# cliarie/radix-join

Hardware: AMD Instinct MI355X
Metric: probe_tuples_per_sec (higher is better)
Workload: dtype int32

## Files before the change

include/rj.h:

```cpp
#ifndef RJ_H_
#define RJ_H_

#include <stddef.h>
#include <stdint.h>

#ifdef __cplusplus
extern "C" {
#endif

#define RJ_PAGE_SIZE 8192u

typedef enum rj_dtype {
    RJ_INT32   = 0,
    RJ_INT64   = 1,
    RJ_FP64    = 2,
    RJ_VARCHAR = 3
} rj_dtype;

typedef enum rj_status {
    RJ_OK            = 0,
    RJ_ERR_ARG       = 1,
    RJ_ERR_DEVICE    = 2,
    RJ_ERR_NOMEM     = 3,
    RJ_ERR_DATA      = 4,
// ... 18 lines not shown
    RJ_AGG_SUM        = 3,
    RJ_AGG_MIN        = 4,
    RJ_AGG_MAX        = 5
} rj_agg_func;
#define RJ_AGG_OUT(func, col) (((uint64_t)(func) << 56) | (uint64_t)(col))
#define RJ_AGG_FUNC(x) ((uint32_t)((uint64_t)(x) >> 56))
#define RJ_AGG_COL(x) ((uint64_t)(x) & 0x00ffffffffffffffull)

typedef struct rj_node {
    int32_t         kind;
    int32_t         build_left;
    uint64_t        base_table_id;
    uint64_t        left, right;
    uint64_t        left_attr, right_attr;
    uint64_t        n_out;
    const uint64_t* out_idx;
    const int32_t*  out_type;
} rj_node;

typedef struct rj_column {
    int32_t            type;
    uint64_t           n_pages;
    const void* const* pages;
} rj_column;

typedef struct rj_input {
    uint64_t         num_rows;
    uint64_t         n_cols;
    const rj_column* cols;
} rj_input;

typedef struct rj_plan {
    uint64_t        n_nodes;
    const rj_node*  nodes;
    uint64_t        n_inputs;
    const rj_input* inputs;
    uint64_t        root;
} rj_plan;

typedef struct rj_context rj_context;

#define RJ_COMM_ID_BYTES 128
typedef struct rj_comm_id { char bytes[RJ_COMM_ID_BYTES]; } rj_comm_id;
int rj_comm_id_create(rj_comm_id* out);

enum { RJ_EXCHANGE_AUTO = 0, RJ_EXCHANGE_P2P = 1, RJ_EXCHANGE_RCCL = 2 };

typedef struct rj_config {
    int32_t  device;
    int32_t  profile;
    void*    stream;
    int32_t  radix_bits;
    int32_t  n_devices;
    const int32_t* devices;
    int32_t  world_size;
    int32_t  rank_base;
    const rj_comm_id* comm_id;
    int32_t  exchange;
    int32_t  flags;
} rj_config;

enum { RJ_CTX_PREWARM = 1 };

int         rj_context_create(rj_context** out, const rj_config* cfg );
void        rj_context_destroy(rj_context* ctx);
const char* rj_last_error(const rj_context* ctx);
int         rj_abi_version(void);
uint32_t    rj_context_n_devices(const rj_context* ctx);
rj_context* rj_context_device(rj_context* ctx, uint32_t i);

typedef struct rj_table rj_table;

int  rj_table_upload(rj_context* ctx, const rj_input* host, rj_table** out);

int  rj_table_adopt_device(rj_context* ctx, uint64_t num_rows, uint64_t n_cols,
                           const int32_t* col_type, const void* const* dev_pages,
                           const uint64_t* n_pages, rj_table** out);
void rj_table_release(rj_context* ctx, rj_table* t);

typedef enum rj_filter_opcode {
    RJ_F_EQ = 0, RJ_F_NEQ = 1, RJ_F_LT = 2, RJ_F_GT = 3, RJ_F_LEQ = 4, RJ_F_GEQ = 5,
    RJ_F_IS_NULL = 6, RJ_F_IS_NOT_NULL = 7,
    RJ_F_HOST_BITMAP = 8,
    RJ_F_AND = 9, RJ_F_OR = 10, RJ_F_NOT = 11,
    RJ_F_LIKE = 12, RJ_F_NOT_LIKE = 13
} rj_filter_opcode;

typedef struct rj_filter_op {
    int32_t        op;
    int32_t        column;
    int64_t        ivalue;
    const uint8_t* bytes;
} rj_filter_op;

int rj_table_from_csv(rj_context* ctx, const char* text, uint64_t n_bytes, uint64_t n_cols,
                      const int32_t* col_type, const rj_filter_op* filter, uint64_t n_filter_ops,
                      rj_table** out);
int rj_debug_parse_fp64(const char* field, uint64_t n, uint64_t* bits);
uint64_t rj_table_num_rows(const rj_table* t);
uint64_t rj_table_col_pages(const rj_table* t, uint64_t col);
int      rj_table_copy_pages(rj_context* ctx, const rj_table* t, uint64_t col, void* const* dst, uint64_t n_dst);

typedef struct rj_result rj_result;

enum { RJ_EXEC_KEEP_ON_DEVICE = 1 };

int rj_execute(rj_context* ctx, const rj_plan* plan, rj_result** out);
int rj_execute_resident(rj_context* ctx, const rj_plan* plan, rj_table* const* tables,
                        uint64_t n_tables, int32_t flags, rj_result** out);

uint64_t rj_result_num_rows(const rj_result* r);
uint64_t rj_result_num_cols(const rj_result* r);
int32_t  rj_result_col_type(const rj_result* r, uint64_t col);
uint64_t rj_result_col_pages(const rj_result* r, uint64_t col);
int      rj_result_copy_pages(rj_result* r, uint64_t col, void* const* dst, uint64_t n_dst);
const void* rj_result_device_pages(const rj_result* r, uint64_t col);
void     rj_result_free(rj_result* r);

int rj_execute_sharded(rj_context* ctx, const rj_plan* plan, rj_table* const* tables,
                       uint64_t n_inputs, int32_t flags, rj_result** out );
int rj_plan_shardable(const rj_plan* plan, char* why, size_t why_cap);

int rj_exchange_plan(uint32_t world, uint32_t subs, uint32_t rank, const uint64_t* counts,
                     uint64_t* send_off, uint64_t* send_cnt, uint64_t* recv_off, uint64_t* recv_cnt,
                     uint32_t* seg_begin, uint32_t* seg_end, uint32_t* part_off, uint64_t* n_recv);

typedef struct rj_tuples {
    uint64_t n;
    void*    key;
    void*    carry;
    uint32_t hashed;
    uint32_t reserved;
} rj_tuples;

int  rj_shard_partition(rj_context* ctx, const rj_table* t, uint64_t key_col,
                        uint64_t carry_col, uint32_t n_ranks, rj_tuples* out,
                        uint64_t* counts );

int  rj_join_tuples(rj_context* ctx, const rj_tuples* build, const rj_tuples* probe,
                    uint32_t skip_rank_bits, int32_t flags, rj_result** out);

typedef struct rj_kernel_stat {
    char     name[48];
    uint64_t launches;
    double   total_ms;
} rj_kernel_stat;

int  rj_profile_read(rj_context* ctx, rj_kernel_stat* out, uint64_t cap, uint64_t* n);
void rj_profile_reset(rj_context* ctx);

int  rj_debug_launch_log(rj_context* ctx, int on);
int  rj_debug_launch_read(rj_context* ctx, char* buf, uint64_t cap, uint64_t* need);
int  rj_debug_pool(rj_context* ctx, uint64_t out[4]);

typedef struct rj_device_info {
    char     name[128];
    char     arch[64];
    int32_t  compute_units;
    int32_t  wavefront;
    uint64_t hbm_bytes;
    uint64_t lds_per_cu;
    int32_t  device_count;
    int32_t  reserved;
} rj_device_info;
int rj_device_query(rj_context* ctx, rj_device_info* out);

#ifdef __cplusplus
}
#endif
#endif
```

radix-join_amd/csrc/rj_api.hip:

```cpp
#include <chrono>
#include <cstdlib>
#include <mutex>

#include "rj_internal.hpp"
#include "rj_xplan.hpp"

using namespace rj;

static std::mutex  g_err_mu;
static std::string g_create_error;

template <class F>
static int guarded(rj_context* ctx, F&& f) {
    try {
        f();
        return RJ_OK;
    } catch (const rj::Error& e) {
        if (ctx) ctx->last_error = e.what();
        return e.code;
    } catch (const std::bad_alloc&) {
        if (ctx) ctx->last_error = "host allocation failed";
        return RJ_ERR_NOMEM;
    } catch (const std::exception& e) {
        if (ctx) ctx->last_error = e.what();
// ... 35 lines not shown
            c->device = dev;
            if (first && cfg && cfg->stream) {
                c->stream = static_cast<hipStream_t>(cfg->stream);
            } else {
                RJ_HIP(hipStreamCreateWithFlags(&c->stream, hipStreamNonBlocking));
                c->own_stream = true;
            }
            c->prof.on = cfg && cfg->profile;
            c->prof.level = cfg && cfg->profile >= 2 ? 2 : 1;
            c->prof.stream = c->stream;
            c->radix_bits_override = cfg ? cfg->radix_bits : 0;
            c->tune.from_env();
            c->pool.set_poison(c.get(), c->tune.debug_poison);
            if (!c->radix_bits_override && c->tune.radix_bits > 0) c->radix_bits_override = c->tune.radix_bits;
            return c;
        };
        std::unique_ptr<rj_context> c = make_lane(devs[0], true);
        for (size_t i = 1; i < devs.size(); ++i) {
            rj_context* p = make_lane(devs[i], false).release();
            p->group = c.get();
            c->peers.push_back(p);
        }
        const int world = cfg && cfg->world_size > 0 ? cfg->world_size : (int)devs.size();
        if (world > 1 || (cfg && cfg->exchange != RJ_EXCHANGE_AUTO)) {
            std::vector<Context*> lanes;
            for (int i = 0; i < c->n_lanes(); ++i) lanes.push_back(c->lane(i));
            c->comm.reset(new Comm(lanes, world, cfg ? cfg->rank_base : 0, cfg ? cfg->exchange : 0,
                                   cfg ? cfg->comm_id : nullptr, c->tune.exchange_timeout_ms,
                                   c->tune.bringup_timeout_ms));
        }
        if (cfg && (cfg->flags & RJ_CTX_PREWARM))
            for (int i = 0; i < c->n_lanes(); ++i) c->lane(i)->prewarm();
        RJ_HIP(hipSetDevice(devs[0]));
        *out = c.release();
    } catch (const rj::Error& e) {
        code = e.code;
        msg = e.what();
    } catch (const std::exception& e) {
        code = RJ_ERR_DEVICE;
        msg = e.what();
    }
    if (code != RJ_OK) {
        std::lock_guard<std::mutex> g(g_err_mu);
        g_create_error = msg;
    }
    return code;
}

void rj_context_destroy(rj_context* ctx) {
    if (!ctx) return;
    if (ctx->group) {
        ctx->last_error = "rj_context_destroy: this is a per-device handle owned by its group context (ignored)";
        return;
    }
    delete ctx;
}

uint32_t rj_context_n_devices(const rj_context* ctx) { return ctx ? (uint32_t)ctx->n_lanes() : 0; }

rj_context* rj_context_device(rj_context* ctx, uint32_t i) {
    if (!ctx || i >= (uint32_t)ctx->n_lanes()) return nullptr;
    return static_cast<rj_context*>(ctx->lane((int)i));
}

int rj_comm_id_create(rj_comm_id* out) {
    if (!out) return RJ_ERR_ARG;
    try {
        Comm::make_id(out);
        return RJ_OK;
    } catch (const std::exception& e) {
        std::lock_guard<std::mutex> g(g_err_mu);
        g_create_error = e.what();
        return RJ_ERR_DEVICE;
    }
}

const char* rj_last_error(const rj_context* ctx) {
    if (ctx) return ctx->last_error.c_str();
    std::lock_guard<std::mutex> g(g_err_mu);
    return g_create_error.c_str();
}

int rj_table_upload(rj_context* ctx, const rj_input* host, rj_table** out) {
    if (!ctx || !out) return RJ_ERR_ARG;
    *out = nullptr;
    return guarded(ctx, [&] {
        RJ_HIP(hipSetDevice(ctx->device));
        *out = static_cast<rj_table*>(table_upload(ctx, host));
    });
}

int rj_table_adopt_device(rj_context* ctx, uint64_t num_rows, uint64_t n_cols,
                          const int32_t* col_type, const void* const* dev_pages,
                          const uint64_t* n_pages, rj_table** out) {
    if (!ctx || !out || (n_cols && (!col_type || !dev_pages || !n_pages))) return RJ_ERR_ARG;
    *out = nullptr;
    return guarded(ctx, [&] {
        RJ_HIP(hipSetDevice(ctx->device));
        *out = static_cast<rj_table*>(
            table_adopt(ctx, num_rows, n_cols, col_type, dev_pages, n_pages));
    });
}

int rj_table_from_csv(rj_context* ctx, const char* text, uint64_t n_bytes, uint64_t n_cols, const int32_t* col_type,
                      const rj_filter_op* filter, uint64_t n_filter_ops, rj_table** out) {
    if (!ctx || !out || (n_filter_ops && !filter)) return RJ_ERR_ARG;
    *out = nullptr;
    return guarded(ctx, [&] {
        RJ_HIP(hipSetDevice(ctx->device));
        *out = static_cast<rj_table*>(table_from_csv(ctx, text, n_bytes, n_cols, col_type, filter, n_filter_ops));
    });
}

int rj_debug_parse_fp64(const char* field, uint64_t n, uint64_t* bits) {
    if (!bits || (n && !field)) return RJ_ERR_ARG;
    return rj::parse_fp64_host(field, n, bits);
}

int rj_debug_launch_log(rj_context* ctx, int on) {
    if (!ctx) return RJ_ERR_ARG;
    for (int l = 0; l < ctx->n_lanes(); ++l) {
        ctx->lane(l)->klog.clear();
        ctx->lane(l)->klog.on = on != 0;
    }
    return RJ_OK;
}

int rj_debug_launch_read(rj_context* ctx, char* buf, uint64_t cap, uint64_t* need) {
    if (!ctx || !need || (cap && !buf)) return RJ_ERR_ARG;
    return guarded(ctx, [&] {
        std::map<std::string, uint64_t> all;
        for (int l = 0; l < ctx->n_lanes(); ++l) ctx->lane(l)->klog.merge_into(all);
        std::string text;
        for (const auto& kv : all) text += kv.first + " " + std::to_string(kv.second) + "\n";
        *need = text.size() + 1;
        if (cap) {
            const size_t n = std::min<size_t>(text.size(), cap - 1);
            memcpy(buf, text.data(), n);
            buf[n] = 0;
        }
    });
}

int rj_debug_pool(rj_context* ctx, uint64_t out[4]) {
    if (!ctx || !out) return RJ_ERR_ARG;
    out[0] = out[1] = out[2] = out[3] = 0;
    for (int l = 0; l < ctx->n_lanes(); ++l) {
        const DevPool& p = ctx->lane(l)->pool;
        out[0] += p.bytes_in_use();
        out[1] += p.bytes_cached();
        out[2] += p.n_fills();
        out[3] += p.bytes_filled();
    }
    return RJ_OK;
}

uint64_t rj_table_num_rows(const rj_table* t) { return t ? t->num_rows : 0; }
uint64_t rj_table_col_pages(const rj_table* t, uint64_t col) { return table_col_pages(t, col); }

int rj_table_copy_pages(rj_context* ctx, const rj_table* t, uint64_t col, void* const* dst, uint64_t n_dst) {
    if (!ctx || !t || (n_dst && !dst)) return RJ_ERR_ARG;
    return guarded(ctx, [&] {
        RJ_HIP(hipSetDevice(ctx->device));
        table_copy_pages(ctx, t, col, dst, n_dst);
    });
}

void rj_table_release(rj_context* ctx, rj_table* t) {
    (void)ctx;
    delete t;
}

int rj_execute_resident(rj_context* ctx, const rj_plan* plan, rj_table* const* tables,
                        uint64_t n_tables, int32_t flags, rj_result** out) {
    if (!ctx || !plan || !out) return RJ_ERR_ARG;
    *out = nullptr;
    return guarded(ctx, [&] {
        RJ_HIP(hipSetDevice(ctx->device));
        std::vector<Table*> ts(n_tables);
        for (uint64_t i = 0; i < n_tables; ++i) {
            if (!tables[i]) throw rj::Error(RJ_ERR_ARG, "null table");
            ts[i] = tables[i];
        }
        *out = static_cast<rj_result*>(execute_plan(ctx, plan, ts.data(), n_tables, flags));
    });
}

int rj_execute(rj_context* ctx, const rj_plan* plan, rj_result** out) {
    if (!ctx || !plan || !out) return RJ_ERR_ARG;
    *out = nullptr;
    return guarded(ctx, [&] {
        RJ_HIP(hipSetDevice(ctx->device));
        if (plan->n_inputs && !plan->inputs) throw rj::Error(RJ_ERR_ARG, "plan has no inputs");
        std::vector<bool> used(plan->n_inputs, false);
        for (uint64_t i = 0; i < plan->n_nodes; ++i)
            if (plan->nodes[i].kind == RJ_NODE_SCAN) {
                if (plan->nodes[i].base_table_id >= plan->n_inputs)
                    throw rj::Error(RJ_ERR_ARG, "scan: bad base_table_id");
                used[plan->nodes[i].base_table_id] = true;
            }
        std::vector<std::vector<bool>> col_used(plan->n_inputs);
        for (uint64_t i = 0; i < plan->n_inputs; ++i)
            col_used[i].assign(plan->inputs[i].n_cols, false);
        for (uint64_t i = 0; i < plan->n_nodes; ++i) {
            const rj_node& nd = plan->nodes[i];
            if (nd.kind != RJ_NODE_SCAN) continue;
            for (uint64_t k = 0; k < nd.n_out; ++k) {
                if (nd.out_idx[k] >= col_used[nd.base_table_id].size())
                    throw rj::Error(RJ_ERR_ARG, "scan: output attr out of range");
                col_used[nd.base_table_id][nd.out_idx[k]] = true;
            }
        }
        if (ctx->n_lanes() > 1 && !ctx->group) {
            if (Result* r = execute_host_sharded(ctx, plan, used, col_used)) {
                *out = static_cast<rj_result*>(r);
                return;
            }
        }
        const bool  diag = ctx->tune.diag >= 2;
        auto        t0 = std::chrono::steady_clock::now();
        const uint64_t m0 = ctx->pool.n_malloc, tr0 = ctx->pool.n_trim;
        const double   mm0 = ctx->pool.malloc_ms;
        auto        ms_since = [](std::chrono::steady_clock::time_point t) {
            return std::chrono::duration<double, std::milli>(std::chrono::steady_clock::now() - t).count();
        };
        if (ctx->tune.sync_upload > 0) {
            std::vector<std::unique_ptr<Table>> owned(plan->n_inputs);
            std::vector<Table*>                 ts(plan->n_inputs, nullptr);
            rj_input                            none{};
            for (uint64_t i = 0; i < plan->n_inputs; ++i) {
                owned[i].reset(table_upload(ctx, used[i] ? &plan->inputs[i] : &none,
                                            used[i] ? &col_used[i] : nullptr, true));
                ts[i] = owned[i].get();
            }
            double up = ms_since(t0);
            *out = static_cast<rj_result*>(execute_plan(ctx, plan, ts.data(), plan->n_inputs, 0));
            if (diag)
                fprintf(stderr, "[rj host] upload %.2f ms, then plan (device + host VARCHAR) %.2f ms\n", up,
                        ms_since(t0) - up);
            return;
        }
        AsyncUpload  upl(ctx, plan, used, col_used);
        try {
            *out = static_cast<rj_result*>(execute_plan(ctx, plan, nullptr, plan->n_inputs, 0, &upl));
        } catch (...) {
            (void)hipStreamSynchronize(ctx->stream);
            throw;
        }
        if (diag)
            fprintf(stderr,
                    "[rj host] execute %.2f ms (plan walk blocked on uploads for %.2f ms); HBM cache: %llu "
                    "hipMalloc %.2f ms, %llu trims, %.1f GB in use, %.1f GB cached\n",
                    ms_since(t0), upl.wait_ms(), (unsigned long long)(ctx->pool.n_malloc - m0),
                    ctx->pool.malloc_ms - mm0, (unsigned long long)(ctx->pool.n_trim - tr0),
                    ctx->pool.bytes_in_use() / 1e9, ctx->pool.bytes_cached() / 1e9);
    });
}

uint64_t rj_result_num_rows(const rj_result* r) { return r ? r->num_rows : 0; }
uint64_t rj_result_num_cols(const rj_result* r) { return r ? r->cols.size() : 0; }
int32_t  rj_result_col_type(const rj_result* r, uint64_t c) {
    return (r && c < r->cols.size()) ? r->cols[c].type : -1;
}
uint64_t rj_result_col_pages(const rj_result* r, uint64_t c) {
    return (r && c < r->cols.size()) ? r->cols[c].n_pages : 0;
}

int rj_result_copy_pages(rj_result* r, uint64_t col, void* const* dst, uint64_t n_dst) {
    if (!r) return RJ_ERR_ARG;
    return guarded(static_cast<rj_context*>(r->ctx), [&] {
        RJ_HIP(hipSetDevice(r->ctx->device));
        result_copy_pages(r, col, dst, n_dst);
    });
}

const void* rj_result_device_pages(const rj_result* r, uint64_t c) {
    if (!r || c >= r->cols.size() || !r->cols[c].dev_pages) return nullptr;
    if (!r->cols[c].more.empty()) return nullptr;
    return r->cols[c].dev_pages->p;
}

void rj_result_free(rj_result* r) { delete r; }

int rj_execute_sharded(rj_context* ctx, const rj_plan* plan, rj_table* const* tables,
                       uint64_t n_inputs, int32_t flags, rj_result** out) {
    if (!ctx || !plan || !out || (n_inputs && !tables)) return RJ_ERR_ARG;
    const int nl = ctx->n_lanes();
    for (int l = 0; l < nl; ++l) out[l] = nullptr;
    return guarded(ctx, [&] {
        if (ctx->group) throw rj::Error(RJ_ERR_ARG, "rj_execute_sharded wants the group context, not one of its devices");
        std::vector<Table*>  ts((size_t)nl * n_inputs);
        for (size_t i = 0; i < ts.size(); ++i) ts[i] = tables[i];
        std::vector<Result*> rs((size_t)nl, nullptr);
        execute_sharded(ctx, plan, ts.data(), n_inputs, flags, rs.data());
        for (int l = 0; l < nl; ++l) out[l] = static_cast<rj_result*>(rs[l]);
    });
}

int rj_plan_shardable(const rj_plan* plan, char* why, size_t why_cap) {
    std::string w;
    bool        ok = false;
    try {
        ok = plan_shardable(plan, &w);
    } catch (const std::exception& e) {
        w = e.what();
    }
// ... 99 lines not shown
```

radix-join_amd/csrc/rj_context.hip:

```cpp
#include <dlfcn.h>

#include <chrono>
#include <cstdlib>

#include "rj_internal.hpp"

namespace rj {

[[noreturn]] void launch_failed(const char* kernel, const char* what, bool unsupported) {
    throw_fmt(unsupported ? RJ_ERR_UNSUPPORTED : RJ_ERR_DEVICE, "launch %s: %s", kernel, what);
}

static int env_int(const char* name, int def) {
    const char* v = getenv(name);
    return v && *v ? atoi(v) : def;
}

void Tuning::from_env() {
    blocked_mid = env_int("RJ_TUNE_BLOCKED_MID", blocked_mid);
    mall_chunk = env_int("RJ_TUNE_MALL_CHUNK", mall_chunk);
    radix_bits = env_int("RJ_TUNE_RADIX_BITS", radix_bits);
    p1_bits = env_int("RJ_TUNE_P1_BITS", p1_bits);
    fine = env_int("RJ_TUNE_FINE", fine);
    pack = env_int("RJ_TUNE_PACK", pack);
    aos3 = env_int("RJ_TUNE_AOS3", aos3);
    aos_mid = env_int("RJ_TUNE_AOS_MID", aos_mid);
    tpg1 = env_int("RJ_TUNE_TPG1", tpg1);
    xcd_split = env_int("RJ_TUNE_XCD_SPLIT", xcd_split);
    tpg2 = env_int("RJ_TUNE_TPG2", tpg2);
    packed_side = env_int("RJ_TUNE_PACKED_SIDE", packed_side);
    xcd_min_rows = env_int("RJ_TUNE_XCD_MIN_ROWS", xcd_min_rows);
    bcast = env_int("RJ_TUNE_BCAST", bcast);
    diag = env_int("RJ_DIAG", diag);
    varchar_dev_rows = env_int("RJ_TUNE_VARCHAR_DEV", varchar_dev_rows);
    vkey_hash_bits = env_int("RJ_DEBUG_VKEY_HASH_BITS", vkey_hash_bits);
    sync_upload = env_int("RJ_SYNC_UPLOAD", sync_upload);
    wide_carry = env_int("RJ_TUNE_WIDE_CARRY", wide_carry);
    fold_owner = env_int("RJ_TUNE_FOLD_OWNER", fold_owner);
    exchange_timeout_ms = env_int("RJ_EXCHANGE_TIMEOUT_MS", exchange_timeout_ms);
    bringup_timeout_ms = env_int("RJ_BRINGUP_TIMEOUT_MS", bringup_timeout_ms);
    debug_shard_fail = env_int("RJ_DEBUG_SHARD_FAIL", debug_shard_fail);
    debug_shard_fail_rank = env_int("RJ_DEBUG_SHARD_FAIL_RANK", debug_shard_fail_rank);
    if (const char* v = getenv("RJ_DEBUG_POISON"))
        debug_poison = (int)strtol(v, nullptr, 0) & 0x1ff;
}

static size_t round_size(size_t n) {
    const size_t small = 256, big = size_t(2) << 20;
    if (n < (size_t(1) << 20)) return (n + small - 1) / small * small;
    return (n + big - 1) / big * big;
}

void* DevPool::alloc(size_t bytes) {
    size_t need = round_size(bytes ? bytes : 1);
    int    best = -1;
    for (size_t i = 0; i < blocks_.size(); ++i) {
        Block& b = blocks_[i];
        if (!b.free || b.size < need) continue;
        if (b.size > need + need / 2 + (size_t(4) << 20)) continue;
        if (best < 0 || b.size < blocks_[best].size) best = (int)i;
    }
    if (best >= 0) {
        if (poison_) {
            hipError_t e = fill(blocks_[best].p, blocks_[best].size);
            if (e != hipSuccess) throw_fmt(RJ_ERR_DEVICE, "RJ_DEBUG_POISON: fill on alloc failed: %s", hipGetErrorString(e));
        }
        blocks_[best].free = false;
        in_use_ += blocks_[best].size;
        cached_ -= blocks_[best].size;
        return blocks_[best].p;
    }
    void*      p = nullptr;
    auto       t0 = std::chrono::steady_clock::now();
    hipError_t e = hipMalloc(&p, need);
    if (e != hipSuccess) {
        (void)hipGetLastError();
        trim();
        ++n_trim;
        e = hipMalloc(&p, need);
        if (e != hipSuccess) {
            (void)hipGetLastError();
            throw_fmt(RJ_ERR_NOMEM, "hipMalloc(%zu bytes) failed: %s", need, hipGetErrorString(e));
        }
    }
    ++n_malloc;
    malloc_ms += std::chrono::duration<double, std::milli>(std::chrono::steady_clock::now() - t0).count();
    if (poison_) {
        hipError_t f = fill(p, need);
        if (f != hipSuccess) {
            (void)hipFree(p);
            throw_fmt(RJ_ERR_DEVICE, "RJ_DEBUG_POISON: fill on alloc failed: %s", hipGetErrorString(f));
        }
    }
    blocks_.push_back({p, need, false});
    in_use_ += need;
    return p;
}

hipError_t DevPool::fill(void* p, size_t bytes) {
    Context* c = owner_;
    int      prev = -1;
    if (hipGetDevice(&prev) != hipSuccess) prev = -1;
    hipError_t e = prev == c->device ? hipSuccess : hipSetDevice(c->device);
    for (hipStream_t s : {c->stream, c->aux, c->copy_stream})
        if (e == hipSuccess && s) e = hipStreamSynchronize(s);
    if (e == hipSuccess) e = hipMemsetAsync(p, poison_ & 0xff, bytes, c->stream);
    if (e == hipSuccess) e = hipStreamSynchronize(c->stream);
    if (e == hipSuccess) {
        n_fill_.fetch_add(1, std::memory_order_relaxed);
        fill_bytes_.fetch_add(bytes, std::memory_order_relaxed);
    } else {
        (void)hipGetLastError();
    }
    if (prev >= 0 && prev != c->device) (void)hipSetDevice(prev);
    return e;
}

void DevPool::release(void* p) {
    if (!p) return;
    for (Block& b : blocks_)
        if (b.p == p && !b.free) {
            if (poison_ & 0x100) (void)fill(b.p, b.size);
            b.free = true;
            in_use_ -= b.size;
            cached_ += b.size;
            return;
        }
}

void DevPool::trim() {
    std::vector<Block> keep;
    for (Block& b : blocks_) {
        if (b.free) {
            (void)hipFree(b.p);
            cached_ -= b.size;
        } else {
            keep.push_back(b);
        }
    }
    blocks_.swap(keep);
}

DevPool::~DevPool() {
    for (Block& b : blocks_) (void)hipFree(b.p);
}

Buf::Buf(Context* c, size_t n) : ctx(c), bytes(n) { p = c->pool.alloc(n); }
Buf::~Buf() {
    if (ctx && p) ctx->pool.release(p);
}

hipEvent_t Profiler::get_event() {
    if (!spare_.empty()) {
        hipEvent_t e = spare_.back();
        spare_.pop_back();
        return e;
    }
    hipEvent_t e;
    RJ_HIP(hipEventCreate(&e));
    return e;
}

static bool hot_kernel(const char* n) {
    return !strncmp(n, "pass", 4) || !strncmp(n, "join_build", 10) || !strncmp(n, "exchange", 8);
}

bool Profiler::timed(const char* name, hipEvent_t* start, hipEvent_t* stop) {
    if (!on || (level < 2 && !hot_kernel(name))) return false;
    Rec r{name, get_event(), get_event()};
    open_.push_back(r);
    *start = r.a;
    *stop = r.b;
    return true;
}

void Profiler::drain() {
    if (open_.empty()) return;
    RJ_HIP(hipStreamSynchronize(stream));
    for (Rec& r : open_) {
        float ms = 0;
        if (hipEventElapsedTime(&ms, r.a, r.b) == hipSuccess) {
            auto it = totals.find(r.name);
            if (it == totals.end()) {
                order.push_back(r.name);
// ... 154 lines not shown
```

radix-join_amd/csrc/rj_device.hpp:

```cpp
#pragma once
#include <stdint.h>

namespace rj {

constexpr uint32_t PAGE_BYTES = 8192;
constexpr uint32_t ROWS32 = 1984;
constexpr uint32_t ROWS64 = 1007;
constexpr uint32_t HDR32 = 4;
constexpr uint32_t HDR64 = 8;

enum ColKind : int32_t {
    COL_NONE  = 0,
    COL_PAGED = 1,
    COL_DENSE = 2,
    COL_IOTA  = 3
};

struct ColRef {
    const uint8_t* ptr;
    const uint8_t* valid;
    int32_t        kind;
    int32_t        width;
};

enum CarryMode : int32_t {
    CARRY_NONE   = 0,
    CARRY_ROWIDX = 1,
    CARRY_COLUMN = 2,
    CARRY_WIDE   = 3
};

enum WideLayout : int32_t {
    WIDE_NONE = 0,
    WIDE_32S  = 1,
    WIDE_64_32 = 2
};

struct TupleSrc {
    ColRef   key;
    ColRef   carry;
    uint32_t n_rows;
    int32_t  carry_mode;
    int32_t  key_f64;
    int32_t  prehashed;
    int32_t  wide;
    int32_t  pad;
    ColRef   carry2, carry3;
};

constexpr int MAX_WORDS = 4;
struct Words {
    uint32_t* w[MAX_WORDS];
};

#ifndef RJ_PT_THREADS
#define RJ_PT_THREADS 1024
#endif
#ifndef RJ_PT_ITEMS
#define RJ_PT_ITEMS 16
#endif
constexpr int PT_THREADS = RJ_PT_THREADS;
constexpr int PT_ITEMS   = RJ_PT_ITEMS;
constexpr int PT_TILE    = PT_THREADS * PT_ITEMS;
constexpr uint32_t PT_ALL_ITEMS = PT_ITEMS >= 32 ? 0xffffffffu : ((1u << (PT_ITEMS & 31)) - 1u);
#ifndef RJ_PT_CAPBITS
#define RJ_PT_CAPBITS 9
#endif
constexpr int PT_CAPBITS = RJ_PT_CAPBITS;
constexpr int PT_MAXF    = 1 << PT_CAPBITS;
constexpr int PT_MAXBITS = 9;
static_assert(PT_CAPBITS >= PT_MAXBITS && PT_CAPBITS <= 10, "fan-out capacity");
constexpr int PT_FINEBITS = 15;
constexpr int LDS_BYTES  = 160 * 1024;
static_assert(PT_THREADS >= PT_MAXF, "thread d scans digit d");
static_assert(PT_TILE * 8 + 3 * PT_MAXF * 4 + (PT_THREADS / 64) * 4 <= LDS_BYTES,
              "scatter tile does not fit the 160 KiB of LDS");
static_assert((4 << PT_FINEBITS) <= LDS_BYTES, "fine histogram does not fit the LDS");
static_assert(PT_TILE <= 65536, "ranks are packed into 16 bits");
static_assert(PT_ITEMS % 4 == 0 && PT_ITEMS <= 32, "full tiles are loaded as 16-byte vectors; one mask bit per item");

struct PassParams {
    const uint32_t* seg_off;
    const uint32_t* grp_start;
    uint32_t        nseg;
    uint32_t        n;
    uint32_t        shift;
    uint32_t        fanout_log2;
    uint32_t        tiles_per_group;
    uint32_t*       hist;
    uint32_t*       cursor;
    uint32_t        xcd_log2;
    uint32_t        xcd_remap;
    uint16_t*       side_out;
    uint32_t        next_shift, next_mask;
    const uint32_t* seg_end;
    uint32_t        oseg_shift;
    uint32_t        grp_base;
    uint32_t        hi_shift, lo_bits;
};

__host__ __device__ inline uint32_t pass_digit(const PassParams& pp, uint32_t w, uint32_t mask) {
    if (pp.hi_shift) return (((w >> pp.shift) & ((1u << pp.lo_bits) - 1u)) | ((w >> pp.hi_shift) << pp.lo_bits)) & mask;
    return (w >> pp.shift) & mask;
}

#ifndef RJ_JN_THREADS
#define RJ_JN_THREADS 512
#endif
#ifndef RJ_JN_SPT
#define RJ_JN_SPT 8
#endif
#ifndef RJ_JN_CAP
#define RJ_JN_CAP 8192
#endif
constexpr int      JN_THREADS = RJ_JN_THREADS;
constexpr int      JN_SPT     = RJ_JN_SPT;
constexpr int      JN_SUB     = JN_THREADS * JN_SPT;
constexpr int      JN_CAP     = RJ_JN_CAP;
constexpr int      JN_RMAX    = JN_CAP / 2;
constexpr int      JN_RPT     = (JN_RMAX + JN_THREADS - 1) / JN_THREADS;
constexpr int jn_threads(int table_words) { return table_words >= 3 ? 2 * JN_THREADS : JN_THREADS; }
constexpr int jn_min_waves(int table_words) {
    int blocks = (160 * 1024) / (JN_CAP * 4 * table_words + JN_CAP + 1024);
    int w = blocks * jn_threads(table_words) / 256;
    return w > 8 ? 8 : (w < 1 ? 1 : w);
}
static_assert(JN_RPT % 4 == 0 && JN_SPT % 4 == 0, "tuples are loaded as 16-byte vectors");
static_assert(JN_CAP * 4 * 4 + JN_CAP + 1024 <= 160 * 1024, "a four-array join table does not fit the LDS");
#ifndef RJ_JN_PPW
#define RJ_JN_PPW 1
#endif
#ifndef RJ_JN_PPW3
#define RJ_JN_PPW3 4
#endif
constexpr int jn_ppw(int table_words) { return table_words >= 3 ? RJ_JN_PPW3 : RJ_JN_PPW; }
#ifndef RJ_JN_HEAVY
#define RJ_JN_HEAVY 65536
#endif
constexpr uint32_t JN_HEAVY   = RJ_JN_HEAVY;
constexpr uint32_t JN_TARGET_BUILD = JN_RMAX * 3 / 4;

enum StreamMode : int32_t {
    ST_NONE    = 0,
    ST_DENSE32 = 1,
    ST_DENSE64 = 2,
    ST_PAGED32 = 3,
    ST_PAGED64 = 4,
    ST_DENSE96 = 5
};

struct OutStream {
    uint8_t* base;
    int32_t  mode;
    int32_t  pad;
};

struct JoinParams {
    Words           R, S;
    const uint32_t* offR;
    const uint32_t* offS;
    uint32_t        NP;
    uint32_t        radix_bits;
    uint32_t        n_pass;
    uint32_t        pass_bits[4];
    OutStream       key, bc, pc;
    unsigned long long* out_cursor;
    uint64_t        out_cap;
    const uint32_t* heavy_tasks;
    const uint32_t* n_heavy;
    uint32_t        heavy_grid;
    int32_t         packR, packS;
    int32_t         aosR, aosS;
    int32_t         pad;
    unsigned long long* diag;
};

struct SplitParams {
    const uint32_t* rec;
    uint32_t        cw;
    int32_t         n_cols;
    int32_t         valid_word;
    int32_t         pad;
    struct Col {
        uint8_t* out;
        uint8_t* valid;
        int32_t  word;
        int32_t  width;
        int32_t  valid_bit;
        int32_t  paged;
    } col[3];
};

struct VcRow {
    uint32_t page;
    uint32_t beg;
    uint32_t len;
};
struct VcPage {
    uint32_t first;
    uint32_t nr;
    uint32_t kind;
};
constexpr uint32_t VC_CHUNK = 512;

struct BcastParams {
    TupleSrc        R, S;
    OutStream       key, bc, pc;
    unsigned long long* out_cursor;
    uint64_t        out_cap;
};

struct FilterParams {
    TupleSrc        F, P;
    Words           Fw, Pw;
    const uint32_t* offF;
    const uint32_t* offP;
    uint32_t        NP;
    uint32_t        radix_bits;
    int32_t         packP, aosP;
    const uint32_t* heavy_tasks;
    const uint32_t* n_heavy;
    uint32_t        heavy_grid;
    int32_t         anti;
    int32_t         keyless;
    int32_t         pad;
    OutStream       key, pc;
    unsigned long long* out_cursor;
    uint64_t        out_cap;
};

constexpr uint32_t OUTER_NO_ROW = 0xffffffffu;
struct OuterParams {
    TupleSrc        B, P;
    Words           Bw, Pw;
    const uint32_t* offB;
    const uint32_t* offP;
    uint32_t        NP;
    uint32_t        radix_bits;
    int32_t         packB, aosB;
    int32_t         packP, aosP;
    const uint32_t* heavy_tasks;
    const uint32_t* n_heavy;
    uint32_t        heavy_grid;
    int32_t         keyless;
    uint32_t        pad_bc;
    int32_t         pad;
    OutStream       key, bc, pc;
    unsigned long long* out_cursor;
    uint64_t        out_cap;
};

struct FullParams {
    OuterParams     o;
    uint32_t*       flags;
    uint32_t        pad_pc;
    int32_t         use_flags;
};

constexpr int AGG_THREADS = 512;
constexpr int AGG_SPT     = 2;
constexpr int AGG_STEP    = AGG_THREADS * AGG_SPT;
constexpr int AGG_CAP     = 1024;
constexpr int AGG_FREEZE  = AGG_CAP * 5 / 8;
constexpr int AGG_WALK    = 32;
constexpr uint32_t AGG_TARGET = AGG_CAP * 3 / 8;
constexpr int AGG_MAX_COLS = 3;
static_assert((AGG_CAP & (AGG_CAP - 1)) == 0 && AGG_CAP % AGG_THREADS == 0, "table entries: a power of two, whole rows of threads");
static_assert(AGG_CAP * (12 + 28 * AGG_MAX_COLS) + 1024 <= LDS_BYTES, "the widest aggregation table does not fit the LDS");

enum AggNeed : uint32_t { AGG_NEED_COUNT = 1, AGG_NEED_SUM = 2, AGG_NEED_MIN = 4, AGG_NEED_MAX = 8 };
struct AggCol {
    int32_t  word;
    int32_t  width;
    int32_t  valid_bit;
    uint32_t need;
};
struct AggArrays {
    uint8_t*            key;
    unsigned long long* rows;
    unsigned long long* nn[AGG_MAX_COLS];
    unsigned long long* sum[AGG_MAX_COLS];
    long long*          mn[AGG_MAX_COLS];
    long long*          mx[AGG_MAX_COLS];
};
constexpr unsigned long long AGG_NO_KEY = ~0ull;
struct AggParams {
    TupleSrc        src;
    Words           W;
    const uint32_t* off;
    uint32_t        NP;
    int32_t         pack, aos;
    const uint32_t* heavy_tasks;
    const uint32_t* n_heavy;
    uint32_t        heavy_grid;
    int32_t         n_cols;
    int32_t         valid_word;
    AggCol          col[AGG_MAX_COLS];
    AggArrays       out;
    uint8_t*        out_keyvalid;
    unsigned long long* out_cursor;
    uint64_t        out_cap;
    AggArrays       m;
    uint32_t        m_slots;
    uint32_t*       m_overflow;
};

}
// ... 1 lines not shown
```

radix-join_amd/csrc/rj_exec.hip:

```cpp
#include <algorithm>
#include <chrono>
#include <cstdlib>
#include <functional>
#include <set>

#include "rj_internal.hpp"
#include "rj_xplan.hpp"

namespace rj {

namespace {

struct DCol {
    int32_t        type = RJ_INT32;
    int32_t        kind = COL_NONE;
    int32_t        width = 4;
    const uint8_t* ptr = nullptr;
    const uint8_t* valid = nullptr;
    BufP           hold, hold_valid;
    int            vc_table = -1, vc_col = -1;
    const TableColumn* tcol = nullptr;
    ColRef ref() const { return ColRef{ptr, valid, kind, width}; }
};

// ... 132 lines not shown

    void run_shard(const Table* t, uint64_t key_col, uint64_t carry_col, uint32_t n_ranks,
                   rj_tuples* out, uint64_t* counts) {
        if (n_ranks == 0 || (n_ranks & (n_ranks - 1)) || n_ranks > (1u << PT_MAXBITS))
            throw_fmt(RJ_ERR_UNSUPPORTED, "n_ranks must be a power of two <= %d", 1 << PT_MAXBITS);
        if (key_col >= t->cols.size() || carry_col >= t->cols.size())
            throw_fmt(RJ_ERR_ARG, "column out of range");
        DCol k = table_col(t, (int)key_col), c = table_col(t, (int)carry_col);
        if (k.type != RJ_INT32 || c.type != RJ_INT32)
            throw_fmt(RJ_ERR_UNSUPPORTED, "sharded path carries INT32 key + INT32 payload");
        if (c.valid) throw_fmt(RJ_ERR_UNSUPPORTED, "sharded path: payload column has NULLs");
        TupleSrc src{};
        src.key = k.ref();
        src.carry = c.ref();
        src.n_rows = (uint32_t)t->num_rows;
        src.carry_mode = CARRY_COLUMN;
        if (!out->key || !out->carry) throw_fmt(RJ_ERR_ARG, "rj_shard_partition: null output buffers");
        uint32_t rb = ceil_log2(n_ranks);
        Words    ext{};
        ext.w[0] = static_cast<uint32_t*>(out->key);
        ext.w[1] = static_cast<uint32_t*>(out->carry);
        Parted P = partition(&src, nullptr, 1, 1, rb, rb ? 32 - rb : 31,  true, &ext);
        std::vector<uint32_t> off(n_ranks + 1);
        RJ_HIP(hipMemcpyAsync(off.data(), P.off->p, (n_ranks + 1) * 4, hipMemcpyDeviceToHost,
                              ctx->stream));
        ctx->sync();
        for (uint32_t r = 0; r < n_ranks; ++r) counts[r] = off[r + 1] - off[r];
        out->n = off[n_ranks];
        out->hashed = 1;
        out->reserved = 0;
    }

    Context*       ctx;
    const rj_plan* plan;
    Table* const*  tables;
    uint64_t       n_tables;
    int            flags;
    TableFetch*    fetch = nullptr;
    Launch         L;
    std::map<std::pair<const Table*, int>, DCol> decoded_;
    std::map<std::pair<int, int>, std::vector<uint64_t>> vc_dir_;

    DCol table_col(const Table* t, int c) {
        const TableColumn& tc = t->cols[c];
        if (tc.skipped) throw_fmt(RJ_ERR_ARG, "column was not uploaded (not referenced by a scan)");
        DCol               d;
        d.type = tc.type;
        d.tcol = &tc;
        if (tc.type == RJ_VARCHAR) {
            d.kind = COL_IOTA;
            d.width = 4;
            return d;
        }
        d.width = tc.type == RJ_INT32 ? 4 : 8;
        if (t->num_rows == 0) {
            d.kind = COL_DENSE;
            return d;
        }
        if (tc.regular) {
            d.kind = COL_PAGED;
            d.ptr = tc.dev_pages;
            return d;
        }
        auto key = std::make_pair(t, c);
        auto it = decoded_.find(key);
        if (it != decoded_.end()) return it->second;
        uint64_t n = t->num_rows;
        d.kind = COL_DENSE;
        d.hold = ctx->buf(n * d.width);
        d.hold_valid = ctx->buf(n);
        RJ_HIP(hipMemsetAsync(d.hold->p, 0, n * d.width, ctx->stream));
        RJ_HIP(hipMemsetAsync(d.hold_valid->p, 0, n, ctx->stream));
        if (tc.n_pages) {
            BufP row_base = ctx->buf((tc.n_pages + 1) * 4);
            launch_scan_bins(L, tc.page_rows->as<uint32_t>(), (uint32_t)tc.n_pages,
                             row_base->as<uint32_t>(), nullptr);
            launch_decode_pages(L, tc.dev_pages, (uint32_t)tc.n_pages, d.width,
                                row_base->as<uint32_t>(), n, d.hold->as<uint8_t>(),
                                d.hold_valid->as<uint8_t>());
        }
        d.ptr = d.hold->as<uint8_t>();
        d.valid = d.hold_valid->as<uint8_t>();
        decoded_[key] = d;
        return d;
    }

    const Table* table_of(const rj_node& n) {
        return table_by_id(n.base_table_id);
    }
    const Table* table_by_id(uint64_t id) {
        if (id >= n_tables) throw_fmt(RJ_ERR_ARG, "scan: bad base_table_id");
        return fetch ? fetch->get(id) : tables[id];
    }

    Rel scan(const rj_node& n) {
        const Table* t = table_of(n);
        Rel          r;
        r.n = t->num_rows;
        for (uint64_t k = 0; k < n.n_out; ++k) {
            uint64_t c = n.out_idx[k];
            if (c >= t->cols.size()) throw_fmt(RJ_ERR_ARG, "scan: output attr out of range");
            if (t->cols[c].type != n.out_type[k])
                throw_fmt(RJ_ERR_ARG, "scan: declared type differs from the column's type");
            DCol d = table_col(t, (int)c);
            if (d.type == RJ_VARCHAR) {
                d.vc_table = (int)n.base_table_id;
                d.vc_col = (int)c;
            }
            r.cols.push_back(d);
        }
        return r;
    }

    void root_scan(const rj_node& n, Result& res) {
        const Table* t = table_of(n);
        res.num_rows = t->num_rows;
        for (uint64_t k = 0; k < n.n_out; ++k) {
            uint64_t c = n.out_idx[k];
            if (c >= t->cols.size()) throw_fmt(RJ_ERR_ARG, "scan: output attr out of range");
            const TableColumn& tc = t->cols[c];
            if (tc.type != n.out_type[k])
                throw_fmt(RJ_ERR_ARG, "scan: declared type differs from the column's type");
            ResultColumn rc;
            rc.type = tc.type;
            rc.n_pages = tc.n_pages;
            if (tc.skipped) throw_fmt(RJ_ERR_ARG, "column was not uploaded");
            if (tc.type == RJ_VARCHAR) {
                rc.n_pages = tc.vc_pages.size();
                rc.host_pages.resize(rc.n_pages * PAGE_BYTES);
                for (uint64_t pg = 0; pg < rc.n_pages; ++pg)
                    memcpy(rc.host_pages.data() + pg * PAGE_BYTES, tc.vc_pages[pg], PAGE_BYTES);
            } else if (tc.n_pages) {
                rc.dev_pages = ctx->buf(tc.n_pages * PAGE_BYTES);
                RJ_HIP(hipMemcpyAsync(rc.dev_pages->p, tc.dev_pages, tc.n_pages * PAGE_BYTES,
                                      hipMemcpyDeviceToDevice, ctx->stream));
            }
            res.cols.push_back(std::move(rc));
        }
    }

    Rel node(uint64_t idx, Result* root_res, int depth) {
        if (idx >= plan->n_nodes) throw_fmt(RJ_ERR_ARG, "bad node index");
        if (depth > 4096) throw_fmt(RJ_ERR_ARG, "plan too deep (cycle?)");
        const rj_node& n = plan->nodes[idx];
        if (n.kind == RJ_NODE_SCAN) return scan(n);
        if (n.kind == RJ_NODE_AGG) {
            Rel child = node(n.left, nullptr, depth + 1);
            return agg(child, n, root_res);
        }
        const JoinKind& K = join_kind(n.kind);
        Rel             l = node(n.left, nullptr, depth + 1);
        Rel             r = node(n.right, nullptr, depth + 1);
        const JoinSpec  js = join_spec(n, ctx->radix_bits_override);
        if (n.kind == RJ_NODE_OUTER) return outer_join(l, r, js, K, root_res);
        if (n.kind == RJ_NODE_FULL) return full_join(l, r, js, K, root_res);
        if (n.kind != RJ_NODE_JOIN) return filter_join(l, r, js, K, root_res);
        return join_core(l, r, js, root_res);
    }

    static uint32_t tiles_per_group(uint64_t tuples_per_segment, uint64_t target_groups) {
        uint64_t k = (tuples_per_segment + (uint64_t)PT_TILE * target_groups - 1) /
                     ((uint64_t)PT_TILE * target_groups);
        return (uint32_t)std::min<uint64_t>(std::max<uint64_t>(k, 1), 8);
    }

    Parted partition(const TupleSrc* srcp, const WordSrc* ws, int KW, int CW, uint32_t bits,
                     uint32_t shift0 = 0, bool single_pass = false, const Words* external = nullptr,
                     const std::function<void(const uint32_t*)>* after_offsets = nullptr,
                     const PassShape* shape = nullptr) {
        Parted P;
        const bool preseg = shape && shape->nseg > 0;
        P.NW = KW + CW;
        const TupleSrc none{};
        const TupleSrc& src = srcp ? *srcp : none;
        const uint64_t  n = ws ? ws->n : src.n_rows;
        uint32_t       passes = single_pass ? 1 : (bits + PT_MAXBITS - 1) / PT_MAXBITS;
        if (passes == 0) passes = 1;
        std::vector<uint32_t> pbits(passes, bits / passes);
        for (uint32_t i = 0; i < bits % passes; ++i) pbits[i]++;
        if (passes == 2 && ctx->tune.p1_bits > 0) {
            uint32_t b1 = (uint32_t)ctx->tune.p1_bits;
            if (b1 < bits && b1 <= PT_CAPBITS && bits - b1 <= PT_CAPBITS) {
                pbits[0] = b1;
                pbits[1] = bits - b1;
            }
        }

        const bool fine = passes == 2 && bits <= (uint32_t)PT_FINEBITS && !external && !shape &&
                          ctx->tune.fine != 0;
        const int pack_mode = ctx->tune.pack;
        P.packed = ws ? ws->packed
                      : (!external && KW == 1 && CW == 1 && (pack_mode == 1 || (pack_mode == 2 && fine)));
        P.aos3 = KW == 1 && CW == 2 && !external && !single_pass && ctx->tune.aos3 != 0;
        const bool aos_mid = P.aos3 && passes >= 2 &&
                             (ctx->tune.aos_mid == 1 || ctx->tune.aos_mid == 3 || (ctx->tune.aos_mid == 2 && fine));
        const bool mid_side = aos_mid && !fine && ctx->tune.aos_mid != 3;
        BufP  A[MAX_WORDS], B[MAX_WORDS], AOS, MID[2], SIDE[2];
        Words wa{}, wb{}, waos{};
        if (P.aos3) {
            AOS = ctx->buf(std::max<uint64_t>(n, 1) * 12);
            waos.w[0] = AOS->as<uint32_t>();
        }
        if (aos_mid) {
            for (uint32_t k = 0; k < std::min<uint32_t>(passes - 1, 2); ++k) {
                MID[k] = ctx->buf(std::max<uint64_t>(n, 1) * 12);
                if (mid_side) SIDE[k] = ctx->buf(std::max<uint64_t>(n, 1) * 2 + 16);
            }
        }
        const bool packed_side = P.packed && !fine && passes >= 2 && ctx->tune.packed_side != 0 &&
                                 n >= (uint64_t)ctx->tune.xcd_min_rows;
        if (packed_side)
            for (uint32_t k = 0; k < std::min<uint32_t>(passes - 1, 2); ++k)
                SIDE[k] = ctx->buf(std::max<uint64_t>(n, 1) * 2 + 16);
        const int pair_word = CW >= 2 ? KW + CW - 2 : -1;
        for (int a = 0; a < (P.packed ? 1 : P.NW); ++a) {
            if (pair_word >= 0 && a == pair_word + 1) continue;
            const uint64_t wbytes = (P.packed || a == pair_word) ? 8 : 4;
            if (external) {
                wa.w[a] = external->w[a];
                continue;
            }
            if ((P.aos3 && passes == 1) || aos_mid) continue;
            A[a] = ctx->buf(n * wbytes + 2048);
            wa.w[a] = A[a]->as<uint32_t>();
            if (passes > (P.aos3 ? 2u : 1u)) {
                B[a] = ctx->buf(n * wbytes + 2048);
                wb.w[a] = B[a]->as<uint32_t>();
            }
        }
        BufP     seg_off;
        uint32_t nseg = 1, shift = shift0;
        Words    cur = ws ? ws->w : Words{}, nxt = (P.aos3 && passes == 1) ? waos : wa;
        bool     cur_is_a = false;
        BufP       fine_off, fine_cursor, coarse_off, coarse_cursor;
        uint32_t tpg_first = tiles_per_group(n, 4096);
        if (ctx->tune.tpg1 > 0) tpg_first = (uint32_t)ctx->tune.tpg1;
        bool fine_xcd = false;
        if (fine) {
            const uint32_t NB = 1u << bits, F1 = 1u << pbits[0], F2 = 1u << pbits[1];
            BufP           fh = ctx->buf((uint64_t)NB * 4);
            const uint64_t tiles = (n + PT_TILE - 1) / PT_TILE;
            uint32_t       fgrid = (uint32_t)std::min<uint64_t>(tiles, (uint64_t)ctx->compute_units());
            fine_xcd = ctx->tune.xcd_split && n >= (uint64_t)ctx->tune.xcd_min_rows && fgrid >= 8;
            if (fine_xcd) fgrid &= ~7u;
            fine_off = ctx->buf(((uint64_t)NB + 1) * 4);
            fine_cursor = ctx->buf((uint64_t)NB * 4);
            coarse_off = ctx->buf(((uint64_t)F1 + 1) * 4);
            coarse_cursor = ctx->buf((uint64_t)F1 * 4 * (fine_xcd ? 8 : 1));
            BufP coarse_x;
            RJ_HIP(hipMemsetAsync(fh->p, 0, (uint64_t)NB * 4, ctx->stream));
            if (fine_xcd) {
                coarse_x = ctx->buf((uint64_t)F1 * 8 * 4);
                RJ_HIP(hipMemsetAsync(coarse_x->p, 0, (uint64_t)F1 * 8 * 4, ctx->stream));
            }
            uint32_t* cx = fine_xcd ? coarse_x->as<uint32_t>() : nullptr;
            if (ws)
                launch_fine_hist_words(L, ws->w, ws->packed, (uint32_t)n, shift0, pbits[0], pbits[1], fgrid,
                                       fh->as<uint32_t>(), fine_xcd ? tpg_first : 0u, cx);
            else
                launch_fine_hist_src(L, src, KW, shift0, pbits[0], pbits[1], fgrid, fh->as<uint32_t>(),
                                     fine_xcd ? tpg_first : 0u, cx);
            launch_scan_fine(L, fh->as<uint32_t>(), F1, F2, fine_off->as<uint32_t>(),
                             fine_cursor->as<uint32_t>(), coarse_off->as<uint32_t>(),
                             coarse_cursor->as<uint32_t>(), cx);
        }
        struct Ev2 {
            hipEvent_t e = nullptr;
            void       make() { RJ_HIP(hipEventCreateWithFlags(&e, hipEventDisableTiming)); }
            ~Ev2() {
                if (e) (void)hipEventDestroy(e);
            }
        } chunk_ev;
        const bool chunk_second = ctx->tune.mall_chunk > 0 && passes == 2 && !fine && !shape && !ws && !external && P.packed &&
                                  !packed_side && ctx->tune.xcd_split && n >= (uint64_t)ctx->tune.xcd_min_rows;
        const bool blocked_mid = ctx->tune.blocked_mid != 0 && P.packed && passes >= 2 && !fine && !shape && !ws && !external &&
                                 !packed_side && !chunk_second;
        for (uint32_t p = 0; p < passes; ++p) {
            const uint32_t F = 1u << pbits[p];
            PassParams     pp{};
            pp.nseg = nseg;
            pp.n = (uint32_t)n;
            pp.shift = shift;
            pp.fanout_log2 = pbits[p];
            uint32_t n_groups;
            BufP     grp_start;
            const bool      first_preseg = p == 0 && preseg;
            const uint32_t  nseg_in = first_preseg ? shape->nseg : nseg;
            const uint32_t  n_oseg = first_preseg ? shape->n_oseg : nseg;
            const uint64_t  bins = (uint64_t)n_oseg * F;
            if (p == 0 && shape && shape->hi_shift) {
                pp.hi_shift = shape->hi_shift;
                pp.lo_bits = shape->lo_bits;
            }
            if (p == 0 && !preseg) {
                pp.tiles_per_group = tpg_first;
                uint64_t gt = (uint64_t)pp.tiles_per_group * PT_TILE;
                n_groups = (uint32_t)((n + gt - 1) / gt);
            } else {
                pp.tiles_per_group = tiles_per_group(n / nseg_in + 1, 16);
                if (P.aos3 && p + 1 == passes) pp.tiles_per_group = std::min<uint32_t>(pp.tiles_per_group, 2u);
                uint64_t gt = (uint64_t)pp.tiles_per_group * PT_TILE;
                if (ctx->tune.tpg2 > 0) {
                    pp.tiles_per_group = (uint32_t)ctx->tune.tpg2;
                    gt = (uint64_t)pp.tiles_per_group * PT_TILE;
                }
                n_groups = (uint32_t)(n / gt + nseg_in);
                if (ctx->tune.xcd_split && n >= (uint64_t)ctx->tune.xcd_min_rows) {
                    pp.xcd_remap = 1;
                    n_groups += 8;
                }
                const uint32_t* in_off = first_preseg ? shape->seg_begin : seg_off->as<uint32_t>();
                grp_start = ctx->buf(((uint64_t)nseg_in + 1) * 4);
                launch_group_table(L, in_off, nseg_in, (uint32_t)gt, grp_start->as<uint32_t>(),
                                   first_preseg ? shape->seg_end : nullptr);
                pp.nseg = nseg_in;
                pp.seg_off = in_off;
                pp.seg_end = first_preseg ? shape->seg_end : nullptr;
                pp.oseg_shift = first_preseg ? shape->oseg_shift : 0u;
                pp.grp_start = grp_start->as<uint32_t>();
            }
            BufP off, hist, cursor;
            if (fine) {
                off = p == 0 ? coarse_off : fine_off;
                cursor = p == 0 ? coarse_cursor : fine_cursor;
                pp.cursor = cursor->as<uint32_t>();
                pp.xcd_log2 = (p == 0 && fine_xcd) ? 3u : 0u;
            } else {
                pp.xcd_log2 = (ctx->tune.xcd_split && p == 0 && !preseg && n >= (uint64_t)ctx->tune.xcd_min_rows) ? 3u : 0u;
                hist = ctx->buf((bins << pp.xcd_log2) * 4);
                off = ctx->buf((bins + 1) * 4);
                cursor = ctx->buf((bins << pp.xcd_log2) * 4);
                RJ_HIP(hipMemsetAsync(hist->p, 0, (bins << pp.xcd_log2) * 4, ctx->stream));
                pp.hist = hist->as<uint32_t>();
                pp.cursor = cursor->as<uint32_t>();
                if (p == 1 && chunk_second) {
                    RJ_HIP(hipEventSynchronize(chunk_ev.e));
                    const uint32_t* hoff = static_cast<const uint32_t*>(ctx->small_pinned());
                    const uint64_t  gt = (uint64_t)pp.tiles_per_group * PT_TILE;
                    std::vector<uint32_t> gstart(nseg_in + 1, 0);
                    for (uint32_t sgi = 0; sgi < nseg_in; ++sgi)
                        gstart[sgi + 1] = gstart[sgi] + (uint32_t)(((uint64_t)(hoff[sgi + 1] - hoff[sgi]) + gt - 1) / gt);
                    Ev2 e_in, e_aux;
                    e_in.make();
                    e_aux.make();
                    hipStream_t aux = ctx->aux_stream();
                    RJ_HIP(hipEventRecord(e_in.e, ctx->stream));
                    RJ_HIP(hipStreamWaitEvent(aux, e_in.e, 0));
                    Launch L2 = L;
                    L2.stream = aux;
                    const uint32_t CH = (uint32_t)ctx->tune.mall_chunk;
                    uint32_t       c = 0;
                    for (uint32_t s0 = 0; s0 < nseg_in; s0 += CH, ++c) {
                        const uint32_t s1 = std::min(nseg_in, s0 + CH), G = gstart[s1] - gstart[s0];
                        const Launch& Lc = (c & 1u) ? L2 : L;
                        PassParams    pc = pp;
                        pc.nseg = s1 - s0;
                        pc.seg_off = pp.seg_off + s0;
                        pc.grp_start = pp.grp_start + s0;
                        pc.grp_base = gstart[s0];
                        pc.hist = pp.hist + (size_t)s0 * F;
                        pc.cursor = pp.cursor + (size_t)s0 * F;
                        const uint32_t grid = pp.xcd_remap ? ((G + 7u) & ~7u) : G;
                        if (G) launch_pass_hist_packed(Lc, cur.w[0], pc, grid);
                        launch_scan_segments(Lc, pc.hist, pc.seg_off, pc.nseg, F, 0, off->as<uint32_t>() + (size_t)s0 * F, pc.cursor);
                        if (G) launch_pass_scatter_packed(Lc, cur.w[0], pc, grid, nxt.w[0]);
                    }
                    RJ_HIP(hipEventRecord(e_aux.e, aux));
                    RJ_HIP(hipStreamWaitEvent(ctx->stream, e_aux.e, 0));
                    seg_off = off;
                    nseg = (uint32_t)bins;
                    shift += pbits[p];
                    cur = nxt;
                    cur_is_a = (p % 2 == 0);
                    nxt = cur_is_a ? wb : wa;
                    continue;
                }
                if (p == 0 && !ws)
                    launch_pass_hist_src(L, src, KW, pp, n_groups);
                else if ((mid_side || packed_side) && p > 0)
                    launch_pass_hist_digits(L, SIDE[(p - 1) % 2]->as<uint16_t>(), pp, n_groups);
                else if (aos_mid && p > 0)
                    launch_pass_hist_aos3(L, MID[(p - 1) % 2]->as<uint32_t>(), pp, n_groups);
                else if (P.packed && blocked_mid && p > 0)
                    launch_pass_hist_blocked(L, cur.w[0], pp, n_groups);
                else if (P.packed)
                    launch_pass_hist_packed(L, cur.w[0], pp, n_groups);
                else
                    launch_pass_hist_dense(L, cur, pp, n_groups);
                launch_scan_segments(L, pp.hist, first_preseg ? shape->oseg_off : (p == 0 ? nullptr : pp.seg_off),
                                     n_oseg, F, pp.xcd_log2, off->as<uint32_t>(), pp.cursor);
            }
            if (p == 0 && after_offsets) (*after_offsets)(off->as<uint32_t>());
            if (p == 0 && chunk_second) {
                if ((bins + 1) * 4 > Context::SMALL_PINNED / 4) throw_fmt(RJ_ERR_DEVICE, "chunked pass: too many segments");
                RJ_HIP(hipMemcpyAsync(ctx->small_pinned(), off->p, (bins + 1) * 4, hipMemcpyDeviceToHost, ctx->stream));
                chunk_ev.make();
                RJ_HIP(hipEventRecord(chunk_ev.e, ctx->stream));
            }
            if (aos_mid) {
                const bool last = p + 1 == passes;
                Words      o{};
                o.w[0] = last ? waos.w[0] : MID[p % 2]->as<uint32_t>();
                if (!last && mid_side) {
                    pp.side_out = SIDE[p % 2]->as<uint16_t>();
                    pp.next_shift = shift + pbits[p];
                    pp.next_mask = (1u << pbits[p + 1]) - 1u;
                }
                if (p == 0 && !ws)
                    launch_pass_scatter_src(L, src, KW, CW, pp, n_groups, o, true);
                else if (p == 0)
                    launch_pass_scatter_dense(L, cur, P.NW, KW, pp, n_groups, o, true);
                else
                    launch_pass_scatter_aos3(L, MID[(p - 1) % 2]->as<uint32_t>(), pp, n_groups, o.w[0]);
                nxt = o;
            } else if (P.packed) {
                if (packed_side && p + 1 < passes) {
                    pp.side_out = SIDE[p % 2]->as<uint16_t>();
                    pp.next_shift = shift + pbits[p];
                    pp.next_mask = (1u << pbits[p + 1]) - 1u;
                }
                const bool blk_out = blocked_mid && p + 1 < passes;
                if (p == 0 && !ws)
                    launch_pass_scatter_src_packed(L, src, pp, n_groups, nxt.w[0], blk_out);
                else if (blocked_mid)
                    launch_pass_scatter_blocked(L, cur.w[0], pp, n_groups, nxt.w[0], blk_out);
                else
                    launch_pass_scatter_packed(L, cur.w[0], pp, n_groups, nxt.w[0]);
            } else if (p == 0 && !ws) {
                launch_pass_scatter_src(L, src, KW, CW, pp, n_groups, nxt, P.aos3 && p + 1 == passes);
            } else {
                launch_pass_scatter_dense(L, cur, P.NW, pair_word, pp, n_groups, nxt,
                                          P.aos3 && p + 1 == passes);
            }
            seg_off = off;
            nseg = (uint32_t)bins;
            shift += pbits[p];
            cur = nxt;
            cur_is_a = (p % 2 == 0);
            nxt = cur_is_a ? wb : wa;
            if (P.aos3 && p + 2 == passes) nxt = waos;
            if (aos_mid) {
            }
        }
        P.w = cur;
        for (int a = 0; a < P.NW; ++a) P.wbuf[a] = cur_is_a ? A[a] : B[a];
        if (P.aos3) P.wbuf[0] = AOS;
        P.off = seg_off;
        P.NP = nseg;
        P.pbits = pbits;
        if (shape && !shape->prior_bits.empty()) P.pbits.insert(P.pbits.begin(), shape->prior_bits.begin(), shape->prior_bits.end());
        P.n_tuples = n;
        return P;
    }

    struct Side {
        Rel*          rel = nullptr;
        uint64_t      key_col = 0;
        std::set<int> need;
        int           carry_mode = CARRY_NONE;
        int           carry_col = -1;
        int           CW = 0;
        BufP          stream;
        int           stream_mode = ST_NONE;
        std::vector<int> wide_cols;
        int              wide = WIDE_NONE;
        int              valid_word = -1;
        BufP             vword;
        struct WideOut {
            BufP values, valid;
            int  mode = ST_NONE;
        };
        std::map<int, WideOut> wide_out;
        uint64_t null_mask = 0;
        bool     shared = false;
        bool     optional = false;
        bool     nullable(int c) const {
            if (optional || rel->cols[c].valid != nullptr) return true;
            return shared && (c >= 64 || ((null_mask >> c) & 1u));
        }
    };
    static uint64_t null_columns(const Rel& r) {
        uint64_t m = 0;
        for (size_t c = 0; c < r.cols.size() && c < 64; ++c)
            if (r.cols[c].valid != nullptr) m |= 1ull << c;
        return m;
    }

    static uint64_t pages_for(uint64_t rows, int width) {
        uint64_t rf = width == 4 ? ROWS32 : ROWS64;
        return (rows + rf - 1) / rf;
    }

    Rel empty_rel(const JoinSpec& js, Result* root_res) {
        Rel r;
        r.n = 0;
        for (size_t k = 0; k < js.out_type.size(); ++k) {
            DCol d;
            d.type = js.out_type[k];
            d.kind = COL_DENSE;
            d.width = d.type == RJ_INT32 || d.type == RJ_VARCHAR ? 4 : 8;
            r.cols.push_back(d);
        }
        if (root_res) {
            root_res->num_rows = 0;
            for (size_t k = 0; k < js.out_type.size(); ++k) {
                ResultColumn rc;
                rc.type = js.out_type[k];
                root_res->cols.push_back(std::move(rc));
            }
        }
        return r;
    }

    struct JoinState {
        Side     ls, rs;
        bool     build_left = true, is_root = false, f64 = false, need_key_stream = false;
        bool     type_mismatch = false;
        size_t   lw = 0, rw = 0;
        int      KW = 1;
        uint64_t cap_hint = 0;
        const JoinKind* kind = nullptr;
        bool vkey = false;
        struct VKey {
            Rel            rel;
            BufP           rows, hash, valid;
            const uint8_t* pages = nullptr;
            uint32_t       n_pages = 0;
        } vk[2];
        Side&    bs() { return build_left ? ls : rs; }
        Side&    ps() { return build_left ? rs : ls; }
    };

    void join_prepare(Rel& left, Rel& right, const JoinSpec& js, bool is_root, JoinState& st, const JoinKind& K,
                      const uint64_t* shared_nulls = nullptr) {
        st.kind = &K;
        const size_t lw = left.cols.size(), rw = right.cols.size();
        st.lw = lw;
        st.rw = rw;
        st.is_root = is_root;
        st.build_left = js.build_left;
        if (js.left_attr >= lw || js.right_attr >= rw)
            throw_fmt(RJ_ERR_ARG, "join: key attr out of range");
        for (size_t k = 0; k < js.out_idx.size(); ++k) {
            if (js.out_idx[k] >= lw + rw) throw_fmt(RJ_ERR_ARG, "join: output attr out of range");
            const DCol& c = js.out_idx[k] < lw ? left.cols[js.out_idx[k]]
                                               : right.cols[js.out_idx[k] - lw];
            if (c.type != js.out_type[k])
                throw_fmt(RJ_ERR_ARG, "join: declared type differs from the child column's type");
        }
        Side &ls = st.ls, &rs = st.rs;
        ls.rel = &left;
        ls.key_col = js.left_attr;
        rs.rel = &right;
        rs.key_col = js.right_attr;
        if (shared_nulls) {
            ls.shared = rs.shared = true;
            ls.null_mask = shared_nulls[0];
            rs.null_mask = shared_nulls[1];
        }
        const DCol& bk = st.bs().rel->cols[st.bs().key_col];
        const DCol& pk = st.ps().rel->cols[st.ps().key_col];
        if (bk.type < RJ_INT32 || bk.type > RJ_VARCHAR) throw_fmt(RJ_ERR_ARG, "Unsupported join type");
        st.type_mismatch = pk.type != bk.type;
        st.vkey = bk.type == RJ_VARCHAR && !st.type_mismatch;
        st.KW = bk.type == RJ_INT32 ? 1 : 2;
        st.f64 = bk.type == RJ_FP64;
        const bool key_stream_ok =
            K.node == RJ_NODE_JOIN ||
            (!st.type_mismatch && !(K.emits_unmatched && st.ps().rel->cols[st.ps().key_col].valid));
        st.bs().optional = K.build_optional;
        st.ps().optional = K.probe_optional;
        for (size_t k = 0; k < js.out_idx.size(); ++k) {
            bool  is_left = js.out_idx[k] < lw;
            Side& s = is_left ? ls : rs;
            int   c = (int)(is_left ? js.out_idx[k] : js.out_idx[k] - lw);
            if ((uint64_t)c == s.key_col && !st.vkey && key_stream_ok && !s.optional)
                st.need_key_stream = true;
            else
                s.need.insert(c);
        }
        for (Side* s : {&ls, &rs}) {
            if (st.vkey) {
                s->carry_mode = CARRY_ROWIDX;
                s->CW = 1;
            } else if (s->need.empty()) {
                s->carry_mode = CARRY_NONE;
                s->CW = 0;
            } else if (s->need.size() == 1 && !s->nullable(*s->need.begin())) {
                s->carry_mode = CARRY_COLUMN;
                s->carry_col = *s->need.begin();
                s->CW = s->rel->cols[s->carry_col].width / 4;
            } else if (plan_wide_carry(*s, st.KW)) {
                s->carry_mode = CARRY_WIDE;
            } else {
                s->carry_mode = CARRY_ROWIDX;
                s->CW = 1;
            }
        }
        st.cap_hint = std::max(left.n, right.n);
    }

    bool plan_wide_carry(Side& s, int KW, bool honour_switch = true) {
        if ((honour_switch && !ctx->tune.wide_carry) || s.need.empty()) return false;
        int  words = 0, n64 = 0;
        bool any_null = false;
        for (int c : s.need) {
            const DCol& col = s.rel->cols[c];
            if (col.width != 4 && col.width != 8) return false;
            words += col.width / 4;
            n64 += col.width == 8;
            any_null = any_null || s.nullable(c);
        }
        if (any_null) ++words;
        if (words < 2 || words > MAX_WORDS - KW || n64 > 1 || (n64 == 1 && words != 3)) return false;
        s.wide_cols.clear();
        for (int c : s.need)
            if (s.rel->cols[c].width == 8) s.wide_cols.push_back(c);
        for (int c : s.need)
            if (s.rel->cols[c].width == 4) s.wide_cols.push_back(c);
        s.wide = n64 ? WIDE_64_32 : WIDE_32S;
        s.valid_word = any_null ? words - 1 : -1;
        s.CW = words;
        return true;
    }

    void prepare_wide(Side& s) {
        if (s.carry_mode != CARRY_WIDE || s.valid_word < 0 || s.rel->n == 0) return;
        const uint8_t* v[3] = {nullptr, nullptr, nullptr};
        for (size_t i = 0; i < s.wide_cols.size() && i < 3; ++i) v[i] = s.rel->cols[s.wide_cols[i]].valid;
        s.vword = ctx->buf(s.rel->n * 4);
        launch_pack_validity(L, v[0], v[1], v[2], (uint32_t)s.rel->n, s.vword->as<uint32_t>());
    }

    uint32_t join_bits(const JoinSpec& js, uint64_t build_n, uint32_t top_bits_taken = 0) {
        uint32_t bits = js.forced_bits > 0 ? (uint32_t)js.forced_bits
                                           : ceil_log2((build_n + JN_TARGET_BUILD - 1) / JN_TARGET_BUILD);
        if (js.forced_bits <= 0 && bits > 2 * PT_MAXBITS &&
            (build_n >> (2 * PT_MAXBITS)) <= (uint64_t)(JN_RMAX * 0.95))
            bits = 2 * PT_MAXBITS;
        bits = std::min<uint32_t>(std::max<uint32_t>(bits, 1), 21);
        if (top_bits_taken && bits > 32 - top_bits_taken) bits = 32 - top_bits_taken;
        return bits;
    }

    TupleSrc make_src(const JoinState& st, const Side& s, const JoinSpec& js) {
        TupleSrc src{};
        src.key = s.rel->cols[s.key_col].ref();
        src.n_rows = (uint32_t)s.rel->n;
        src.carry_mode = s.carry_mode;
        if (s.carry_mode == CARRY_COLUMN) {
            src.carry = s.rel->cols[s.carry_col].ref();
            if (src.carry.kind == COL_IOTA) src.carry_mode = CARRY_ROWIDX;
        }
        if (s.carry_mode == CARRY_WIDE) {
            ColRef refs[3] = {};
            size_t k = 0;
            for (int c : s.wide_cols) refs[k++] = s.rel->cols[c].ref();
            if (s.valid_word >= 0)
                refs[k++] = ColRef{s.vword ? s.vword->as<uint8_t>() : nullptr, nullptr, COL_DENSE, 4};
            src.wide = s.wide;
            src.carry = refs[0];
            src.carry2 = refs[1];
            src.carry3 = refs[2];
        }
        src.key_f64 = st.f64 ? 1 : 0;
        src.prehashed = js.prehashed ? 1 : 0;
        return src;
    }


    bool broadcast_form(JoinState& st, const JoinSpec& js) const {
        const uint64_t nb = st.bs().rel->n;
        return (nb <= (uint64_t)JN_RMAX && js.forced_bits <= 0 && !js.prehashed && ctx->tune.bcast != 0) || nb == 0 ||
               st.type_mismatch;
    }
    uint32_t stride_grid(uint64_t rows) const {
        return (uint32_t)std::min<uint64_t>((rows + JN_SUB - 1) / JN_SUB, (uint64_t)ctx->compute_units() * 8);
    }

    struct CoParts {
        Parted   B, P;
        BufP     tasks;
        uint32_t max_tasks = 0;
    };
    CoParts partition_sides(JoinState& st, const JoinSpec& js, uint32_t bits) {
        CoParts        cp;
        const TupleSrc sb = make_src(st, st.bs(), js), sp = make_src(st, st.ps(), js);
        cp.B = partition(&sb, nullptr, st.KW, st.bs().CW, bits);
        cp.P = partition(&sp, nullptr, st.KW, st.ps().CW, bits);
        return cp;
    }
    void heavy_tasks(CoParts& cp, const BufP& counters) {
        cp.max_tasks = (uint32_t)(2 * (cp.P.n_tuples / JN_HEAVY) + 2);
        cp.tasks = ctx->buf((uint64_t)cp.max_tasks * 12);
        launch_heavy_tasks_zeroed(cp.B, cp.P, cp.tasks, counters, cp.max_tasks);
    }
    CoParts co_partition(JoinState& st, const JoinSpec& js, uint32_t bits, const BufP& counters) {
        CoParts cp = partition_sides(st, js, bits);
        heavy_tasks(cp, counters);
        return cp;
    }
    BufP zeroed_counters() {
        BufP counters = ctx->buf(16);
        RJ_HIP(hipMemsetAsync(counters->p, 0, 16, ctx->stream));
        return counters;
    }
    template <class Params>
    static void set_heavy(Params& p, const CoParts& cp, const BufP& counters, uint32_t bits) {
        p.NP = cp.B.NP;
        p.radix_bits = bits;
        p.heavy_tasks = cp.tasks->as<uint32_t>();
        p.n_heavy = counters->as<uint32_t>() + 2;
        p.heavy_grid = cp.max_tasks;
    }
    static void set_parts(OuterParams& op, const CoParts& cp, const BufP& counters, uint32_t bits) {
        set_heavy(op, cp, counters, bits);
        op.Bw = cp.B.w;
        op.Pw = cp.P.w;
        op.offB = cp.B.off->as<uint32_t>();
        op.offP = cp.P.off->as<uint32_t>();
        op.packB = cp.B.packed ? 1 : 0;
        op.aosB = cp.B.aos3 ? 1 : 0;
        op.packP = cp.P.packed ? 1 : 0;
        op.aosP = cp.P.aos3 ? 1 : 0;
    }

    static OutStream out_stream(const BufP& b, int mode) { return OutStream{b ? b->as<uint8_t>() : nullptr, mode, 0}; }
    static OutStream out_stream(const Side& s) { return out_stream(s.stream, s.stream_mode); }
    static uint64_t first_cap(uint64_t rows) { return std::min<uint64_t>(rows + 1024, 0xfffffff0ull); }

    struct Emitted {
        uint64_t        nrows = 0;
        BufP            key_stream;
        int             key_mode = ST_NONE;
        std::set<void*> finished;
    };
    template <class LaunchFn>
    Emitted emit_with_retry(JoinState& st, const BufP& counters, uint64_t cap, LaunchFn&& launch) {
        const JoinKind& K = *st.kind;
        Emitted         e;
        e.key_mode = st.need_key_stream ? stream_mode_of(st.is_root, st.KW * 4, true) : ST_NONE;
        for (int attempt = 1;; ++attempt) {
            e.key_stream = e.key_mode != ST_NONE ? ctx->buf(stream_bytes(e.key_mode, cap)) : BufP();
            for (Side* s : {&st.ls, &st.rs})
                s->stream = s->stream_mode != ST_NONE ? ctx->buf(stream_bytes(s->stream_mode, cap)) : BufP();
            if (K.attempts > 1) RJ_HIP(hipMemsetAsync(counters->p, 0, 8, ctx->stream));
            launch(out_stream(e.key_stream, e.key_mode), cap);
            e.finished.clear();
            finish_paged_streams(st, e, counters, cap);
            unsigned long long h = 0;
            RJ_HIP(hipMemcpyAsync(&h, counters->p, 8, hipMemcpyDeviceToHost, ctx->stream));
            ctx->sync();
            e.nrows = h;
            if (e.nrows <= cap) return e;
            if (K.attempts == 1)
                throw_fmt(RJ_ERR_DEVICE, "%s emitted %llu rows out of %llu", K.name, h, (unsigned long long)cap);
            if (e.nrows > 0xfffffff0ull) throw_fmt(RJ_ERR_UNSUPPORTED, "%s result exceeds 2^32 rows (%llu)", K.name, h);
            if (attempt == K.attempts) throw_fmt(RJ_ERR_DEVICE, "%s output overflowed twice", K.name);
            cap = e.nrows;
        }
    }

    Rel join_core(Rel& left, Rel& right, const JoinSpec& js, Result* root_res) {
        if (left.n == 0 || right.n == 0) return empty_rel(js, root_res);
        JoinState st;
        join_prepare(left, right, js, root_res != nullptr, st, join_kind(RJ_NODE_JOIN));
        if (st.type_mismatch) return empty_rel(js, root_res);
        if (st.vkey) hash_varchar_keys(st);
        prepare_wide(st.ls);
        prepare_wide(st.rs);
        Side&          bs = st.bs();
        Side&          ps = st.ps();
        const uint32_t bits = join_bits(js, bs.rel->n, js.top_bits_taken);
        if (ctx->tune.diag >= 2)
            fprintf(stderr, "[rj diag] join build=%llu probe=%llu bits=%u cw=%d/%d\n",
                    (unsigned long long)bs.rel->n, (unsigned long long)ps.rel->n, bits, bs.CW, ps.CW);
        if (broadcast_form(st, js)) return join_finish(st, js, nullptr, bits, root_res);
        CoParts cp = partition_sides(st, js, bits);
        return join_finish(st, js, &cp, bits, root_res);
    }

    Rel join_finish(JoinState& st, const JoinSpec& js, CoParts* cp, uint32_t bits, Result* root_res) {
        Side &    bs = st.bs(), &ps = st.ps();
        const int KW = st.KW;
        BufP counters = ctx->buf(16);
        if (cp) heavy_tasks(*cp, counters);
        plan_carry_streams(st);
        Emitted e = emit_with_retry(st, counters, first_cap(st.cap_hint), [&](const OutStream& key, uint64_t cap) {
            if (!cp) {
                BcastParams bp{};
                bp.R = make_src(st, bs, js);
                bp.S = make_src(st, ps, js);
                bp.key = key;
                bp.bc = out_stream(bs);
                bp.pc = out_stream(ps);
                bp.out_cursor = counters->as<unsigned long long>();
                bp.out_cap = cap;
                launch_join_bcast(L, KW, bs.CW, ps.CW, bp, stride_grid(ps.rel->n));
                return;
            }
            const Parted &PB = cp->B, &PP = cp->P;
            JoinParams    jp{};
            set_heavy(jp, *cp, counters, bits);
            jp.R = PB.w;
            jp.S = PP.w;
            jp.packR = PB.packed ? 1 : 0;
            jp.packS = PP.packed ? 1 : 0;
            jp.aosR = PB.aos3 ? 1 : 0;
            jp.aosS = PP.aos3 ? 1 : 0;
            jp.offR = PB.off->as<uint32_t>();
            jp.offS = PP.off->as<uint32_t>();
            jp.n_pass = (uint32_t)PB.pbits.size();
            for (size_t i = 0; i < PB.pbits.size() && i < 4; ++i) jp.pass_bits[i] = PB.pbits[i];
            jp.key = key;
            jp.bc = out_stream(bs);
            jp.pc = out_stream(ps);
            jp.out_cursor = counters->as<unsigned long long>();
            jp.out_cap = cap;
            BufP diag;
            if (ctx->tune.diag) {
                diag = ctx->buf(16 * 8);
                RJ_HIP(hipMemsetAsync(diag->p, 0, 16 * 8, ctx->stream));
                jp.diag = diag->as<unsigned long long>();
            }
            const uint32_t ppw = join_partitions_per_workgroup(KW, bs.CW, jp);
            launch_join(L, KW, bs.CW, ps.CW, jp, cp->max_tasks + (PB.NP + ppw - 1) / ppw);
            if (diag) {
                unsigned long long hd[16];
                RJ_HIP(hipMemcpyAsync(hd, diag->p, sizeof hd, hipMemcpyDeviceToHost, ctx->stream));
                ctx->sync();
                static const char* names[] = {"loads issued", "table clear", "build", "count/probe",
                                              "prefix+barrier", "reserve", "emit"};
                double tot = 0;
                for (int i = 0; i < 7; ++i) tot += (double)hd[i];
                fprintf(stderr, "[rj diag] join phases (cycles of thread 0, summed over %u workgroups):\n", PB.NP);
                for (int i = 0; i < 7; ++i)
                    fprintf(stderr, "[rj diag]   %-16s %6.1f %%  %8.0f cyc/wg\n", names[i],
                            100.0 * hd[i] / tot, (double)hd[i] / PB.NP);
            }
        });
        if (st.vkey && e.nrows) e.nrows = verify_varchar_pairs(st, e.nrows);
        return join_assemble(st, js, e, root_res);
    }

    Rel filter_join(Rel& left, Rel& right, const JoinSpec& js, const JoinKind& K, Result* root_res) {
        const bool   anti = K.node == RJ_NODE_ANTI;
        Rel&         fil = js.build_left ? left : right;
        Rel&         pre = js.build_left ? right : left;
        const size_t lw = left.cols.size();
        for (uint64_t o : js.out_idx)
            if (o < lw + right.cols.size() && (o < lw) == js.build_left)
                throw_fmt(RJ_ERR_ARG, "%s: output attr %llu names a column of the filter side", K.name,
                          (unsigned long long)o);
        const uint64_t fattr = js.build_left ? js.left_attr : js.right_attr;
        if (fattr < fil.cols.size() && fil.cols[fattr].type == RJ_VARCHAR)
            throw_fmt(RJ_ERR_UNSUPPORTED, "%s on a VARCHAR key", K.name);
        if (pre.n == 0 || (!anti && fil.n == 0)) return empty_rel(js, root_res);
        JoinState st;
        join_prepare(left, right, js, root_res != nullptr, st, K);
        if (st.type_mismatch && !anti) return empty_rel(js, root_res);
        Side&     fs = st.bs();
        Side&     ps = st.ps();
        const int KW = st.KW;
        prepare_wide(ps);
        plan_carry_streams(st);
        const bool     bcast = broadcast_form(st, js);
        const uint32_t bits = join_bits(js, fs.rel->n);
        if (ctx->tune.diag >= 2)
            fprintf(stderr, "[rj diag] %s filter=%llu preserved=%llu %s bits=%u cw=%d\n", K.name,
                    (unsigned long long)fs.rel->n, (unsigned long long)ps.rel->n, bcast ? "broadcast" : "partitioned",
                    bits, ps.CW);

        FilterParams fp{};
        fp.anti = anti ? 1 : 0;
        fp.keyless = st.type_mismatch ? 1 : 0;
        fp.P = make_src(st, ps, js);
        if (bcast && !fp.keyless) fp.F = make_src(st, fs, js);
        BufP counters = zeroed_counters();
        fp.out_cursor = counters->as<unsigned long long>();
        CoParts cp;
        if (!bcast) {
            cp = co_partition(st, js, bits, counters);
            set_heavy(fp, cp, counters, bits);
            fp.Fw = cp.B.w;
            fp.Pw = cp.P.w;
            fp.offF = cp.B.off->as<uint32_t>();
            fp.offP = cp.P.off->as<uint32_t>();
            fp.packP = cp.P.packed ? 1 : 0;
            fp.aosP = cp.P.aos3 ? 1 : 0;
        }
        Emitted e = emit_with_retry(st, counters, ps.rel->n, [&](const OutStream& key, uint64_t cap) {
            fp.key = key;
            fp.pc = out_stream(ps);
            fp.out_cap = cap;
            if (bcast) {
                launch_filter_bcast(L, KW, ps.CW, fp, stride_grid(ps.rel->n));
            } else {
                launch_filter_join(L, KW, ps.CW, fp, cp.max_tasks + cp.B.NP);
                if (anti && (fp.P.key.valid || fp.P.key_f64))
                    launch_filter_nullkeys(L, KW, ps.CW, fp, stride_grid(ps.rel->n));
            }
        });
        return join_assemble(st, js, e, root_res);
    }

    Rel outer_join(Rel& left, Rel& right, const JoinSpec& js, const JoinKind& K, Result* root_res) {
        Rel&           opt = js.build_left ? left : right;
        Rel&           pre = js.build_left ? right : left;
        const uint64_t oattr = js.build_left ? js.left_attr : js.right_attr;
        if (oattr < opt.cols.size() && opt.cols[oattr].type == RJ_VARCHAR)
            throw_fmt(RJ_ERR_UNSUPPORTED, "%s on a VARCHAR key", K.name);
        if (pre.n == 0) return empty_rel(js, root_res);
        JoinState st;
        join_prepare(left, right, js, root_res != nullptr, st, K);
        return outer_probe(st, js, root_res);
    }

    Rel full_join(Rel& left, Rel& right, const JoinSpec& js_in, const JoinKind& K, Result* root_res) {
        for (int side = 0; side < 2; ++side) {
            const Rel&     r = side == 0 ? left : right;
            const uint64_t a = side == 0 ? js_in.left_attr : js_in.right_attr;
            if (a < r.cols.size() && r.cols[a].type == RJ_VARCHAR)
                throw_fmt(RJ_ERR_UNSUPPORTED, "%s on a VARCHAR key", K.name);
        }
        if (left.n == 0 && right.n == 0) {
            JoinState chk;
            join_prepare(left, right, js_in, root_res != nullptr, chk, K);
            refuse_varchar_outputs(chk);
            return empty_rel(js_in, root_res);
        }
        JoinSpec js = js_in;
        if ((js.build_left ? right : left).n == 0) js.build_left = !js.build_left;
        JoinState st;
        join_prepare(left, right, js, root_res != nullptr, st, K);
        return outer_probe(st, js, root_res);
    }

    static void refuse_varchar_outputs(JoinState& st) {
        for (Side* s : {&st.ls, &st.rs})
            for (int c : s->need) {
                if (!s->optional || s->rel->cols[c].type != RJ_VARCHAR) continue;
                if (st.kind->probe_optional)
                    throw_fmt(RJ_ERR_UNSUPPORTED,
                              "full outer join: a VARCHAR column in the output is not supported (%s child column %d)",
                              s == &st.ls ? "left" : "right", c);
                throw_fmt(RJ_ERR_UNSUPPORTED,
                          "outer join: a VARCHAR column of the optional side in the output is not supported "
                          "(child column %d)", c);
            }
    }

    Rel outer_probe(JoinState& st, const JoinSpec& js, Result* root_res) {
        const bool full = st.kind->probe_optional;
        Side&      bs = st.bs();
        Side&      ps = st.ps();
        const int  KW = st.KW;
        refuse_varchar_outputs(st);
        prepare_wide(bs);
        prepare_wide(ps);
        plan_carry_streams(st);
        const bool     bcast = broadcast_form(st, js);
        const uint32_t bits = join_bits(js, bs.rel->n);
        if (ctx->tune.diag >= 2)
            fprintf(stderr, "[rj diag] %s %s=%llu %s=%llu %s bits=%u cw=%d/%d\n", st.kind->name, full ? "built" : "optional",
                    (unsigned long long)bs.rel->n, full ? "probed" : "preserved", (unsigned long long)ps.rel->n,
                    bcast ? "broadcast" : "partitioned", bits, bs.CW, ps.CW);

        FullParams   fp{};
        OuterParams& op = fp.o;
        op.keyless = st.type_mismatch ? 1 : 0;
        op.pad_bc = bs.carry_mode == CARRY_ROWIDX ? OUTER_NO_ROW : 0u;
        op.P = make_src(st, ps, js);
        if (full || !op.keyless) op.B = make_src(st, bs, js);
        BufP counters = zeroed_counters();
        op.out_cursor = counters->as<unsigned long long>();
        CoParts cp;
        if (!bcast) {
            cp = co_partition(st, js, bits, counters);
            set_parts(op, cp, counters, bits);
        }
        BufP flags;
        if (full) {
            fp.pad_pc = ps.carry_mode == CARRY_ROWIDX ? OUTER_NO_ROW : 0u;
            const uint64_t flag_bytes = ((bcast ? (uint64_t)JN_RMAX : cp.B.n_tuples) / 32 + 2) * 4;
            flags = ctx->buf(flag_bytes);
            RJ_HIP(hipMemsetAsync(flags->p, 0, flag_bytes, ctx->stream));
            fp.flags = flags->as<uint32_t>();
            fp.use_flags = bcast ? 1 : 0;
        }
        const uint32_t probe_grid = stride_grid(ps.rel->n), build_grid = stride_grid(bs.rel->n);
        const uint64_t rows0 = std::max(st.cap_hint, full ? bs.rel->n + ps.rel->n : ps.rel->n);
        Emitted e = emit_with_retry(st, counters, first_cap(rows0), [&](const OutStream& key, uint64_t cap) {
            op.key = key;
// ... 1170 lines not shown
```

radix-join_amd/csrc/rj_internal.hpp:

```cpp
#pragma once
#include <hip/hip_runtime.h>

#include <atomic>
#include <cstdarg>
#include <cstdio>
#include <cstring>
#include <functional>
#include <map>
#include <memory>
#include <mutex>
#include <stdexcept>
#include <string>
#include <vector>

#include "../../include/rj.h"
#include "rj_comm.hpp"
#include "rj_device.hpp"
#include "rj_kernels.hpp"

namespace rj {

struct Context;

struct Error : std::runtime_error {
// ... 7 lines not shown
    va_start(ap, fmt);
    vsnprintf(buf, sizeof buf, fmt, ap);
    va_end(ap);
    throw Error(code, buf);
}

#define RJ_HIP(expr)                                                                          \
    do {                                                                                      \
        hipError_t _e = (expr);                                                               \
        if (_e != hipSuccess)                                                                 \
            ::rj::throw_fmt(_e == hipErrorOutOfMemory ? RJ_ERR_NOMEM : RJ_ERR_DEVICE,         \
                            "%s failed: %s (%s:%d)", #expr, hipGetErrorString(_e), __FILE__, \
                            __LINE__);                                                        \
    } while (0)

class DevPool {
   public:
    void* alloc(size_t bytes);
    void  release(void* p);
    void     set_poison(Context* owner, int mode) { owner_ = owner, poison_ = mode; }
    int      poison() const { return poison_; }
    uint64_t n_fills() const { return n_fill_.load(std::memory_order_relaxed); }
    uint64_t bytes_filled() const { return fill_bytes_.load(std::memory_order_relaxed); }
    void  trim();
    ~DevPool();
    size_t bytes_in_use() const { return in_use_; }
    size_t bytes_cached() const { return cached_; }
    uint64_t n_malloc = 0, n_trim = 0;
    double   malloc_ms = 0;

   private:
    struct Block {
        void*  p;
        size_t size;
        bool   free;
    };
    std::vector<Block> blocks_;
    size_t             in_use_ = 0, cached_ = 0;
    Context*           owner_ = nullptr;
    int                poison_ = 0;
    std::atomic<uint64_t> n_fill_{0}, fill_bytes_{0};
    hipError_t         fill(void* p, size_t bytes);
};

struct Buf {
    Context* ctx = nullptr;
    void*    p = nullptr;
    size_t   bytes = 0;
    Buf(Context* c, size_t n);
    ~Buf();
    Buf(const Buf&) = delete;
    Buf& operator=(const Buf&) = delete;
    template <class T>
    T* as() const {
        return reinterpret_cast<T*>(p);
    }
};
using BufP = std::shared_ptr<Buf>;

class Profiler {
   public:
    bool        on = false;
    int         level = 1;
    hipStream_t stream = nullptr;
    bool        timed(const char* name, hipEvent_t* start, hipEvent_t* stop);
    void        drain();
    void        reset();
    struct Tot {
        uint64_t launches = 0;
        double   ms = 0;
    };
    std::map<std::string, Tot> totals;
    std::vector<std::string>   order;
    ~Profiler();

   private:
    struct Rec {
        const char* name;
        hipEvent_t  a, b;
    };
    std::vector<Rec>        open_;
    std::vector<hipEvent_t> spare_;
    hipEvent_t              get_event();
};

class LaunchLog {
   public:
    bool on = false;
    void add(const void* kernel);
    void clear();
    void merge_into(std::map<std::string, uint64_t>& out);

   private:
    std::mutex                         mu_;
    std::map<const void*, uint64_t>    counts_;
    std::map<const void*, std::string> names_;
};

struct TableColumn {
    int32_t  type = 0;
    uint64_t n_pages = 0;
    const uint8_t* dev_pages = nullptr;
    BufP           owned;
    bool           regular = false;
    uint64_t       page_rows_total = 0;
    BufP           page_rows;
    std::vector<uint32_t> page_rows_host;
    std::vector<uint8_t>        host_pages;
    std::vector<const uint8_t*> vc_pages;
    mutable BufP vc_dev, vc_dev_dir;
    bool                        skipped = false;
};

struct Table {
    Context*                 ctx = nullptr;
    uint64_t                 num_rows = 0;
    std::vector<TableColumn> cols;
};

struct ResultColumn {
    int32_t              type = 0;
    uint64_t             n_pages = 0;
    BufP                 dev_pages;
    std::vector<uint8_t> host_pages;
    struct Part {
        Context* ctx;
        BufP     pages;
        uint64_t n_pages;
    };
    std::vector<Part> more;
    uint64_t          n_first = 0;
};

struct Result {
    Context*                  ctx = nullptr;
    uint64_t                  num_rows = 0;
    std::vector<ResultColumn> cols;
};

struct Tuning {
    int blocked_mid = 1;
    int mall_chunk = 0;
    int radix_bits = 0;
    int p1_bits = 0;
    int fine = 1;
    int pack = 1;
    int aos3 = 1;
    int aos_mid = 2;
    int tpg1 = 0;
    int packed_side = 0;
    int tpg2 = 0;
    int xcd_min_rows = 40 << 20;
    int xcd_split = 1;
    int bcast = 1;
    int diag = 0;
    int varchar_dev_rows = 200000;
    int vkey_hash_bits = 0;
    int sync_upload = 0;
    int wide_carry = 1;
    int fold_owner = 1;
    int exchange_timeout_ms = 120000;
    int bringup_timeout_ms = 0;
    int debug_shard_fail = 0, debug_shard_fail_rank = 0;
    int debug_poison = 0;
    void from_env();
};

struct Context {
    Tuning      tune;
    int         device = 0;
    hipStream_t stream = nullptr;
    bool        own_stream = false;
    int         radix_bits_override = 0;
    DevPool     pool;
    Profiler    prof;
    LaunchLog   klog;
    std::string last_error;
    void*  pinned = nullptr;
    size_t pinned_bytes = 0;
    static constexpr size_t SMALL_PINNED = 32768;
    void*  pinned_small = nullptr;
    void*  small_pinned();
    hipStream_t copy_stream = nullptr;
    void*       pinned_up = nullptr;
    size_t      pinned_up_bytes = 0;
    hipStream_t upload_stream();
    hipStream_t aux = nullptr;
    hipStream_t aux_stream();
    void*       upload_staging(size_t bytes);
    Launch launch() {
        Launch L;
        L.stream = stream;
        L.self = this;
        L.timed = prof.on ? [](void* s, const char* n, hipEvent_t* a, hipEvent_t* b) {
            return static_cast<Context*>(s)->prof.timed(n, a, b);
        } : (bool (*)(void*, const char*, hipEvent_t*, hipEvent_t*)) nullptr;
        L.logged = klog.on ? [](void* s, const void* k) { static_cast<Context*>(s)->klog.add(k); }
                           : (void (*)(void*, const void*)) nullptr;
        return L;
    }
    std::vector<Context*>  peers;
    std::unique_ptr<Comm>  comm;
    Context*               group = nullptr;
    int                    n_lanes() const { return 1 + (int)peers.size(); }
    Context*               lane(int i) { return i == 0 ? this : peers[(size_t)i - 1]; }
    int   n_cu = 0;
    int   compute_units();
    void  prewarm();
    BufP  buf(size_t bytes) { return std::make_shared<Buf>(this, bytes ? bytes : 16); }
    void* staging(size_t bytes);
    void  sync() { RJ_HIP(hipStreamSynchronize(stream)); }
    ~Context();
};

struct TableFetch {
    virtual Table* get(uint64_t id) = 0;
    virtual ~TableFetch() = default;
};

Result* execute_plan(Context* ctx, const rj_plan* plan, Table* const* tables, uint64_t n_tables,
                     int flags, TableFetch* fetch = nullptr);
Result* join_tuples(Context* ctx, const rj_tuples* build, const rj_tuples* probe,
                    uint32_t skip_rank_bits, int flags);
void    execute_sharded(Context* group, const rj_plan* plan, Table* const* tables, uint64_t n_inputs,
                        int flags, Result** out);
bool    plan_shardable(const rj_plan* plan, std::string* why);
void    shard_partition(Context* ctx, const Table* t, uint64_t key_col, uint64_t carry_col,
                        uint32_t n_ranks, rj_tuples* out, uint64_t* counts);

Table* table_upload(Context* ctx, const rj_input* host, const std::vector<bool>* col_used = nullptr,
                    bool borrow_varchar = false);
class AsyncUpload : public TableFetch {
   public:
    AsyncUpload(Context* ctx, const rj_plan* plan, const std::vector<bool>& used,
                const std::vector<std::vector<bool>>& col_used);
    ~AsyncUpload() override;
    Table* get(uint64_t id) override;
    double busy_ms() const { return busy_ms_; }
    double wait_ms() const { return wait_ms_; }

   private:
    struct Impl;
    std::unique_ptr<Impl> im_;
    double                busy_ms_ = 0, wait_ms_ = 0;
};
Table* table_adopt(Context* ctx, uint64_t num_rows, uint64_t n_cols, const int32_t* types,
                   const void* const* dev_pages, const uint64_t* n_pages);
void   result_copy_pages(Result* r, uint64_t col, void* const* dst, uint64_t n_dst);
void   upload_host_pages(Context* ctx, const uint8_t* const* pages, uint64_t n_pages, uint8_t* dev);
Result* execute_host_sharded(Context* group, const rj_plan* plan, const std::vector<bool>& used,
                             const std::vector<std::vector<bool>>& col_used);

Table*   table_from_csv(Context* ctx, const char* text, uint64_t n_bytes, uint64_t n_cols, const int32_t* col_type,
                        const rj_filter_op* filter, uint64_t n_filter_ops);
int parse_fp64_host(const char* s, uint64_t n, uint64_t* bits);
uint64_t table_col_pages(const Table* t, uint64_t col);
void     table_copy_pages(Context* ctx, const Table* t, uint64_t col, void* const* dst, uint64_t n_dst);

void parallel_for(size_t n, size_t grain, const std::function<void(size_t, size_t)>& fn);

void copy_page(void* dst, const void* src);
void copy_pages_fence();

void varchar_dir_build(const uint8_t* const* pages, uint64_t n_pages, uint64_t num_rows,
                       std::vector<uint64_t>& row_base);
void varchar_gather_encode(const uint8_t* const* pages, uint64_t n_pages,
                           const std::vector<uint64_t>& row_base, const uint32_t* idx, uint64_t n,
                           std::vector<uint8_t>& out_pages, uint64_t& n_out_pages);

}

struct rj_context : rj::Context {};
struct rj_table : rj::Table {};
struct rj_result : rj::Result {};
```

radix-join_amd/csrc/rj_kernels.hip:

```cpp
#include <hip/hip_ext.h>

#include "rj_kernels.hpp"

#include <algorithm>
#include <type_traits>

namespace rj {

__device__ __forceinline__ uint32_t fmix32(uint32_t h) {
    h ^= h >> 16;
    h *= 0x85ebca6bu;
    h ^= h >> 13;
    h *= 0xc2b2ae35u;
    h ^= h >> 16;
    return h;
}
__device__ __forceinline__ uint32_t unfmix32(uint32_t h) {
    h ^= h >> 16;
    h *= 0x7ed1b41du;
    h ^= (h >> 13) ^ (h >> 26);
    h *= 0xa5cb9243u;
    h ^= h >> 16;
    return h;
}
// ... 703 lines not shown
        ok = drop_invalid(base + PT_TILE <= end, base, end, ok);
        return hash_keys(ok, lo, hi);
    }
    template <int NW>
    __device__ __forceinline__ uint32_t issue_tile(uint32_t base, uint32_t end,
                                                   uint32_t (&w)[PT_ITEMS][NW]) const {
        static_assert(NW == KW + CW, "word count");
        const bool vec = base + PT_TILE <= end;
        uint32_t   lo[PT_ITEMS], hi[PT_ITEMS];
        uint32_t   ok = raw_keys(vec, base, end, lo, hi);
        if constexpr (WIDE == WIDE_32S) {
            uint32_t c0[PT_ITEMS];
            load_col32_any(s.carry, vec, base, end, c0);
#pragma unroll
            for (int j = 0; j < PT_ITEMS; ++j) w[j][KW] = c0[j];
            load_col32_any(s.carry2, vec, base, end, c0);
#pragma unroll
            for (int j = 0; j < PT_ITEMS; ++j) w[j][KW + 1] = c0[j];
            if constexpr (CW == 3) {
                load_col32_any(s.carry3, vec, base, end, c0);
#pragma unroll
                for (int j = 0; j < PT_ITEMS; ++j) w[j][KW + 2] = c0[j];
            }
        } else if constexpr (WIDE == WIDE_64_32) {
            uint32_t c0[PT_ITEMS], c1[PT_ITEMS];
            load_col64(s.carry, vec, base, end, c0, c1);
#pragma unroll
            for (int j = 0; j < PT_ITEMS; ++j) {
                w[j][KW] = c0[j];
                w[j][KW + 1] = c1[j];
            }
            load_col32_any(s.carry2, vec, base, end, c0);
#pragma unroll
            for (int j = 0; j < PT_ITEMS; ++j) w[j][KW + 2] = c0[j];
        } else if constexpr (CW >= 1) {
            if (s.carry_mode == CARRY_ROWIDX) {
#pragma unroll
                for (int j = 0; j < PT_ITEMS; ++j) w[j][KW] = item_row(vec, base, j);
            } else if constexpr (CW == 1) {
                uint32_t c0[PT_ITEMS];
                load_col32(s.carry, vec, base, end, c0);
#pragma unroll
                for (int j = 0; j < PT_ITEMS; ++j) w[j][KW] = c0[j];
            } else {
                uint32_t c0[PT_ITEMS], c1[PT_ITEMS];
                load_col64(s.carry, vec, base, end, c0, c1);
#pragma unroll
                for (int j = 0; j < PT_ITEMS; ++j) {
                    w[j][KW] = c0[j];
                    w[j][KW + 1] = c1[j];
                }
            }
        }
#pragma unroll
        for (int j = 0; j < PT_ITEMS; ++j) {
            w[j][0] = lo[j];
            if constexpr (KW == 2) w[j][1] = hi[j];
        }
        return ok;
    }
    template <int NW>
    __device__ __forceinline__ uint32_t finish_tile(uint32_t base, uint32_t end, uint32_t ok,
                                                    uint32_t (&w)[PT_ITEMS][NW]) const {
        const bool vec = base + PT_TILE <= end;
        uint32_t   lo[PT_ITEMS], hi[PT_ITEMS];
#pragma unroll
        for (int j = 0; j < PT_ITEMS; ++j) {
            lo[j] = w[j][0];
            hi[j] = KW == 2 ? w[j][KW - 1] : 0u;
        }
        ok = drop_invalid(vec, base, end, ok);
        ok = hash_keys(ok, lo, hi);
#pragma unroll
        for (int j = 0; j < PT_ITEMS; ++j) {
            w[j][0] = lo[j];
            if constexpr (KW == 2) w[j][1] = hi[j];
        }
        return ok;
    }
    template <int NW>
    __device__ __forceinline__ uint32_t load_tile(uint32_t base, uint32_t end,
                                                  uint32_t (&w)[PT_ITEMS][NW]) const {
        return finish_tile<NW>(base, end, issue_tile<NW>(base, end, w), w);
    }
};

__device__ __forceinline__ bool group_range(const PassParams& pp, uint32_t g, uint32_t& seg,
                                            uint32_t& begin, uint32_t& end) {
    const uint32_t gt = pp.tiles_per_group * (uint32_t)PT_TILE;
    if (pp.seg_off == nullptr) {
        seg = 0;
        uint64_t b = (uint64_t)g * gt;
        if (b >= pp.n) return false;
        begin = (uint32_t)b;
        end = (uint32_t)min((uint64_t)pp.n, b + gt);
        return true;
    }
    const uint32_t G = pp.grp_start[pp.nseg] - pp.grp_base;
    if (pp.xcd_remap) {
        const uint32_t per = (G + 7u) >> 3;
        if ((g >> 3) >= per) return false;
        g = (g & 7u) * per + (g >> 3);
    }
    if (g >= G) return false;
    uint32_t lo = 0, hi = pp.nseg;
    while (hi - lo > 1) {
        uint32_t mid = (lo + hi) >> 1;
        if (pp.grp_start[mid] - pp.grp_base <= g)
            lo = mid;
        else
            hi = mid;
    }
    seg = lo >> pp.oseg_shift;
    uint32_t gi = g - (pp.grp_start[lo] - pp.grp_base);
    uint64_t b = (uint64_t)pp.seg_off[lo] + (uint64_t)gi * gt;
    begin = (uint32_t)b;
    end = (uint32_t)min((uint64_t)(pp.seg_end ? pp.seg_end[lo] : pp.seg_off[lo + 1]), b + gt);
    return begin < end;
}

template <class L, class = void>
struct loader_needs_begin : std::false_type {};
template <class L>
struct loader_needs_begin<L, std::enable_if_t<L::kNeedsBegin>> : std::true_type {};

template <class Loader>
__global__ __launch_bounds__(PT_THREADS) void k_pass_hist(Loader ld, PassParams pp) {
    __shared__ uint32_t s_h[PT_MAXF];
    uint32_t            seg, begin, end;
    if (!group_range(pp, blockIdx.x, seg, begin, end)) return;
    const uint32_t F = 1u << pp.fanout_log2, mask = F - 1u;
    for (uint32_t d = threadIdx.x; d < F; d += PT_THREADS) s_h[d] = 0;
    lds_barrier();
    for (uint32_t base = begin; base < end; base += PT_TILE) {
        uint32_t hk[PT_ITEMS];
        uint32_t ok;
        if constexpr (loader_needs_begin<Loader>::value)
            ok = ld.key_tile(base, begin, end, hk);
        else
            ok = ld.key_tile(base, end, hk);
#pragma unroll
        for (int j = 0; j < PT_ITEMS; ++j) {
            if ((ok >> j) & 1u) atomicAdd(&s_h[pass_digit(pp, hk[j], mask)], 1u);
        }
    }
    if constexpr (loader_needs_begin<Loader>::value) {
        uint32_t hx;
        if (ld.extra(begin, end, hx)) atomicAdd(&s_h[pass_digit(pp, hx, mask)], 1u);
    }
    lds_barrier();
    for (uint32_t d = threadIdx.x; d < F; d += PT_THREADS) {
        uint32_t c = s_h[d];
        if (c) atomicAdd(&pp.hist[(((size_t)seg * F + d) << pp.xcd_log2) | (blockIdx.x & ((1u << pp.xcd_log2) - 1u))], c);
    }
}

template <class Loader>
__global__ __launch_bounds__(PT_THREADS) void k_fine_hist(Loader ld, uint32_t n, uint32_t shift,
                                                          uint32_t b1, uint32_t b2,
                                                          uint32_t* fine, uint32_t xcd_tpg,
                                                          uint32_t* coarse_x) {
    __shared__ uint32_t s_f[1u << PT_FINEBITS];
    const uint32_t      NB = 1u << (b1 + b2), m1 = (1u << b1) - 1u, m2 = (1u << b2) - 1u;
    for (uint32_t d = threadIdx.x; d < NB; d += PT_THREADS) s_f[d] = 0;
    lds_barrier();
    const uint32_t tiles = (uint32_t)(((uint64_t)n + PT_TILE - 1) / PT_TILE);
    const uint32_t x = blockIdx.x & 7u, gstride = gridDim.x >> 3;
    uint32_t       gk = blockIdx.x >> 3, gj = 0;
    auto           tile_of = [&](uint32_t k, uint32_t j) { return (x + 8u * k) * xcd_tpg + j; };
    auto           advance = [&](uint32_t t) -> uint32_t {
        if (!xcd_tpg) return t + gridDim.x;
        if (++gj < xcd_tpg && tile_of(gk, gj) < tiles) return tile_of(gk, gj);
        gk += gstride;
        gj = 0;
        const uint64_t nt = (uint64_t)(x + 8ull * gk) * xcd_tpg;
        return nt < tiles ? (uint32_t)nt : 0xffffffffu;
    };
    uint32_t t = xcd_tpg ? tile_of(gk, 0) : blockIdx.x;
    uint32_t lo[PT_ITEMS], hi[PT_ITEMS], raw = 0;
    if (t < tiles) raw = ld.issue_keys(t * (uint32_t)PT_TILE, n, lo, hi);
    while (t < tiles) {
        const uint32_t ok = ld.finish_keys(t * (uint32_t)PT_TILE, n, raw, lo, hi);
        uint32_t       q[PT_ITEMS];
#pragma unroll
        for (int j = 0; j < PT_ITEMS; ++j) {
            const uint32_t h = lo[j] >> shift;
            q[j] = ((h & m1) << b2) | ((h >> b1) & m2);
        }
        const uint32_t t2 = advance(t);
        if (t2 < tiles) raw = ld.issue_keys(t2 * (uint32_t)PT_TILE, n, lo, hi);
#pragma unroll
        for (int j = 0; j < PT_ITEMS; ++j)
            if ((ok >> j) & 1u) atomicAdd(&s_f[q[j]], 1u);
        t = t2;
    }
    lds_barrier();
    for (uint32_t d = threadIdx.x; d < NB; d += PT_THREADS) {
        uint32_t c = s_f[d];
        if (c) atomicAdd(&fine[d], c);
    }
    if (xcd_tpg) {
        const uint32_t F2 = 1u << b2;
        for (uint32_t d1 = threadIdx.x; d1 <= m1; d1 += PT_THREADS) {
            uint32_t sum = 0;
            for (uint32_t i = 0; i < F2; ++i) sum += s_f[d1 * F2 + ((i + d1) & m2)];
            if (sum) atomicAdd(&coarse_x[(d1 << 3) | x], sum);
        }
    }
}

__global__ __launch_bounds__(PT_MAXF) void k_scan_fine(const uint32_t* fine, uint32_t F1,
                                                       uint32_t F2, uint32_t* off2,
                                                       uint32_t* cursor2, uint32_t* off1,
                                                       uint32_t* cursor1, const uint32_t* coarse_x) {
    __shared__ uint32_t s_wsum[PT_MAXF / 64];
    const uint32_t      d1 = blockIdx.x, below = d1 * F2;
    uint32_t            sum = 0;
    if ((F2 & 3u) == 0) {
        const uint4* f4 = reinterpret_cast<const uint4*>(fine);
        for (uint32_t i = threadIdx.x; i < below / 4; i += PT_MAXF) {
            const uint4 v = f4[i];
            sum += v.x + v.y + v.z + v.w;
        }
    } else {
        for (uint32_t i = threadIdx.x; i < below; i += PT_MAXF) sum += fine[i];
    }
    uint32_t base, tot;
    (void)block_excl_scan(sum, s_wsum, base);
    lds_barrier();
    const uint32_t v = threadIdx.x < F2 ? fine[below + threadIdx.x] : 0u;
    const uint32_t ex = block_excl_scan(v, s_wsum, tot);
    if (threadIdx.x < F2) {
        off2[below + threadIdx.x] = base + ex;
        cursor2[below + threadIdx.x] = base + ex;
    }
    if (threadIdx.x == 0) {
        off1[d1] = base;
        if (coarse_x) {
            uint32_t at = base;
            for (uint32_t x = 0; x < 8; ++x) {
                cursor1[(d1 << 3) | x] = at;
                at += coarse_x[(d1 << 3) | x];
            }
        } else {
            cursor1[d1] = base;
        }
        if (d1 + 1 == F1) {
            off1[F1] = base + tot;
            off2[(size_t)F1 * F2] = base + tot;
        }
    }
}

template <int NW, class Loader, int PAIR, bool AOS>
__global__ __launch_bounds__(PT_THREADS) void k_pass_scatter(Loader ld, PassParams pp, Words out) {
    static_assert(PAIR < 0 || (PAIR >= 1 && PAIR + 1 < NW), "pair = two carry words behind the key");
    static_assert(!AOS || (NW == 3 && PAIR == 1), "12-byte tuples: one key word + a two-word carry");
    __shared__ uint2    s_stage2[PT_TILE];
    uint32_t* const     s_stage = reinterpret_cast<uint32_t*>(s_stage2);
    __shared__ uint32_t s_cnt[PT_MAXF];
    __shared__ uint32_t s_base[PT_MAXF];
    __shared__ uint32_t s_delta[PT_MAXF];
    __shared__ uint32_t s_wsum[PT_THREADS / 64];
    uint32_t            seg, begin, end;
    if (!group_range(pp, blockIdx.x, seg, begin, end)) return;
    const uint32_t F = 1u << pp.fanout_log2, mask = F - 1u;

    uint32_t run = 0;
    uint32_t w[PT_ITEMS][NW];

    for (uint32_t base = begin; base < end; base += PT_TILE) {
        for (uint32_t d = threadIdx.x; d < F; d += PT_THREADS) s_cnt[d] = 0;
        lds_barrier();

        uint32_t dr[PT_ITEMS];
        const uint32_t ok = ld.template load_tile<NW>(base, end, w);
#pragma unroll
        for (int j = 0; j < PT_ITEMS; ++j) {
            dr[j] = 0xffffffffu;
            if ((ok >> j) & 1u) {
                uint32_t d = pass_digit(pp, w[j][0], mask);
                uint32_t r = atomicAdd(&s_cnt[d], 1u);
                dr[j] = (d << 16) | r;
            }
        }
        lds_barrier();

        uint32_t c = threadIdx.x < F ? s_cnt[threadIdx.x] : 0u;
        if (c) {
            run = atomicAdd(&pp.cursor[(((size_t)seg * F + threadIdx.x) << pp.xcd_log2) |
                                       (blockIdx.x & ((1u << pp.xcd_log2) - 1u))], c);
        }
        uint32_t total;
        uint32_t ex = block_excl_scan(c, s_wsum, total);
        if (threadIdx.x < F) s_base[threadIdx.x] = ex;
        lds_barrier();

#pragma unroll
        for (int j = 0; j < PT_ITEMS; ++j)
            if (dr[j] != 0xffffffffu) dr[j] = s_base[dr[j] >> 16] + (dr[j] & 0xffffu);

        if constexpr (NW == 3 && PAIR == 1) {
            constexpr uint32_t HALF = PT_TILE / 2;
            uint2* const       s_p = s_stage2;
            uint32_t* const    s_k = reinterpret_cast<uint32_t*>(s_stage2 + HALF);
            if (threadIdx.x < F) s_delta[threadIdx.x] = run - ex;
#pragma unroll
            for (int h = 0; h < 2; ++h) {
#pragma unroll
                for (int j = 0; j < PT_ITEMS; ++j) {
                    const uint32_t lp = dr[j] - h * HALF;
                    if (lp < HALF) {
                        s_k[lp] = w[j][0];
                        s_p[lp] = make_uint2(w[j][1], w[j][2]);
                    }
                }
                lds_barrier();
#pragma unroll
                for (int k = 0; k < PT_ITEMS / 2; ++k) {
                    const uint32_t i = k * PT_THREADS + threadIdx.x, gi = h * HALF + i;
                    if (gi < total) {
                        const uint32_t v = s_k[i];
                        const uint2    c = s_p[i];
                        const uint32_t g = s_delta[pass_digit(pp, v, mask)] + gi;
                        if constexpr (AOS) {
                            uint32_t* o = out.w[0] + (size_t)g * 3u;
                            o[0] = v;
                            o[1] = c.x;
                            o[2] = c.y;
                            if (pp.side_out) pp.side_out[g] = (uint16_t)((v >> pp.next_shift) & pp.next_mask);
                        } else {
                            out.w[0][g] = v;
                            reinterpret_cast<uint2*>(out.w[1])[g] = c;
                        }
                    }
                }
                lds_barrier();
            }
            continue;
        }
#pragma unroll
        for (int j = 0; j < PT_ITEMS; ++j)
            if (dr[j] != 0xffffffffu) s_stage[dr[j]] = w[j][0];
        if (threadIdx.x < F) s_delta[threadIdx.x] = run - ex;
        lds_barrier();
        uint32_t dest[PT_ITEMS];
#pragma unroll
        for (int k = 0; k < PT_ITEMS; ++k) {
            const uint32_t i = k * PT_THREADS + threadIdx.x;
            dest[k] = 0;
            if (i < total) {
                const uint32_t v = s_stage[i];
                dest[k] = s_delta[pass_digit(pp, v, mask)] + i;
                out.w[0][dest[k]] = v;
            }
        }
        lds_barrier();
#pragma unroll
        for (int a = 1; a < NW; ++a) {
            if constexpr (PAIR >= 0) {
                if (a == PAIR + 1) continue;
                if (a == PAIR) {
#pragma unroll
                    for (int j = 0; j < PT_ITEMS; ++j)
                        if (dr[j] != 0xffffffffu)
                            s_stage2[dr[j]] = make_uint2(w[j][a], w[j][a + 1 < NW ? a + 1 : a]);
                    lds_barrier();
                    uint2* dst2 = reinterpret_cast<uint2*>(out.w[a]);
#pragma unroll
                    for (int k = 0; k < PT_ITEMS; ++k) {
                        const uint32_t i = k * PT_THREADS + threadIdx.x;
                        if (i < total) dst2[dest[k]] = s_stage2[i];
                    }
                    lds_barrier();
                    continue;
                }
            }
#pragma unroll
            for (int j = 0; j < PT_ITEMS; ++j)
                if (dr[j] != 0xffffffffu) s_stage[dr[j]] = w[j][a];
            lds_barrier();
            uint32_t* dst = out.w[a];
#pragma unroll
            for (int k = 0; k < PT_ITEMS; ++k) {
                const uint32_t i = k * PT_THREADS + threadIdx.x;
                if (i < total) dst[dest[k]] = s_stage[i];
            }
            lds_barrier();
        }
    }
}

template <class Loader, bool BLK_OUT = false>
__global__ __launch_bounds__(PT_THREADS) void k_pass_scatter_packed(Loader ld, PassParams pp, uint2* out) {
    __shared__ uint2    s_stage[PT_TILE];
    __shared__ uint32_t s_cnt[PT_MAXF];
    __shared__ uint32_t s_base[PT_MAXF];
    __shared__ uint32_t s_delta[PT_MAXF];
    __shared__ uint32_t s_wsum[PT_THREADS / 64];
    uint32_t            seg, begin, end;
    if (!group_range(pp, blockIdx.x, seg, begin, end)) return;
    const uint32_t F = 1u << pp.fanout_log2, mask = F - 1u;

    uint32_t run = 0;
    uint32_t w[PT_ITEMS][2];
    uint32_t ok_raw = ld.template issue_tile<2>(begin, end, w);
    for (uint32_t base = begin; base < end; base += PT_TILE) {
        for (uint32_t d = threadIdx.x; d < F; d += PT_THREADS) s_cnt[d] = 0;
        lds_barrier();

        uint32_t       dr[PT_ITEMS];
        const uint32_t ok = ld.template finish_tile<2>(base, end, ok_raw, w);
#pragma unroll
        for (int j = 0; j < PT_ITEMS; ++j) {
            dr[j] = 0xffffffffu;
            if ((ok >> j) & 1u) {
                uint32_t d = pass_digit(pp, w[j][0], mask);
                uint32_t r = atomicAdd(&s_cnt[d], 1u);
                dr[j] = (d << 16) | r;
            }
        }
        lds_barrier();

        uint32_t c = threadIdx.x < F ? s_cnt[threadIdx.x] : 0u;
        if (c)
            run = atomicAdd(&pp.cursor[(((size_t)seg * F + threadIdx.x) << pp.xcd_log2) |
                                       (blockIdx.x & ((1u << pp.xcd_log2) - 1u))], c);
        uint32_t total;
        uint32_t ex = block_excl_scan(c, s_wsum, total);
        if (threadIdx.x < F) s_base[threadIdx.x] = ex;
        lds_barrier();

#pragma unroll
        for (int j = 0; j < PT_ITEMS; ++j)
            if (dr[j] != 0xffffffffu)
                s_stage[s_base[dr[j] >> 16] + (dr[j] & 0xffffu)] = make_uint2(w[j][0], w[j][1]);
        if (base + PT_TILE < end) ok_raw = ld.template issue_tile<2>(base + PT_TILE, end, w);
        if (threadIdx.x < F) s_delta[threadIdx.x] = run - ex;
        lds_barrier();

#pragma unroll
        for (int k = 0; k < PT_ITEMS; ++k) {
            const uint32_t i = k * PT_THREADS + threadIdx.x;
            if (i < total) {
                const uint2    v = s_stage[i];
                const uint32_t g = s_delta[pass_digit(pp, v.x, mask)] + i;
                if constexpr (BLK_OUT) {
                    uint32_t* o = reinterpret_cast<uint32_t*>(out) + BlockedLoader::key_at(g);
                    o[0] = v.x;
                    o[BlockedLoader::BLK] = v.y;
                } else {
                    out[g] = v;
                }
                if (pp.side_out) pp.side_out[g] = (uint16_t)((v.x >> pp.next_shift) & pp.next_mask);
            }
        }
    }
}

__global__ void k_heavy_tasks(const uint32_t* offR, const uint32_t* offS, uint32_t NP,
                              uint32_t* tasks, uint32_t* n_heavy, uint32_t max_tasks) {
    uint32_t q = blockIdx.x * blockDim.x + threadIdx.x;
    if (q >= NP) return;
    uint32_t sb = offS[q], se = offS[q + 1];
    uint32_t len = se - sb;
    if (len <= JN_HEAVY || offR[q + 1] == offR[q]) return;
    uint32_t nt = (len + JN_HEAVY - 1) / JN_HEAVY;
    uint32_t b = atomicAdd(n_heavy, nt);
    for (uint32_t t = 0; t < nt; ++t) {
        uint32_t k = b + t;
        if (k >= max_tasks) break;
        tasks[3 * k + 0] = q;
        tasks[3 * k + 1] = (uint32_t)((uint64_t)sb + (uint64_t)t * JN_HEAVY);
        tasks[3 * k + 2] = (uint32_t)min((uint64_t)se, (uint64_t)sb + (uint64_t)(t + 1) * JN_HEAVY);
    }
}

template <int KW, int CW>
__device__ __forceinline__ void part_tuple(const Words& W, int pack, int aos, uint32_t idx, uint32_t (&t)[KW + CW]) {
    constexpr int NW = KW + CW;
    if constexpr (KW == 1 && CW == 2) {
        if (aos) {
            const uint32_t* p = W.w[0] + (size_t)idx * 3u;
            t[0] = p[0];
            t[1] = p[1];
            t[2] = p[2];
            return;
        }
    }
    if constexpr (KW == 1 && CW == 1) {
        if (pack) {
            const uint2 v = reinterpret_cast<const uint2*>(W.w[0])[idx];
            t[0] = v.x;
            t[1] = v.y;
            return;
        }
    }
    constexpr int NA = CW >= 2 ? NW - 2 : NW;
#pragma unroll
    for (int a = 0; a < NA; ++a) t[a] = W.w[a][idx];
    if constexpr (CW >= 2) {
        const uint2 v = reinterpret_cast<const uint2*>(W.w[NA])[idx];
        t[NA] = v.x;
        t[NA + 1] = v.y;
    }
}

template <int KW, int CW>
__device__ __forceinline__ void tuple_carry(const uint32_t (&t)[KW + CW], uint32_t& c0, uint32_t& c1, uint32_t& c2) {
    constexpr int W = KW + CW;
    c0 = CW >= 1 ? t[KW < W ? KW : 0] : 0u;
    c1 = CW >= 2 ? t[KW + 1 < W ? KW + 1 : 0] : 0u;
    c2 = CW == 3 ? t[W - 1] : 0u;
}

template <int KW>
__device__ __forceinline__ void unhash_key(uint32_t lo, uint32_t hi, uint32_t& k0, uint32_t& k1) {
    if constexpr (KW == 1) {
        k0 = unfmix32(lo);
    } else {
        const uint64_t k64 = unfmix64((uint64_t)lo | ((uint64_t)hi << 32));
        k0 = (uint32_t)k64;
        k1 = (uint32_t)(k64 >> 32);
    }
}

enum { OM_GENERIC = 0, OM_PAGED32 = 1, OM_DENSE32 = 2, OM_P32_64_64 = 3 };

#define RJ_STAMP(PHASE)                                                         \
    do {                                                                        \
        if (jp.diag) {                                                          \
            unsigned long long _t = __builtin_amdgcn_s_memtime();               \
            if (threadIdx.x == 0) atomicAdd(&jp.diag[PHASE], _t - diag_t);      \
            diag_t = _t;                                                        \
        }                                                                       \
    } while (0)

template <int KW, int CWR, int CWS, int OM, int PK, int TG>
__global__ __launch_bounds__(jn_threads(TG ? 2 : KW + CWR), jn_min_waves(TG ? 2 : KW + CWR)) void k_join(JoinParams jp) {
    static_assert(!TG || (KW == 1 && CWR == 2), "tagged table: one key word + two-word build carry");
    constexpr int      TH = jn_threads(TG ? 2 : KW + CWR);
    constexpr int      RPT = (JN_RMAX + TH - 1) / TH;
    constexpr int      SPT = JN_SUB / TH;
    constexpr int      SUB = JN_SUB;
    static_assert(RPT % 4 == 0 && SPT % 4 == 0, "tuples are loaded as 16-byte vectors");
    constexpr int      RW = KW + CWR;
    constexpr int      SW = KW + CWS;
    __shared__ __attribute__((aligned(16))) uint32_t t_w[TG ? 1 : RW][JN_CAP];
    __shared__ __attribute__((aligned(16))) uint2    t_c2[TG ? JN_RMAX : 1];
    __shared__ __attribute__((aligned(16))) uint32_t t_cnt[JN_CAP / 4];
    __shared__ uint32_t s_wtot[TH / 64];
    __shared__ unsigned long long s_obase;

    const uint32_t     lane = threadIdx.x & 63u, wid = threadIdx.x >> 6;
    constexpr uint32_t SMASK = JN_CAP - 1;
    constexpr uint32_t BMASK = JN_CAP / 4 - 1;

    constexpr int PPW = jn_ppw(TG ? 2 : KW + CWR);
    struct Task {
        uint32_t q, rbeg, rend, sbeg, send;
        bool     active;
    };
    const bool     heavy_wg = blockIdx.x < jp.heavy_grid;
    const uint32_t wg = heavy_wg ? blockIdx.x : blockIdx.x - jp.heavy_grid;
    auto get_task = [&](uint32_t k) {
        Task t{0, 0, 0, 0, 0, false};
        if (heavy_wg) {
            if (k == 0 && wg < *jp.n_heavy) {
                t.q = jp.heavy_tasks[3 * wg + 0];
                t.sbeg = jp.heavy_tasks[3 * wg + 1];
                t.send = jp.heavy_tasks[3 * wg + 2];
                t.rbeg = jp.offR[t.q];
                t.rend = jp.offR[t.q + 1];
                t.active = t.rbeg < t.rend && t.sbeg < t.send;
            }
            return t;
        }
        t.q = wg * PPW + k;
        if (k < (uint32_t)PPW && t.q < jp.NP) {
            t.rbeg = jp.offR[t.q];
            t.rend = jp.offR[t.q + 1];
            t.sbeg = jp.offS[t.q];
            t.send = jp.offS[t.q + 1];
            t.active = t.rbeg < t.rend && t.sbeg < t.send && t.send - t.sbeg <= JN_HEAVY;
        }
        return t;
    };

    uint32_t rw[RPT][RW];
    uint32_t sw[SPT][SW];
    auto item_index = [&](int j, bool packed) -> uint32_t {
        return packed ? ((j / 2) * TH + threadIdx.x) * 2 + (j % 2)
                      : ((j / 4) * TH + threadIdx.x) * 4 + (j % 4);
    };
    constexpr bool packR = (PK & 1) != 0, packS = (PK & 2) != 0;
    constexpr bool aosR = (PK & 4) != 0, aosS = (PK & 8) != 0;
    static_assert(!aosR || (KW == 1 && CWR == 2), "12-byte build tuples: key + two-word carry");
    static_assert(!aosS || (KW == 1 && CWS == 2), "12-byte probe tuples: key + two-word carry");
    auto load_aos3 = [&](const uint32_t* base, uint32_t n, auto& regs, auto n_items) {
        constexpr int NI = decltype(n_items)::value;
#pragma unroll
        for (int v = 0; v < NI / 4; ++v) {
            const uint32_t  i0 = (v * TH + threadIdx.x) * 4;
            const uint32_t* p = base + (size_t)i0 * 3;
            if (i0 + 3 < n) {
                const u32x4a x = *reinterpret_cast<const u32x4a*>(p), y = *reinterpret_cast<const u32x4a*>(p + 4),
                             z = *reinterpret_cast<const u32x4a*>(p + 8);
                regs[4 * v + 0][0] = x[0];
                regs[4 * v + 0][1] = x[1];
                regs[4 * v + 0][2] = x[2];
                regs[4 * v + 1][0] = x[3];
// ... 1655 lines not shown
template <int KW = 1, int CW = 0, class F>
static void for_shape(const char* name, int kw, int cw, F&& f) {
    if constexpr (KW > 2) {
        launch_failed(name, "no kernel for this key/carry word count", true);
    } else {
        if constexpr (KW + CW <= MAX_WORDS)
            if (kw == KW && cw == CW) return f(int_c<KW>{}, int_c<CW>{});
        for_shape<(CW < 3 ? KW : KW + 1), (CW < 3 ? CW + 1 : 0)>(name, kw, cw, f);
    }
}

template <class F>
static void for_shape2(const char* name, int kw, int cwa, int cwb, F&& f) {
    for_shape(name, kw, cwa, [&](auto KW, auto CWA) {
        for_shape(name, kw, cwb, [&](auto KW2, auto CWB) {
            if constexpr (decltype(KW2)::value == decltype(KW)::value) f(KW, CWA, CWB);
        });
    });
}

void launch_page_headers(const Launch& L, const uint8_t* pages, uint32_t n_pages, uint32_t rows_full,
                         uint32_t* page_rows, unsigned long long* flags) {
    if (!n_pages) return;
    RJ_KLAUNCH(L, "page_headers", k_page_headers, std::min<uint32_t>((n_pages + 3) / 4, 8192u), 256, pages, n_pages,
               rows_full, page_rows, flags);
}

void launch_rows_beyond(const Launch& L, const uint8_t* pages, uint32_t n_pages,
                        const uint32_t* row_base, uint64_t num_rows, unsigned long long* flag) {
    if (!n_pages) return;
    RJ_KLAUNCH(L, "rows_beyond", k_rows_beyond, (n_pages + 3) / 4, 256, pages, n_pages, row_base,
               num_rows, flag);
}

void launch_decode_pages(const Launch& L, const uint8_t* pages, uint32_t n_pages, int width,
                         const uint32_t* row_base, uint64_t num_rows, uint8_t* values,
                         uint8_t* valid) {
    if (!n_pages) return;
    if (width == 4)
        RJ_KLAUNCH(L, "decode_pages", (k_decode_pages<4>), n_pages, 256, pages, row_base, num_rows,
                   values, valid);
    else
        RJ_KLAUNCH(L, "decode_pages", (k_decode_pages<8>), n_pages, 256, pages, row_base, num_rows,
                   values, valid);
}

void launch_scan_bins(const Launch& L, const uint32_t* in, uint32_t n, uint32_t* off,
                      uint32_t* cursor) {
    RJ_KLAUNCH(L, "scan_bins", (k_scan_bins<0>), 1, 1024, in, (const uint32_t*)nullptr, n, 1u, off, cursor);
}

void launch_scan_segments(const Launch& L, const uint32_t* hist, const uint32_t* seg_off,
                          uint32_t nseg, uint32_t F, uint32_t xcd_log2, uint32_t* off, uint32_t* cursor) {
    RJ_KLAUNCH(L, "scan_segments", k_scan_segments, nseg, PT_MAXF, hist, seg_off, nseg, F, xcd_log2, off,
               cursor);
}

void launch_group_table(const Launch& L, const uint32_t* seg_off, uint32_t nseg,
                        uint32_t group_tuples, uint32_t* grp_start, const uint32_t* seg_end) {
    RJ_KLAUNCH(L, "group_table", (k_scan_bins<1>), 1, 1024, seg_off, seg_end, nseg, group_tuples, grp_start,
               (uint32_t*)nullptr);
}

void launch_pass_hist_src(const Launch& L, const TupleSrc& src, int key_words, const PassParams& pp,
                          uint32_t n_groups) {
    if (!n_groups) return;
    if (key_words == 1) {
        SrcLoader<1, 0> ld{src};
        RJ_KLAUNCH(L, "pass1_hist", (k_pass_hist<SrcLoader<1, 0>>), n_groups, PT_THREADS, ld, pp);
    } else {
        SrcLoader<2, 0> ld{src};
        RJ_KLAUNCH(L, "pass1_hist", (k_pass_hist<SrcLoader<2, 0>>), n_groups, PT_THREADS, ld, pp);
    }
}

void launch_fine_hist_src(const Launch& L, const TupleSrc& src, int key_words, uint32_t shift,
                          uint32_t b1, uint32_t b2, uint32_t grid, uint32_t* fine, uint32_t xcd_tpg,
                          uint32_t* coarse_x) {
    if (!grid || !src.n_rows) return;
    if (key_words == 1) {
        SrcLoader<1, 0> ld{src};
        RJ_KLAUNCH(L, "pass1_hist", (k_fine_hist<SrcLoader<1, 0>>), grid, PT_THREADS, ld, src.n_rows,
                   shift, b1, b2, fine, xcd_tpg, coarse_x);
    } else {
        SrcLoader<2, 0> ld{src};
        RJ_KLAUNCH(L, "pass1_hist", (k_fine_hist<SrcLoader<2, 0>>), grid, PT_THREADS, ld, src.n_rows,
                   shift, b1, b2, fine, xcd_tpg, coarse_x);
    }
}

void launch_fine_hist_words(const Launch& L, const Words& in, bool packed, uint32_t n, uint32_t shift,
                            uint32_t b1, uint32_t b2, uint32_t grid, uint32_t* fine, uint32_t xcd_tpg,
                            uint32_t* coarse_x) {
    if (!grid || !n) return;
    if (packed) {
        PackedLoader ld{reinterpret_cast<const uint2*>(in.w[0])};
        RJ_KLAUNCH(L, "pass1_hist", (k_fine_hist<PackedLoader>), grid, PT_THREADS, ld, n, shift, b1, b2, fine,
                   xcd_tpg, coarse_x);
    } else {
        DenseLoader ld{in};
        RJ_KLAUNCH(L, "pass1_hist", (k_fine_hist<DenseLoader>), grid, PT_THREADS, ld, n, shift, b1, b2, fine,
                   xcd_tpg, coarse_x);
    }
}

void launch_scan_fine(const Launch& L, const uint32_t* fine, uint32_t F1, uint32_t F2,
                      uint32_t* off2, uint32_t* cursor2, uint32_t* off1, uint32_t* cursor1,
                      const uint32_t* coarse_x) {
    RJ_KLAUNCH(L, "scan_fine", k_scan_fine, F1, PT_MAXF, fine, F1, F2, off2, cursor2, off1, cursor1,
               coarse_x);
}

template <int KW, int CW, int WIDE = WIDE_NONE>
static void scatter_src_t(const Launch& L, const TupleSrc& src, const PassParams& pp,
                          uint32_t n_groups, const Words& out) {
    SrcLoader<KW, CW, WIDE> ld{src};
    RJ_KLAUNCH(L, "pass1_scatter", (k_pass_scatter<KW + CW, SrcLoader<KW, CW, WIDE>, (CW >= 2 ? KW + CW - 2 : -1), false>),
               n_groups, PT_THREADS, ld, pp, out);
}

void launch_pass_scatter_src(const Launch& L, const TupleSrc& src, int key_words, int carry_words,
                             const PassParams& pp, uint32_t n_groups, const Words& out, bool aos3) {
    if (!n_groups) return;
    const int wide = src.carry_mode == CARRY_WIDE ? src.wide : WIDE_NONE;
    if (aos3) {
        if (key_words != 1 || carry_words != 2) launch_failed("pass1_scatter", "12-byte tuples need KW=1, CW=2", true);
        if (wide == WIDE_32S) {
            SrcLoader<1, 2, WIDE_32S> ld{src};
            RJ_KLAUNCH(L, "pass1_scatter", (k_pass_scatter<3, SrcLoader<1, 2, WIDE_32S>, 1, true>), n_groups, PT_THREADS, ld, pp, out);
            return;
        }
        SrcLoader<1, 2> ld{src};
        RJ_KLAUNCH(L, "pass1_scatter", (k_pass_scatter<3, SrcLoader<1, 2>, 1, true>), n_groups, PT_THREADS, ld, pp, out);
        return;
    }
    if (wide != WIDE_NONE) {
        switch (key_words * 100 + carry_words * 10 + wide) {
        case 121: scatter_src_t<1, 2, WIDE_32S>(L, src, pp, n_groups, out); break;
        case 131: scatter_src_t<1, 3, WIDE_32S>(L, src, pp, n_groups, out); break;
        case 132: scatter_src_t<1, 3, WIDE_64_32>(L, src, pp, n_groups, out); break;
        case 221: scatter_src_t<2, 2, WIDE_32S>(L, src, pp, n_groups, out); break;
        default: launch_failed("pass1_scatter", "no kernel for this wide carry layout", true);
        }
        return;
    }
    for_shape("pass1_scatter", key_words, carry_words, [&](auto KW, auto CW) {
        if constexpr (CW <= 2)
            scatter_src_t<KW, CW>(L, src, pp, n_groups, out);
        else
            launch_failed("pass1_scatter", "no kernel for this key/carry word count", true);
    });
}

void launch_pass_hist_dense(const Launch& L, const Words& in, const PassParams& pp,
                            uint32_t n_groups) {
    if (!n_groups) return;
    DenseLoader ld{in};
    RJ_KLAUNCH(L, "pass2_hist", (k_pass_hist<DenseLoader>), n_groups, PT_THREADS, ld, pp);
}

void launch_pass_scatter_dense(const Launch& L, const Words& in, int n_words, int pair_word,
                               const PassParams& pp, uint32_t n_groups, const Words& out, bool aos3) {
    if (!n_groups) return;
    if (aos3) {
        if (n_words != 3 || pair_word != 1) launch_failed("pass2_scatter", "12-byte tuples need KW=1, CW=2", true);
        RJ_KLAUNCH(L, "pass2_scatter", (k_pass_scatter<3, DenseLoaderT<1>, 1, true>), n_groups, PT_THREADS,
                   DenseLoaderT<1>{in}, pp, out);
        return;
    }
    switch (n_words * 10 + (pair_word < 0 ? 9 : pair_word)) {
    case 19:
        RJ_KLAUNCH(L, "pass2_scatter", (k_pass_scatter<1, DenseLoader, -1, false>), n_groups, PT_THREADS,
                   DenseLoader{in}, pp, out);
        break;
    case 29:
        RJ_KLAUNCH(L, "pass2_scatter", (k_pass_scatter<2, DenseLoader, -1, false>), n_groups, PT_THREADS,
                   DenseLoader{in}, pp, out);
        break;
    case 39:
        RJ_KLAUNCH(L, "pass2_scatter", (k_pass_scatter<3, DenseLoader, -1, false>), n_groups, PT_THREADS,
                   DenseLoader{in}, pp, out);
        break;
    case 31:
        RJ_KLAUNCH(L, "pass2_scatter", (k_pass_scatter<3, DenseLoaderT<1>, 1, false>), n_groups, PT_THREADS,
                   DenseLoaderT<1>{in}, pp, out);
        break;
    case 42:
        RJ_KLAUNCH(L, "pass2_scatter", (k_pass_scatter<4, DenseLoaderT<2>, 2, false>), n_groups, PT_THREADS,
                   DenseLoaderT<2>{in}, pp, out);
        break;
    default: launch_failed("pass2_scatter", "no kernel for this word layout", true);
    }
}

void launch_pass_hist_digits(const Launch& L, const uint16_t* digits, const PassParams& pp, uint32_t n_groups) {
    if (!n_groups) return;
    DigitLoader ld{digits, pp.shift};
    RJ_KLAUNCH(L, "pass2_hist", (k_pass_hist<DigitLoader>), n_groups, PT_THREADS, ld, pp);
}

void launch_pass_hist_aos3(const Launch& L, const uint32_t* in_tuples, const PassParams& pp, uint32_t n_groups) {
    if (!n_groups) return;
    RJ_KLAUNCH(L, "pass2_hist", (k_pass_hist<Aos3KeyLoader>), n_groups, PT_THREADS, Aos3KeyLoader{in_tuples}, pp);
}

void launch_pass_scatter_aos3(const Launch& L, const uint32_t* in_tuples, const PassParams& pp, uint32_t n_groups,
                              uint32_t* out_tuples) {
    if (!n_groups) return;
    Words out{};
    out.w[0] = out_tuples;
    RJ_KLAUNCH(L, "pass2_scatter", (k_pass_scatter<3, Aos3Loader, 1, true>), n_groups, PT_THREADS,
               Aos3Loader{in_tuples}, pp, out);
}

void launch_pass_hist_packed(const Launch& L, const uint32_t* in_pairs, const PassParams& pp,
                             uint32_t n_groups) {
    if (!n_groups) return;
    PackedLoader ld{reinterpret_cast<const uint2*>(in_pairs)};
    RJ_KLAUNCH(L, "pass2_hist", (k_pass_hist<PackedLoader>), n_groups, PT_THREADS, ld, pp);
}

void launch_pass_scatter_src_packed(const Launch& L, const TupleSrc& src, const PassParams& pp,
                                    uint32_t n_groups, uint32_t* out_pairs, bool blocked_out) {
    if (!n_groups) return;
    SrcLoader<1, 1> ld{src};
    if (blocked_out)
        RJ_KLAUNCH(L, "pass1_scatter", (k_pass_scatter_packed<SrcLoader<1, 1>, true>), n_groups, PT_THREADS, ld,
                   pp, reinterpret_cast<uint2*>(out_pairs));
    else
        RJ_KLAUNCH(L, "pass1_scatter", (k_pass_scatter_packed<SrcLoader<1, 1>>), n_groups, PT_THREADS, ld,
                   pp, reinterpret_cast<uint2*>(out_pairs));
}

void launch_pass_hist_blocked(const Launch& L, const uint32_t* in_blocked, const PassParams& pp, uint32_t n_groups) {
    if (!n_groups) return;
    RJ_KLAUNCH(L, "pass2_hist", (k_pass_hist<BlockedLoader>), n_groups, PT_THREADS, BlockedLoader{in_blocked}, pp);
}
void launch_pass_scatter_blocked(const Launch& L, const uint32_t* in_blocked, const PassParams& pp, uint32_t n_groups,
                                 uint32_t* out_pairs, bool blocked_out) {
    if (!n_groups) return;
    BlockedLoader ld{in_blocked};
    if (blocked_out)
        RJ_KLAUNCH(L, "pass2_scatter", (k_pass_scatter_packed<BlockedLoader, true>), n_groups, PT_THREADS, ld, pp,
                   reinterpret_cast<uint2*>(out_pairs));
    else
        RJ_KLAUNCH(L, "pass2_scatter", (k_pass_scatter_packed<BlockedLoader>), n_groups, PT_THREADS, ld, pp,
                   reinterpret_cast<uint2*>(out_pairs));
}

void launch_pass_scatter_packed(const Launch& L, const uint32_t* in_pairs, const PassParams& pp,
                                uint32_t n_groups, uint32_t* out_pairs) {
    if (!n_groups) return;
    PackedLoader ld{reinterpret_cast<const uint2*>(in_pairs)};
    RJ_KLAUNCH(L, "pass2_scatter", (k_pass_scatter_packed<PackedLoader>), n_groups, PT_THREADS, ld, pp,
               reinterpret_cast<uint2*>(out_pairs));
}

void launch_heavy_tasks(const Launch& L, const uint32_t* offR, const uint32_t* offS, uint32_t NP,
                        uint32_t* tasks, uint32_t* n_heavy, uint32_t max_tasks) {
    RJ_KLAUNCH(L, "heavy_tasks", k_heavy_tasks, (NP + 255) / 256, 256, offR, offS, NP, tasks,
               n_heavy, max_tasks);
}

static bool join_tagged(int key_words, int cw_build, const JoinParams& jp) {
    return key_words == 1 && cw_build == 2 && jp.radix_bits >= 14 && jp.radix_bits <= 31;
}

template <int KW, int CWR, int CWS, int PK>
static void join_pk(const Launch& L, const JoinParams& jp, uint32_t grid) {
    const char* name = "join_build_probe";
    if constexpr (KW == 1 && CWR == 2 && (PK & 1) == 0) {
        const bool p366 = CWS == 2 && jp.key.mode == ST_PAGED32 && jp.bc.mode == ST_PAGED64 &&
                          jp.pc.mode == ST_PAGED64;
        if (join_tagged(KW, CWR, jp)) {
            if constexpr (CWS == 2) {
                if (p366) {
                    RJ_KLAUNCH(L, name, (k_join<KW, CWR, CWS, OM_P32_64_64, PK, 1>), grid, jn_threads(2), jp);
                    return;
                }
            }
            RJ_KLAUNCH(L, name, (k_join<KW, CWR, CWS, OM_GENERIC, PK, 1>), grid, jn_threads(2), jp);
            return;
        }
        if constexpr (CWS == 2) {
            if (p366) {
                RJ_KLAUNCH(L, name, (k_join<KW, CWR, CWS, OM_P32_64_64, PK, 0>), grid, jn_threads(KW + CWR), jp);
                return;
            }
        }
    }
    int om = OM_GENERIC;
    if (KW == 1 && CWR <= 1 && CWS <= 1) {
        auto all = [&](int mode) {
            return jp.key.mode == mode && (CWR == 0 || jp.bc.mode == mode) &&
                   (CWS == 0 || jp.pc.mode == mode);
        };
        if (all(ST_PAGED32)) om = OM_PAGED32;
        if (all(ST_DENSE32)) om = OM_DENSE32;
    }
    if constexpr (KW == 1 && CWR <= 1 && CWS <= 1) {
        if (om == OM_PAGED32) {
            RJ_KLAUNCH(L, name, (k_join<KW, CWR, CWS, OM_PAGED32, PK, 0>), grid, jn_threads(KW + CWR), jp);
            return;
        }
        if (om == OM_DENSE32) {
            RJ_KLAUNCH(L, name, (k_join<KW, CWR, CWS, OM_DENSE32, PK, 0>), grid, jn_threads(KW + CWR), jp);
// ... 224 lines not shown
```

radix-join_amd/csrc/rj_kernels.hpp:

```cpp
#pragma once
#include <hip/hip_runtime.h>

#include "rj_device.hpp"

namespace rj {

struct Launch {
    hipStream_t stream;
    bool (*timed)(void* self, const char* name, hipEvent_t* start, hipEvent_t* stop);
    void* self;
    void (*logged)(void* self, const void* kernel);
};

[[noreturn]] void launch_failed(const char* kernel, const char* what, bool unsupported);

void launch_page_headers(const Launch& L, const uint8_t* pages, uint32_t n_pages, uint32_t rows_full,
                         uint32_t* page_rows, unsigned long long* flags);
void launch_rows_beyond(const Launch& L, const uint8_t* pages, uint32_t n_pages,
                        const uint32_t* row_base, uint64_t num_rows, unsigned long long* flag);
void launch_decode_pages(const Launch& L, const uint8_t* pages, uint32_t n_pages, int width,
                         const uint32_t* row_base, uint64_t num_rows, uint8_t* values,
                         uint8_t* valid);

void launch_scan_bins(const Launch& L, const uint32_t* in, uint32_t n, uint32_t* off,
                      uint32_t* cursor);
void launch_scan_segments(const Launch& L, const uint32_t* hist, const uint32_t* seg_off,
                          uint32_t nseg, uint32_t F, uint32_t xcd_log2, uint32_t* off, uint32_t* cursor);
void launch_group_table(const Launch& L, const uint32_t* seg_off, uint32_t nseg,
                        uint32_t group_tuples, uint32_t* grp_start, const uint32_t* seg_end = nullptr);

void launch_pass_hist_src(const Launch& L, const TupleSrc& src, int key_words, const PassParams& pp,
                          uint32_t n_groups);
void launch_fine_hist_src(const Launch& L, const TupleSrc& src, int key_words, uint32_t shift,
                          uint32_t b1, uint32_t b2, uint32_t grid, uint32_t* fine, uint32_t xcd_tpg = 0,
                          uint32_t* coarse_x = nullptr);
void launch_fine_hist_words(const Launch& L, const Words& in, bool packed, uint32_t n, uint32_t shift,
                            uint32_t b1, uint32_t b2, uint32_t grid, uint32_t* fine, uint32_t xcd_tpg = 0,
                            uint32_t* coarse_x = nullptr);
void launch_scan_fine(const Launch& L, const uint32_t* fine, uint32_t F1, uint32_t F2,
                      uint32_t* off2, uint32_t* cursor2, uint32_t* off1, uint32_t* cursor1,
                      const uint32_t* coarse_x = nullptr);
void launch_pass_scatter_src(const Launch& L, const TupleSrc& src, int key_words, int carry_words,
                             const PassParams& pp, uint32_t n_groups, const Words& out, bool aos3 = false);
void launch_pass_hist_dense(const Launch& L, const Words& in, const PassParams& pp,
                            uint32_t n_groups);
void launch_pass_scatter_dense(const Launch& L, const Words& in, int n_words, int pair_word,
                               const PassParams& pp, uint32_t n_groups, const Words& out, bool aos3 = false);

void launch_pass_hist_digits(const Launch& L, const uint16_t* digits, const PassParams& pp, uint32_t n_groups);
void launch_pass_hist_aos3(const Launch& L, const uint32_t* in_tuples, const PassParams& pp, uint32_t n_groups);
void launch_pass_scatter_aos3(const Launch& L, const uint32_t* in_tuples, const PassParams& pp, uint32_t n_groups,
                              uint32_t* out_tuples);

void launch_pass_hist_packed(const Launch& L, const uint32_t* in_pairs, const PassParams& pp,
                             uint32_t n_groups);
void launch_pass_scatter_src_packed(const Launch& L, const TupleSrc& src, const PassParams& pp,
                                    uint32_t n_groups, uint32_t* out_pairs, bool blocked_out = false);
void launch_pass_hist_blocked(const Launch& L, const uint32_t* in_blocked, const PassParams& pp, uint32_t n_groups);
void launch_pass_scatter_blocked(const Launch& L, const uint32_t* in_blocked, const PassParams& pp, uint32_t n_groups,
                                 uint32_t* out_pairs, bool blocked_out);
void launch_pass_scatter_packed(const Launch& L, const uint32_t* in_pairs, const PassParams& pp,
                                uint32_t n_groups, uint32_t* out_pairs);

void launch_heavy_tasks(const Launch& L, const uint32_t* offR, const uint32_t* offS, uint32_t NP,
                        uint32_t* tasks, uint32_t* n_heavy, uint32_t max_tasks);
uint32_t join_partitions_per_workgroup(int key_words, int cw_build, const JoinParams& jp);
void launch_join(const Launch& L, int key_words, int cw_build, int cw_probe, const JoinParams& jp,
                 uint32_t grid);

void launch_join_bcast(const Launch& L, int key_words, int cw_build, int cw_probe,
                       const BcastParams& bp, uint32_t grid);

void launch_filter_bcast(const Launch& L, int key_words, int cw_preserved, const FilterParams& fp, uint32_t grid);
void launch_filter_join(const Launch& L, int key_words, int cw_preserved, const FilterParams& fp, uint32_t grid);
void launch_filter_nullkeys(const Launch& L, int key_words, int cw_preserved, const FilterParams& fp, uint32_t grid);

void launch_outer_bcast(const Launch& L, int key_words, int cw_optional, int cw_preserved, const OuterParams& op,
                        uint32_t grid);
void launch_outer_join(const Launch& L, int key_words, int cw_optional, int cw_preserved, const OuterParams& op,
                       uint32_t grid);
void launch_outer_nullkeys(const Launch& L, int key_words, int cw_preserved, const OuterParams& op, uint32_t grid);
void launch_outer_gather(const Launch& L, const ColRef& src, const uint32_t* idx, uint64_t n, uint8_t* dst,
                         uint8_t* dst_valid);

void launch_full_bcast(const Launch& L, int key_words, int cw_optional, int cw_preserved, const FullParams& fp,
                       uint32_t grid);
void launch_full_join(const Launch& L, int key_words, int cw_optional, int cw_preserved, const FullParams& fp,
                      uint32_t grid);
void launch_full_unmatched(const Launch& L, int key_words, int cw_built, const FullParams& fp, uint32_t grid);
void launch_full_buildrows(const Launch& L, int key_words, int cw_built, const FullParams& fp, uint32_t grid);

void launch_agg_merge_init(const Launch& L, const AggParams& ap, uint32_t grid);
void launch_agg_parts(const Launch& L, int key_words, int carry_words, const AggParams& ap, uint32_t grid);
void launch_agg_nullkey(const Launch& L, int carry_words, const AggParams& ap, uint32_t grid);
void launch_agg_emit(const Launch& L, int key_words, const AggParams& ap, uint32_t grid);
void launch_agg_column(const Launch& L, const unsigned long long* src, const unsigned long long* nn, uint64_t n, int width,
                       uint8_t* dst, uint8_t* dst_valid);

void launch_gather(const Launch& L, const ColRef& src, const uint32_t* idx, uint64_t n,
                   const OutStream& dst, uint8_t* dst_valid);
void launch_debug_stall(const Launch& L, uint32_t ms);
void launch_pack_validity(const Launch& L, const uint8_t* v0, const uint8_t* v1, const uint8_t* v2, uint32_t n,
                          uint32_t* out);
void launch_split_records(const Launch& L, const SplitParams& sp, uint64_t n);
void launch_finish_pages(const Launch& L, uint8_t* pages, uint64_t n_rows, int width);
void launch_finish_streams(const Launch& L, uint8_t* const* pages, const int* widths, uint32_t n,
                           const unsigned long long* n_rows_dev, uint64_t cap_rows);
void launch_encode_nullable(const Launch& L, const uint8_t* values, const uint8_t* valid,
                            uint64_t n_rows, int width, uint8_t* pages);

void launch_vc_resolve(const Launch& L, const uint8_t* pages, uint32_t n_pages, const uint32_t* row_base,
                       const uint32_t* rowids, uint32_t n, VcRow* out);
void launch_vc_hash(const Launch& L, const uint8_t* pages, uint32_t n_pages, const uint32_t* row_base,
                    const uint32_t* rowids, uint32_t n, VcRow* rows, uint64_t* hash, uint8_t* valid,
                    uint64_t hash_mask = ~0ull);
void launch_vc_verify(const Launch& L, const uint8_t* pages_b, uint32_t np_b, const VcRow* rows_b,
                      const uint8_t* pages_p, uint32_t np_p, const VcRow* rows_p, const uint32_t* bidx,
                      const uint32_t* pidx, uint32_t n, uint8_t* keep, unsigned long long* n_bad);
void launch_vc_compact(const Launch& L, const uint8_t* keep, const uint32_t* bidx, const uint32_t* pidx, uint32_t n,
                       uint32_t* out_b, uint32_t* out_p, unsigned long long* cursor);
void prewarm_varchar_dev(const Launch& L, uint32_t* zeroed);
void launch_vc_walk(const Launch& L, const VcRow* rows, uint32_t n, uint32_t* pages_in_chunk,
                    const uint32_t* page_base, VcPage* page_out);
void launch_vc_encode(const Launch& L, const uint8_t* pages, uint32_t n_pages, const VcRow* rows,
                      const VcPage* plist, uint32_t n_out_pages, uint8_t* out);

}
```

radix-join_amd/pyrj/capi.py:

```python
from __future__ import annotations

import ctypes as C
import os

import numpy as np

from . import pages as pg
from . import plan as pl

PKG_DIR = os.path.dirname(os.path.dirname(os.path.abspath(__file__)))
LIB_PATH = os.path.join(PKG_DIR, "librj.so")

RJ_EXEC_KEEP_ON_DEVICE = 1


class rj_comm_id(C.Structure):
    _fields_ = [("bytes", C.c_char * 128)]


class rj_config(C.Structure):
    _fields_ = [
        ("device", C.c_int32),
        ("profile", C.c_int32),
        ("stream", C.c_void_p),
        ("radix_bits", C.c_int32),
        ("n_devices", C.c_int32),
        ("devices", C.POINTER(C.c_int32)),
        ("world_size", C.c_int32),
        ("rank_base", C.c_int32),
        ("comm_id", C.POINTER(rj_comm_id)),
        ("exchange", C.c_int32),
        ("flags", C.c_int32),
    ]


EXCHANGE_AUTO, EXCHANGE_P2P, EXCHANGE_RCCL = 0, 1, 2
CTX_PREWARM = 1


class rj_tuples(C.Structure):
    _fields_ = [
        ("n", C.c_uint64),
        ("key", C.c_void_p),
        ("carry", C.c_void_p),
        ("hashed", C.c_uint32),
        ("reserved", C.c_uint32),
    ]


class rj_filter_op(C.Structure):
    _fields_ = [("op", C.c_int32), ("column", C.c_int32), ("ivalue", C.c_int64), ("bytes", C.c_void_p)]


F_OPS = {"EQ": 0, "NEQ": 1, "LT": 2, "GT": 3, "LEQ": 4, "GEQ": 5, "IS_NULL": 6, "IS_NOT_NULL": 7, "BITMAP": 8, "AND": 9, "OR": 10, "NOT": 11, "LIKE": 12, "NOT_LIKE": 13}


def filter_to_c(prog):
    prog = list(prog or [])
    arr = (rj_filter_op * max(1, len(prog)))()
    keep = []
    for k, term in enumerate(prog):
        op = F_OPS[term[0]]
        arr[k].op = op
        if (op <= 5 or op >= 12) and isinstance(term[2], (bytes, bytearray)):
            lit = np.frombuffer(bytes(term[2]) or b"\0", dtype=np.uint8).copy()
            keep.append(lit)
            arr[k].column, arr[k].ivalue, arr[k].bytes = int(term[1]), len(term[2]), lit.ctypes.data
        elif op <= 5 and isinstance(term[2], float):
            arr[k].column, arr[k].ivalue = int(term[1]), int(np.array([term[2]], dtype=np.float64).view(np.int64)[0])
        elif op <= 5:
            arr[k].column, arr[k].ivalue = int(term[1]), int(term[2])
        elif op in (6, 7):
            arr[k].column = int(term[1])
        elif op == 8:
            bm = np.ascontiguousarray(term[1], dtype=np.uint8)
            keep.append(bm)
            arr[k].bytes = bm.ctypes.data
    return arr, len(prog), keep


class rj_kernel_stat(C.Structure):
    _fields_ = [("name", C.c_char * 48), ("launches", C.c_uint64), ("total_ms", C.c_double)]


class rj_device_info(C.Structure):
    _fields_ = [
        ("name", C.c_char * 128),
        ("arch", C.c_char * 64),
        ("compute_units", C.c_int32),
        ("wavefront", C.c_int32),
        ("hbm_bytes", C.c_uint64),
        ("lds_per_cu", C.c_uint64),
        ("device_count", C.c_int32),
        ("reserved", C.c_int32),
    ]


EXPORTS = [
    "rj_abi_version",
    "rj_context_create",
    "rj_context_destroy",
    "rj_last_error",
    "rj_context_n_devices",
    "rj_context_device",
    "rj_comm_id_create",
    "rj_execute_sharded",
    "rj_plan_shardable",
    "rj_table_upload",
    "rj_table_adopt_device",
    "rj_table_release",
    "rj_table_from_csv",
    "rj_debug_parse_fp64",
    "rj_table_num_rows",
    "rj_table_col_pages",
    "rj_table_copy_pages",
    "rj_execute",
    "rj_execute_resident",
    "rj_result_num_rows",
    "rj_result_num_cols",
    "rj_result_col_type",
    "rj_result_col_pages",
    "rj_result_copy_pages",
    "rj_result_device_pages",
    "rj_result_free",
    "rj_exchange_plan",
    "rj_shard_partition",
    "rj_join_tuples",
    "rj_profile_read",
    "rj_profile_reset",
    "rj_debug_launch_log",
    "rj_debug_launch_read",
    "rj_debug_pool",
    "rj_device_query",
]

_LIB = None


class RjError(RuntimeError):
    def __init__(self, code, msg):
        super().__init__(f"librj error {code}: {msg}")
        self.code = code
        self.message = msg


def _preload_torch_hip_runtime():
    import importlib.util

    try:
        spec = importlib.util.find_spec("torch")
    except Exception:
        spec = None
    if spec is None or not spec.submodule_search_locations:
        return
    libdir = os.path.join(list(spec.submodule_search_locations)[0], "lib")
    path = os.path.join(libdir, "libamdhip64.so")
    if os.path.exists(path):
        C.CDLL(path, mode=C.RTLD_GLOBAL)


def preload_torch_rccl():
    import importlib.util

    try:
        spec = importlib.util.find_spec("torch")
    except Exception:
        spec = None
    if spec is None or not spec.submodule_search_locations:
        return
    path = os.path.join(list(spec.submodule_search_locations)[0], "lib", "librccl.so")
    if os.path.exists(path):
        C.CDLL(path, mode=C.RTLD_GLOBAL)


def load():
    global _LIB
    if _LIB is not None:
        return _LIB
    lib_path = os.environ.get("RJ_LIB_PATH", LIB_PATH)
    if not os.path.exists(lib_path):
        raise RuntimeError(
            f"{lib_path} is missing: build the HIP extension first (python -c 'import __graft_entry__ as g; g.build()'). "
            "There is no CPU fallback."
        )
    _preload_torch_hip_runtime()
    L = C.CDLL(lib_path)
    vp, u64, i32 = C.c_void_p, C.c_uint64, C.c_int32
    L.rj_abi_version.restype = C.c_int
    L.rj_context_create.argtypes = [C.POINTER(vp), C.POINTER(rj_config)]
    L.rj_context_create.restype = C.c_int
    L.rj_context_destroy.argtypes = [vp]
    L.rj_context_destroy.restype = None
    L.rj_last_error.argtypes = [vp]
    L.rj_last_error.restype = C.c_char_p
    L.rj_context_n_devices.argtypes = [vp]
    L.rj_context_n_devices.restype = C.c_uint32
    L.rj_context_device.argtypes = [vp, C.c_uint32]
    L.rj_context_device.restype = vp
    L.rj_comm_id_create.argtypes = [C.POINTER(rj_comm_id)]
    L.rj_comm_id_create.restype = C.c_int
    L.rj_execute_sharded.argtypes = [vp, C.POINTER(pl.rj_plan), C.POINTER(vp), u64, i32, C.POINTER(vp)]
    L.rj_execute_sharded.restype = C.c_int
    L.rj_plan_shardable.argtypes = [C.POINTER(pl.rj_plan), C.c_char_p, C.c_size_t]
    L.rj_plan_shardable.restype = C.c_int
    L.rj_table_upload.argtypes = [vp, C.POINTER(pl.rj_input), C.POINTER(vp)]
    L.rj_table_upload.restype = C.c_int
    L.rj_table_adopt_device.argtypes = [vp, u64, u64, C.POINTER(i32), C.POINTER(vp), C.POINTER(u64), C.POINTER(vp)]
    L.rj_table_adopt_device.restype = C.c_int
    L.rj_table_release.argtypes = [vp, vp]
    L.rj_table_release.restype = None
    L.rj_table_num_rows.argtypes = [vp]
    L.rj_table_num_rows.restype = u64
    L.rj_execute.argtypes = [vp, C.POINTER(pl.rj_plan), C.POINTER(vp)]
    L.rj_execute.restype = C.c_int
    L.rj_execute_resident.argtypes = [vp, C.POINTER(pl.rj_plan), C.POINTER(vp), u64, i32, C.POINTER(vp)]
    L.rj_execute_resident.restype = C.c_int
    L.rj_result_num_rows.argtypes = [vp]
    L.rj_result_num_rows.restype = u64
    L.rj_result_num_cols.argtypes = [vp]
    L.rj_result_num_cols.restype = u64
    L.rj_result_col_type.argtypes = [vp, u64]
    L.rj_result_col_type.restype = i32
    L.rj_result_col_pages.argtypes = [vp, u64]
    L.rj_result_col_pages.restype = u64
    L.rj_result_copy_pages.argtypes = [vp, u64, C.POINTER(vp), u64]
    L.rj_result_copy_pages.restype = C.c_int
    L.rj_result_device_pages.argtypes = [vp, u64]
    L.rj_result_device_pages.restype = vp
    L.rj_result_free.argtypes = [vp]
    L.rj_result_free.restype = None
    L.rj_shard_partition.argtypes = [vp, vp, u64, u64, C.c_uint32, C.POINTER(rj_tuples), C.POINTER(u64)]
    L.rj_shard_partition.restype = C.c_int
    L.rj_join_tuples.argtypes = [vp, C.POINTER(rj_tuples), C.POINTER(rj_tuples), C.c_uint32, i32, C.POINTER(vp)]
    L.rj_join_tuples.restype = C.c_int
    L.rj_profile_read.argtypes = [vp, C.POINTER(rj_kernel_stat), u64, C.POINTER(u64)]
    L.rj_profile_read.restype = C.c_int
    L.rj_profile_reset.argtypes = [vp]
    L.rj_profile_reset.restype = None
    L.rj_debug_launch_log.argtypes = [vp, C.c_int]
    L.rj_debug_launch_log.restype = C.c_int
    L.rj_debug_launch_read.argtypes = [vp, C.c_char_p, u64, C.POINTER(u64)]
    L.rj_debug_launch_read.restype = C.c_int
    L.rj_debug_pool.argtypes = [vp, C.POINTER(u64)]
    L.rj_debug_pool.restype = C.c_int
    L.rj_device_query.argtypes = [vp, C.POINTER(rj_device_info)]
    L.rj_device_query.restype = C.c_int
    _LIB = L
    return L


class Result:

    def __init__(self, ctx: "Context", handle):
        self.ctx, self.h = ctx, handle

    @property
    def num_rows(self):
        return self.ctx.L.rj_result_num_rows(self.h)

    @property
    def num_cols(self):
        return self.ctx.L.rj_result_num_cols(self.h)

    def col_type(self, c):
        return self.ctx.L.rj_result_col_type(self.h, c)

    def col_pages(self, c):
        return self.ctx.L.rj_result_col_pages(self.h, c)

    def device_pages(self, c):
        return self.ctx.L.rj_result_device_pages(self.h, c)

    def to_table(self) -> pl.ColumnarTable:
        L = self.ctx.L
        t = pl.ColumnarTable(self.num_rows, [])
        for c in range(self.num_cols):
            n = self.col_pages(c)
            pages = np.zeros((n, pg.PAGE_SIZE), dtype=np.uint8)
            if n:
                ptrs = (C.c_void_p * n)()
                base = pages.ctypes.data
                for i in range(n):
                    ptrs[i] = base + i * pg.PAGE_SIZE
                self.ctx._check(L.rj_result_copy_pages(self.h, c, ptrs, n))
            t.columns.append(pl.Column(self.col_type(c), pages))
        return t

    def free(self):
        if self.h and getattr(self.ctx, "h", None):
            self.ctx.L.rj_result_free(self.h)
        self.h = None

    def __del__(self):
        try:
            self.free()
        except Exception:
            pass


class Table:

    def __init__(self, ctx: "Context", handle, keep=None):
        self.ctx, self.h, self.keep = ctx, handle, keep

    def release(self):
        if self.h and getattr(self.ctx, "h", None):
            self.ctx.L.rj_table_release(self.ctx.h, self.h)
        self.h = None

    def __del__(self):
        try:
            self.release()
        except Exception:
            pass


class Context:

    def __init__(self, device=-1, profile=False, stream=None, radix_bits=0, devices=None, world_size=0,
                 rank_base=0, comm_id=None, exchange=EXCHANGE_AUTO, prewarm=False, _lane_of=None, _handle=None):
        self.L = load()
        self._lanes = None
        if _lane_of is not None:
            self.h, self.group = C.c_void_p(_handle), _lane_of
            return
        self.group = None
        cfg = rj_config()
        cfg.device, cfg.profile, cfg.stream, cfg.radix_bits = device, int(profile), stream, radix_bits
        if devices is not None:
            self._devs = (C.c_int32 * len(devices))(*devices)
            cfg.n_devices, cfg.devices = len(devices), self._devs
        cfg.world_size, cfg.rank_base, cfg.exchange = world_size, rank_base, exchange
        cfg.flags = CTX_PREWARM if prewarm else 0
        if comm_id is not None or exchange == EXCHANGE_RCCL:
            preload_torch_rccl()
        if comm_id is not None:
            self._cid = rj_comm_id()
            if len(comm_id) != 128:
                raise ValueError("comm_id must be the 128 bytes of make_comm_id()")
            C.memmove(C.addressof(self._cid), bytes(comm_id), 128)
            cfg.comm_id = C.pointer(self._cid)
        h = C.c_void_p()
        rc = self.L.rj_context_create(C.byref(h), C.byref(cfg))
        if rc != 0:
            raise RjError(rc, (self.L.rj_last_error(None) or b"").decode())
        self.h = h

    @property
    def n_devices(self):
        return int(self.L.rj_context_n_devices(self.h))

    def lane(self, i) -> "Context":
        if self._lanes is None:
            self._lanes = [Context(_lane_of=self, _handle=self.L.rj_context_device(self.h, k)) for k in range(self.n_devices)]
        return self._lanes[i]

    def execute_sharded(self, plan: pl.Plan, tables_per_device):
        cached = getattr(plan, "_c_resident", None)
        if cached is None:
            cached = pl.plan_to_c(plan, with_inputs=False)
            plan._c_resident = cached
        cplan, keep = cached
        nd = self.n_devices
        n_in = len(tables_per_device[0])
        flat = [t.h for d in range(nd) for t in tables_per_device[d]]
        hs = (C.c_void_p * max(1, len(flat)))(*flat)
        outs = (C.c_void_p * nd)()
        self._check(self.L.rj_execute_sharded(self.h, C.byref(cplan), hs, n_in, RJ_EXEC_KEEP_ON_DEVICE, outs))
        return [Result(self.lane(d), C.c_void_p(outs[d])) for d in range(nd)]

    def _check(self, rc):
        if rc != 0:
            raise RjError(rc, (self.L.rj_last_error(self.h) or b"").decode())

    def destroy(self):
        if getattr(self, "group", None) is not None:
            return
        if getattr(self, "h", None):
            for ln in self._lanes or []:
                ln.h = None
            self.L.rj_context_destroy(self.h)
            self.h = None

    def upload(self, t: pl.ColumnarTable) -> Table:
        keep: list = []
        inp = pl.input_to_c(t, keep)
        h = C.c_void_p()
        self._check(self.L.rj_table_upload(self.h, C.byref(inp), C.byref(h)))
        return Table(self, h)

    def from_csv(self, text: bytes, types, filt=None) -> Table:
        n = len(types)
        ct = (C.c_int32 * n)(*types)
        ops, n_ops, keep = filter_to_c(filt)
        h = C.c_void_p()
        self.L.rj_table_from_csv.restype = C.c_int
        self.L.rj_table_from_csv.argtypes = [C.c_void_p, C.c_char_p, C.c_uint64, C.c_uint64, C.POINTER(C.c_int32), C.POINTER(rj_filter_op),
                                             C.c_uint64, C.POINTER(C.c_void_p)]
        self._check(self.L.rj_table_from_csv(self.h, text, len(text), n, ct, ops, n_ops, C.byref(h)))
        del keep
        t = Table(self, h)
        t.types = list(types)
        return t

    def table_to_host(self, t: Table, types=None) -> pl.ColumnarTable:
        types = types or t.types
        L = self.L
        L.rj_table_num_rows.restype = C.c_uint64
        L.rj_table_num_rows.argtypes = [C.c_void_p]
        L.rj_table_col_pages.restype = C.c_uint64
        L.rj_table_col_pages.argtypes = [C.c_void_p, C.c_uint64]
        L.rj_table_copy_pages.restype = C.c_int
        L.rj_table_copy_pages.argtypes = [C.c_void_p, C.c_void_p, C.c_uint64, C.POINTER(C.c_void_p), C.c_uint64]
        cols = []
        for c, ty in enumerate(types):
            npg = int(L.rj_table_col_pages(t.h, c))
            pages = np.zeros((npg, pg.PAGE_SIZE), dtype=np.uint8)
            ptrs = (C.c_void_p * max(1, npg))(*[pages[i].ctypes.data for i in range(npg)])
            self._check(L.rj_table_copy_pages(self.h, t.h, c, ptrs, npg))
            cols.append(pl.Column(ty, pages))
        return pl.ColumnarTable(int(L.rj_table_num_rows(t.h)), cols)

    def adopt_device(self, num_rows, types, dev_ptrs, n_pages, keep=None) -> Table:
        n = len(types)
        ct = (C.c_int32 * n)(*types)
        cp = (C.c_void_p * n)(*dev_ptrs)
        cn = (C.c_uint64 * n)(*n_pages)
        h = C.c_void_p()
        self._check(self.L.rj_table_adopt_device(self.h, num_rows, n, ct, cp, cn, C.byref(h)))
        return Table(self, h, keep)

    def execute(self, plan: pl.Plan) -> pl.ColumnarTable:
        cplan, keep = pl.plan_to_c(plan)
        out = C.c_void_p()
        self._check(self.L.rj_execute(self.h, C.byref(cplan), C.byref(out)))
        r = Result(self, out)
        try:
            return r.to_table()
        finally:
            r.free()
            del keep

    def execute_resident(self, plan: pl.Plan, tables, keep_on_device=True) -> Result:
        cached = getattr(plan, "_c_resident", None)
        if cached is None:
            cached = pl.plan_to_c(plan, with_inputs=False)
            plan._c_resident = cached
        cplan, keep = cached
        hs = (C.c_void_p * max(1, len(tables)))(*[t.h for t in tables])
        out = C.c_void_p()
        flags = RJ_EXEC_KEEP_ON_DEVICE if keep_on_device else 0
        self._check(self.L.rj_execute_resident(self.h, C.byref(cplan), hs, len(tables), flags, C.byref(out)))
        return Result(self, out)

    def shard_partition(self, table: Table, key_col, carry_col, n_ranks, key_ptr, carry_ptr):
        tup = rj_tuples(0, key_ptr, carry_ptr, 0, 0)
        counts = (C.c_uint64 * n_ranks)()
        self._check(self.L.rj_shard_partition(self.h, table.h, key_col, carry_col, n_ranks, C.byref(tup), counts))
        return int(tup.n), [int(c) for c in counts]

    def join_tuples(self, build, probe, skip_rank_bits=0, hashed=True) -> Result:
        build = rj_tuples(build[0], build[1], build[2], 1 if hashed else 0, 0)
        probe = rj_tuples(probe[0], probe[1], probe[2], 1 if hashed else 0, 0)
        out = C.c_void_p()
        self._check(self.L.rj_join_tuples(self.h, C.byref(build), C.byref(probe), skip_rank_bits, RJ_EXEC_KEEP_ON_DEVICE, C.byref(out)))
        return Result(self, out)

    def profile(self):
        n = C.c_uint64()
        buf = (rj_kernel_stat * 64)()
        self._check(self.L.rj_profile_read(self.h, buf, 64, C.byref(n)))
        return [
            {"name": buf[i].name.decode(), "launches": int(buf[i].launches), "total_ms": float(buf[i].total_ms)}
            for i in range(min(n.value, 64))
        ]

    def profile_reset(self):
        self.L.rj_profile_reset(self.h)

    def pool(self) -> dict:
        out = (C.c_uint64 * 4)()
        self._check(self.L.rj_debug_pool(self.h, out))
        return {"in_use": out[0], "cached": out[1], "fills": out[2], "filled_bytes": out[3]}

    def launch_log(self, on=True):
        self._check(self.L.rj_debug_launch_log(self.h, 1 if on else 0))

    def launches(self) -> dict:
        need = C.c_uint64()
        self._check(self.L.rj_debug_launch_read(self.h, None, 0, C.byref(need)))
        buf = C.create_string_buffer(need.value + 256)
        self._check(self.L.rj_debug_launch_read(self.h, buf, len(buf), C.byref(need)))
        out = {}
        for line in buf.value.decode().splitlines():
            name, n = line.rsplit(" ", 1)
            out[name] = int(n)
        return out

    def device_info(self):
        d = rj_device_info()
        self._check(self.L.rj_device_query(self.h, C.byref(d)))
        return {
            "name": d.name.decode(),
            "arch": d.arch.decode(),
            "compute_units": d.compute_units,
            "wavefront": d.wavefront,
            "hbm_bytes": int(d.hbm_bytes),
            "lds_per_cu": int(d.lds_per_cu),
            "device_count": int(d.device_count),
        }


def plan_shardable(plan: pl.Plan):
    L = load()
    cplan, keep = pl.plan_to_c(plan, with_inputs=False)
    buf = C.create_string_buffer(256)
    ok = L.rj_plan_shardable(C.byref(cplan), buf, 256)
    del keep
    return bool(ok), buf.value.decode()


def exchange_plan(world: int, subs: int, rank: int, counts) -> dict:
    L = load()
    cnt = np.ascontiguousarray(np.asarray(counts, dtype=np.uint64).reshape(world, world, subs))
    u64 = lambda n: np.zeros(n, dtype=np.uint64)
    u32 = lambda n: np.zeros(n, dtype=np.uint32)
    out = {
        "send_off": u64(world), "send_cnt": u64(world), "recv_off": u64(world), "recv_cnt": u64(world),
        "seg_begin": u32(subs * world), "seg_end": u32(subs * world), "part_off": u32(subs + 1),
    }
    n_recv = C.c_uint64(0)
    ptr = lambda a: a.ctypes.data_as(C.c_void_p)
    L.rj_exchange_plan.restype = C.c_int
    L.rj_exchange_plan.argtypes = [C.c_uint32, C.c_uint32, C.c_uint32] + [C.c_void_p] * 8 + [C.POINTER(C.c_uint64)]
    rc = L.rj_exchange_plan(world, subs, rank, ptr(cnt), ptr(out["send_off"]), ptr(out["send_cnt"]), ptr(out["recv_off"]),
                            ptr(out["recv_cnt"]), ptr(out["seg_begin"]), ptr(out["seg_end"]), ptr(out["part_off"]),
                            C.byref(n_recv))
    if rc != 0:
        L.rj_last_error.restype = C.c_char_p
        raise RjError(rc, (L.rj_last_error(None) or b"").decode())
    out["n_recv"] = int(n_recv.value)
    return out


def parse_fp64(field: bytes):
    L = load()
    L.rj_debug_parse_fp64.restype = C.c_int
    L.rj_debug_parse_fp64.argtypes = [C.c_char_p, C.c_uint64, C.POINTER(C.c_uint64)]
    bits = C.c_uint64(0)
    st = L.rj_debug_parse_fp64(field, len(field), C.byref(bits))
    return int(st), int(bits.value)


def make_comm_id() -> bytes:
    L = load()
    preload_torch_rccl()
    cid = rj_comm_id()
    rc = L.rj_comm_id_create(C.byref(cid))
    if rc != 0:
        raise RjError(rc, (L.rj_last_error(None) or b"").decode())
    return C.string_at(C.addressof(cid), 128)


def build_context(**kw):
    return Context(**kw)


def destroy_context(ctx: Context):
    ctx.destroy()


def execute(plan: pl.Plan, ctx: Context) -> pl.ColumnarTable:
    return ctx.execute(plan)
```

Baseline: 31.71 billion.

## Add skew bypass that emits hot-key probe matches during first partition pass

Samples the probe side to find heavy-hitter keys and records which of them occur exactly once on the build side. During the first radix pass the probe scatter emits join results for those keys directly and keeps them out of the partitions. The goal is to remove the load imbalance and extra partition traffic that skewed keys cause in the join phase. The cost is an extra sampling step, several small kernels, host syncs, and a fallback path that repartitions when the output capacity overflows. It runs only for probe sides of at least 40M rows.

```diff
diff --git a/include/rj.h b/include/rj.h
--- a/include/rj.h
+++ b/include/rj.h
@@ -194,6 +194,7 @@
 int  rj_debug_launch_log(rj_context* ctx, int on);
 int  rj_debug_launch_read(rj_context* ctx, char* buf, uint64_t cap, uint64_t* need);
 int  rj_debug_pool(rj_context* ctx, uint64_t out[4]);
+int  rj_debug_hot(rj_context* ctx, uint64_t out[4]);
 
 typedef struct rj_device_info {
     char     name[128];
diff --git a/radix-join_amd/csrc/rj_api.hip b/radix-join_amd/csrc/rj_api.hip
--- a/radix-join_amd/csrc/rj_api.hip
+++ b/radix-join_amd/csrc/rj_api.hip
@@ -211,6 +211,12 @@
         out[2] += p.n_fills();
         out[3] += p.bytes_filled();
     }
+    return RJ_OK;
+}
+
+int rj_debug_hot(rj_context* ctx, uint64_t out[4]) {
+    if (!ctx || !out) return RJ_ERR_ARG;
+    for (int i = 0; i < 4; ++i) out[i] = ctx->hot_debug[i];
     return RJ_OK;
 }
 
diff --git a/radix-join_amd/csrc/rj_context.hip b/radix-join_amd/csrc/rj_context.hip
--- a/radix-join_amd/csrc/rj_context.hip
+++ b/radix-join_amd/csrc/rj_context.hip
@@ -30,6 +30,9 @@
     tpg2 = env_int("RJ_TUNE_TPG2", tpg2);
     packed_side = env_int("RJ_TUNE_PACKED_SIDE", packed_side);
     xcd_min_rows = env_int("RJ_TUNE_XCD_MIN_ROWS", xcd_min_rows);
+    hot = env_int("RJ_TUNE_HOT", hot);
+    hot_min_rows = env_int("RJ_TUNE_HOT_MIN_ROWS", hot_min_rows);
+    debug_cap_hint = env_int("RJ_DEBUG_CAP_HINT", debug_cap_hint);
     bcast = env_int("RJ_TUNE_BCAST", bcast);
     diag = env_int("RJ_DIAG", diag);
     varchar_dev_rows = env_int("RJ_TUNE_VARCHAR_DEV", varchar_dev_rows);
diff --git a/radix-join_amd/csrc/rj_device.hpp b/radix-join_amd/csrc/rj_device.hpp
--- a/radix-join_amd/csrc/rj_device.hpp
+++ b/radix-join_amd/csrc/rj_device.hpp
@@ -104,6 +104,32 @@
     return (w >> pp.shift) & mask;
 }
 
+constexpr uint32_t HOT_SLOTS     = 4096;
+constexpr uint32_t HOT_MAX       = 2048;
+constexpr uint32_t HOT_SAMPLES   = 1u << 20;
+constexpr uint32_t HOT_CNT_SLOTS = 1u << 21;
+constexpr int      HOT_CNT_WALK  = 8;
+constexpr uint32_t HOT_CNT_BINS  = 1024;
+constexpr uint32_t HOT_MIN_COUNT = 4;
+struct HotCand {
+    uint32_t n;
+    uint32_t lo, hi;
+    uint32_t pad;
+};
+struct HotState {
+    uint32_t set[HOT_SLOTS];
+    HotCand  cand[HOT_SLOTS];
+    uint32_t tally[HOT_CNT_BINS];
+    uint32_t n_sel;
+    uint32_t n_set;
+    uint32_t n_hot_rows;
+    uint32_t pad;
+    unsigned long long cursor;
+};
+__host__ __device__ inline uint32_t hot_bucket(uint32_t hk) { return (hk >> 22) * 4u; }
+static_assert(HOT_SLOTS == 4096, "hot_bucket takes the top ten hash bits");
+static_assert(PT_TILE * 8 + 3 * PT_MAXF * 4 + (PT_THREADS / 64) * 4 + HOT_SLOTS * 4 + 64 <= LDS_BYTES,
+              "set image does not fit next to the scatter tile");
 #ifndef RJ_JN_THREADS
 #define RJ_JN_THREADS 512
 #endif
@@ -153,6 +179,12 @@
     uint8_t* base;
     int32_t  mode;
     int32_t  pad;
+};
+
+struct HotParams {
+    HotState* st;
+    OutStream key, bc, pc;
+    uint64_t  out_cap;
 };
 
 struct JoinParams {
diff --git a/radix-join_amd/csrc/rj_exec.hip b/radix-join_amd/csrc/rj_exec.hip
--- a/radix-join_amd/csrc/rj_exec.hip
+++ b/radix-join_amd/csrc/rj_exec.hip
@@ -308,6 +308,7 @@
         Rel             l = node(n.left, nullptr, depth + 1);
         Rel             r = node(n.right, nullptr, depth + 1);
         const JoinSpec  js = join_spec(n, ctx->radix_bits_override);
+        std::fill(std::begin(ctx->hot_debug), std::end(ctx->hot_debug), 0);
         if (n.kind == RJ_NODE_OUTER) return outer_join(l, r, js, K, root_res);
         if (n.kind == RJ_NODE_FULL) return full_join(l, r, js, K, root_res);
         if (n.kind != RJ_NODE_JOIN) return filter_join(l, r, js, K, root_res);
@@ -320,10 +321,14 @@
         return (uint32_t)std::min<uint64_t>(std::max<uint64_t>(k, 1), 8);
     }
 
+    struct HotPass {
+        HotState*        hs = nullptr;
+        const HotParams* emit = nullptr;
+    };
     Parted partition(const TupleSrc* srcp, const WordSrc* ws, int KW, int CW, uint32_t bits,
                      uint32_t shift0 = 0, bool single_pass = false, const Words* external = nullptr,
                      const std::function<void(const uint32_t*)>* after_offsets = nullptr,
-                     const PassShape* shape = nullptr) {
+                     const PassShape* shape = nullptr, const HotPass* hot = nullptr) {
         Parted P;
         const bool preseg = shape && shape->nseg > 0;
         P.NW = KW + CW;
@@ -351,6 +356,8 @@
         const bool aos_mid = P.aos3 && passes >= 2 &&
                              (ctx->tune.aos_mid == 1 || ctx->tune.aos_mid == 3 || (ctx->tune.aos_mid == 2 && fine));
         const bool mid_side = aos_mid && !fine && ctx->tune.aos_mid != 3;
+        if (hot && (fine || aos_mid || passes != 2 || ws || external || shape || KW != 1 || (CW == 1 ? !P.packed : CW != 2)))
+            throw_fmt(RJ_ERR_DEVICE, "skew bypass on a plan it does not cover");
         BufP  A[MAX_WORDS], B[MAX_WORDS], AOS, MID[2], SIDE[2];
         Words wa{}, wb{}, waos{};
         if (P.aos3) {
@@ -531,7 +538,9 @@
                     nxt = cur_is_a ? wb : wa;
                     continue;
                 }
-                if (p == 0 && !ws)
+                if (p == 0 && !ws && hot)
+                    launch_hot_pass_hist(L, src, pp, n_groups, hot->hs, hot->emit == nullptr);
+                else if (p == 0 && !ws)
                     launch_pass_hist_src(L, src, KW, pp, n_groups);
                 else if ((mid_side || packed_side) && p > 0)
                     launch_pass_hist_digits(L, SIDE[(p - 1) % 2]->as<uint16_t>(), pp, n_groups);
@@ -576,12 +585,16 @@
                     pp.next_mask = (1u << pbits[p + 1]) - 1u;
                 }
                 const bool blk_out = blocked_mid && p + 1 < passes;
-                if (p == 0 && !ws)
+                if (p == 0 && !ws && hot && hot->emit)
+                    launch_hot_pass_scatter(L, src, 1, pp, n_groups, nxt, blk_out, *hot->emit);
+                else if (p == 0 && !ws)
                     launch_pass_scatter_src_packed(L, src, pp, n_groups, nxt.w[0], blk_out);
                 else if (blocked_mid)
                     launch_pass_scatter_blocked(L, cur.w[0], pp, n_groups, nxt.w[0], blk_out);
                 else
                     launch_pass_scatter_packed(L, cur.w[0], pp, n_groups, nxt.w[0]);
+            } else if (p == 0 && !ws && hot && hot->emit) {
+                launch_hot_pass_scatter(L, src, 2, pp, n_groups, nxt, false, *hot->emit);
             } else if (p == 0 && !ws) {
                 launch_pass_scatter_src(L, src, KW, CW, pp, n_groups, nxt, P.aos3 && p + 1 == passes);
             } else {
@@ -885,6 +898,16 @@
     static OutStream out_stream(const Side& s) { return out_stream(s.stream, s.stream_mode); }
     static uint64_t first_cap(uint64_t rows) { return std::min<uint64_t>(rows + 1024, 0xfffffff0ull); }
 
+    static int key_stream_mode(const JoinState& st) {
+        return st.need_key_stream ? stream_mode_of(st.is_root, st.KW * 4, true) : ST_NONE;
+    }
+    struct HotRun {
+        BufP      state, key_stream;
+        HotParams emit{};
+        uint64_t  overflowed_rows = 0;
+        bool      overflowed = false;
+        HotState* hs() const { return state->as<HotState>(); }
+    };
     struct Emitted {
         uint64_t        nrows = 0;
         BufP            key_stream;
@@ -892,22 +915,46 @@
         std::set<void*> finished;
     };
     template <class LaunchFn>
-    Emitted emit_with_retry(JoinState& st, const BufP& counters, uint64_t cap, LaunchFn&& launch) {
+    Emitted emit_with_retry(JoinState& st, const BufP& counters, uint64_t cap, LaunchFn&& launch, HotRun* hot = nullptr) {
         const JoinKind& K = *st.kind;
         Emitted         e;
-        e.key_mode = st.need_key_stream ? stream_mode_of(st.is_root, st.KW * 4, true) : ST_NONE;
+        e.key_mode = key_stream_mode(st);
         for (int attempt = 1;; ++attempt) {
-            e.key_stream = e.key_mode != ST_NONE ? ctx->buf(stream_bytes(e.key_mode, cap)) : BufP();
-            for (Side* s : {&st.ls, &st.rs})
-                s->stream = s->stream_mode != ST_NONE ? ctx->buf(stream_bytes(s->stream_mode, cap)) : BufP();
-            if (K.attempts > 1) RJ_HIP(hipMemsetAsync(counters->p, 0, 8, ctx->stream));
+            if (hot) {
+                e.key_stream = hot->key_stream;
+            } else {
+                e.key_stream = e.key_mode != ST_NONE ? ctx->buf(stream_bytes(e.key_mode, cap)) : BufP();
+                for (Side* s : {&st.ls, &st.rs})
+                    s->stream = s->stream_mode != ST_NONE ? ctx->buf(stream_bytes(s->stream_mode, cap)) : BufP();
+            }
+            if (hot)
+                launch_hot_seed(L, hot->hs(), counters->as<unsigned long long>());
+            else if (K.attempts > 1)
+                RJ_HIP(hipMemsetAsync(counters->p, 0, 8, ctx->stream));
             launch(out_stream(e.key_stream, e.key_mode), cap);
             e.finished.clear();
             finish_paged_streams(st, e, counters, cap);
             unsigned long long h = 0;
             RJ_HIP(hipMemcpyAsync(&h, counters->p, 8, hipMemcpyDeviceToHost, ctx->stream));
+            uint32_t hn[4] = {0, 0, 0, 0};
+            unsigned long long hcur = 0;
+            if (hot) {
+                RJ_HIP(hipMemcpyAsync(hn, &hot->hs()->n_sel, sizeof hn, hipMemcpyDeviceToHost, ctx->stream));
+                RJ_HIP(hipMemcpyAsync(&hcur, &hot->hs()->cursor, 8, hipMemcpyDeviceToHost, ctx->stream));
+            }
             ctx->sync();
             e.nrows = h;
+            if (hot) {
+                ctx->hot_debug[0] = 1;
+                ctx->hot_debug[1] = hn[1];
+                ctx->hot_debug[2] = hn[2];
+                ctx->hot_debug[3] = hcur;
+                if (e.nrows > cap) {
+                    if (e.nrows > 0xfffffff0ull) throw_fmt(RJ_ERR_UNSUPPORTED, "%s result exceeds 2^32 rows (%llu)", K.name, h);
+                    hot->overflowed = true;
+                    return e;
+                }
+            }
             if (e.nrows <= cap) return e;
             if (K.attempts == 1)
                 throw_fmt(RJ_ERR_DEVICE, "%s emitted %llu rows out of %llu", K.name, h, (unsigned long long)cap);
@@ -932,17 +979,76 @@
             fprintf(stderr, "[rj diag] join build=%llu probe=%llu bits=%u cw=%d/%d\n",
                     (unsigned long long)bs.rel->n, (unsigned long long)ps.rel->n, bits, bs.CW, ps.CW);
         if (broadcast_form(st, js)) return join_finish(st, js, nullptr, bits, root_res);
+        if (ctx->tune.debug_cap_hint > 0) st.cap_hint = (uint64_t)ctx->tune.debug_cap_hint;
+        uint64_t cap = first_cap(st.cap_hint);
+        if (hot_eligible(st, js, bits)) {
+            HotRun hot;
+            if (hot_sample(st, js, hot)) {
+                CoParts cp = hot_partition_sides(st, js, bits, cap, hot);
+                Rel     r = join_finish(st, js, &cp, bits, root_res, cap, &hot);
+                if (!hot.overflowed) return r;
+                cap = hot.overflowed_rows;
+                st.ls.stream.reset();
+                st.rs.stream.reset();
+            }
+        }
         CoParts cp = partition_sides(st, js, bits);
-        return join_finish(st, js, &cp, bits, root_res);
-    }
-
-    Rel join_finish(JoinState& st, const JoinSpec& js, CoParts* cp, uint32_t bits, Result* root_res) {
+        return join_finish(st, js, &cp, bits, root_res, cap);
+    }
+
+    bool hot_eligible(JoinState& st, const JoinSpec& js, uint32_t bits) const {
+        const Tuning& t = ctx->tune;
+        if (!t.hot || st.vkey || st.KW != 1 || js.prehashed || js.top_bits_taken) return false;
+        if ((bits + PT_MAXBITS - 1) / PT_MAXBITS != 2 || (bits <= (uint32_t)PT_FINEBITS && t.fine != 0)) return false;
+        for (Side* s : {&st.ls, &st.rs}) {
+            if (s->CW != 1 && s->CW != 2) return false;
+            if (s->carry_mode != CARRY_COLUMN && s->carry_mode != CARRY_ROWIDX) return false;
+            if (s->CW == 1 && t.pack != 1) return false;
+            if (s->CW == 2 && t.aos3 != 0 && (t.aos_mid == 1 || t.aos_mid == 3)) return false;
+        }
+        return st.ps().rel->n >= (uint64_t)std::max(t.hot_min_rows, 0);
+    }
+    bool hot_sample(JoinState& st, const JoinSpec& js, HotRun& hot) {
+        hot.state = ctx->buf(sizeof(HotState));
+        BufP cnt = ctx->buf((uint64_t)HOT_CNT_SLOTS * 8);
+        RJ_HIP(hipMemsetAsync(hot.state->p, 0, sizeof(HotState), ctx->stream));
+        RJ_HIP(hipMemsetAsync(cnt->p, 0, (uint64_t)HOT_CNT_SLOTS * 8, ctx->stream));
+        launch_hot_sample(L, make_src(st, st.ps(), js), cnt->as<uint32_t>(), cnt->as<uint32_t>() + HOT_CNT_SLOTS, hot.hs());
+        uint32_t n_sel = 0;
+        RJ_HIP(hipMemcpyAsync(&n_sel, &hot.hs()->n_sel, 4, hipMemcpyDeviceToHost, ctx->stream));
+        ctx->sync();
+        if (ctx->tune.diag >= 2) fprintf(stderr, "[rj diag] skew bypass: %u keys selected\n", n_sel);
+        return n_sel != 0;
+    }
+    CoParts hot_partition_sides(JoinState& st, const JoinSpec& js, uint32_t bits, uint64_t cap, HotRun& hot) {
+        CoParts        cp;
+        const TupleSrc sb = make_src(st, st.bs(), js), sp = make_src(st, st.ps(), js);
+        HotPass        hb{hot.hs(), nullptr};
+        cp.B = partition(&sb, nullptr, st.KW, st.bs().CW, bits, 0, false, nullptr, nullptr, nullptr, &hb);
+        launch_hot_finalize(L, hot.hs());
+        plan_carry_streams(st);
+        const int key_mode = key_stream_mode(st);
+        hot.key_stream = key_mode != ST_NONE ? ctx->buf(stream_bytes(key_mode, cap)) : BufP();
+        for (Side* s : {&st.ls, &st.rs})
+            s->stream = s->stream_mode != ST_NONE ? ctx->buf(stream_bytes(s->stream_mode, cap)) : BufP();
+        hot.emit.st = hot.hs();
+        hot.emit.key = out_stream(hot.key_stream, key_mode);
+        hot.emit.bc = out_stream(st.bs());
+        hot.emit.pc = out_stream(st.ps());
+        hot.emit.out_cap = cap;
+        HotPass hp{hot.hs(), &hot.emit};
+        cp.P = partition(&sp, nullptr, st.KW, st.ps().CW, bits, 0, false, nullptr, nullptr, nullptr, &hp);
+        return cp;
+    }
+
+    Rel join_finish(JoinState& st, const JoinSpec& js, CoParts* cp, uint32_t bits, Result* root_res, uint64_t cap = 0,
+                    HotRun* hot = nullptr) {
         Side &    bs = st.bs(), &ps = st.ps();
         const int KW = st.KW;
         BufP counters = ctx->buf(16);
         if (cp) heavy_tasks(*cp, counters);
         plan_carry_streams(st);
-        Emitted e = emit_with_retry(st, counters, first_cap(st.cap_hint), [&](const OutStream& key, uint64_t cap) {
+        Emitted e = emit_with_retry(st, counters, cap ? cap : first_cap(st.cap_hint), [&](const OutStream& key, uint64_t cap) {
             if (!cp) {
                 BcastParams bp{};
                 bp.R = make_src(st, bs, js);
@@ -994,7 +1100,11 @@
                     fprintf(stderr, "[rj diag]   %-16s %6.1f %%  %8.0f cyc/wg\n", names[i],
                             100.0 * hd[i] / tot, (double)hd[i] / PB.NP);
             }
-        });
+        }, hot);
+        if (hot && hot->overflowed) {
+            hot->overflowed_rows = e.nrows;
+            return Rel{};
+        }
         if (st.vkey && e.nrows) e.nrows = verify_varchar_pairs(st, e.nrows);
         return join_assemble(st, js, e, root_res);
     }
diff --git a/radix-join_amd/csrc/rj_internal.hpp b/radix-join_amd/csrc/rj_internal.hpp
--- a/radix-join_amd/csrc/rj_internal.hpp
+++ b/radix-join_amd/csrc/rj_internal.hpp
@@ -183,6 +183,9 @@
     int tpg2 = 0;
     int xcd_min_rows = 40 << 20;
     int xcd_split = 1;
+    int hot = 1;
+    int hot_min_rows = 40 << 20;
+    int debug_cap_hint = 0;
     int bcast = 1;
     int diag = 0;
     int varchar_dev_rows = 200000;
@@ -235,6 +238,7 @@
     Context*               group = nullptr;
     int                    n_lanes() const { return 1 + (int)peers.size(); }
     Context*               lane(int i) { return i == 0 ? this : peers[(size_t)i - 1]; }
+    uint64_t hot_debug[4] = {0, 0, 0, 0};
     int   n_cu = 0;
     int   compute_units();
     void  prewarm();
diff --git a/radix-join_amd/csrc/rj_kernels.hip b/radix-join_amd/csrc/rj_kernels.hip
--- a/radix-join_amd/csrc/rj_kernels.hip
+++ b/radix-join_amd/csrc/rj_kernels.hip
@@ -879,6 +879,122 @@
     for (uint32_t d = threadIdx.x; d < F; d += PT_THREADS) {
         uint32_t c = s_h[d];
         if (c) atomicAdd(&pp.hist[(((size_t)seg * F + d) << pp.xcd_log2) | (blockIdx.x & ((1u << pp.xcd_log2) - 1u))], c);
+    }
+}
+
+__device__ __forceinline__ uint32_t hot_find(const uint4* set4, uint32_t hk) {
+    const uint32_t b = hot_bucket(hk);
+    const uint4    q = set4[b >> 2];
+    uint32_t       s = HOT_SLOTS;
+    s = q.x == hk ? b : s;
+    s = q.y == hk ? b + 1u : s;
+    s = q.z == hk ? b + 2u : s;
+    s = q.w == hk ? b + 3u : s;
+    return hk ? s : HOT_SLOTS;
+}
+__device__ __forceinline__ void hot_load_set(uint4* s_set, const HotState* hs) {
+    const uint4* g = reinterpret_cast<const uint4*>(hs->set);
+    for (uint32_t i = threadIdx.x; i < HOT_SLOTS / 4; i += PT_THREADS) s_set[i] = g[i];
+}
+
+template <bool BUILD>
+__global__ __launch_bounds__(PT_THREADS) void k_hot_pass_hist(SrcLoader<1, 0> ld, PassParams pp, HotState* hs) {
+    __shared__ uint32_t s_h[PT_MAXF];
+    __shared__ uint4    s_set[HOT_SLOTS / 4];
+    __shared__ uint32_t s_nhot;
+    uint32_t            seg, begin, end;
+    if (!group_range(pp, blockIdx.x, seg, begin, end)) return;
+    const uint32_t F = 1u << pp.fanout_log2, mask = F - 1u;
+    for (uint32_t d = threadIdx.x; d < F; d += PT_THREADS) s_h[d] = 0;
+    hot_load_set(s_set, hs);
+    if (threadIdx.x == 0) s_nhot = 0;
+    lds_barrier();
+    uint32_t nhot = 0;
+    for (uint32_t base = begin; base < end; base += PT_TILE) {
+        uint32_t       hk[PT_ITEMS];
+        const uint32_t ok = ld.key_tile(base, end, hk);
+        const bool     vec = base + PT_TILE <= end;
+#pragma unroll
+        for (int j = 0; j < PT_ITEMS; ++j) {
+            const bool     v = (ok >> j) & 1u;
+            const uint32_t slot = hot_find(s_set, hk[j]);
+            const bool     hit = v && slot < HOT_SLOTS;
+            if constexpr (BUILD) {
+                if (hit) {
+                    const TupleSrc& s = ld.s;
+                    const uint32_t  row = SrcLoader<1, 0>::item_row(vec, base, j);
+                    uint32_t        lo = row, hi = 0;
+                    if (s.carry_mode == CARRY_COLUMN) {
+                        if (s.carry.width == 8) {
+                            const uint64_t c = col_load64(s.carry, row);
+                            lo = (uint32_t)c;
+                            hi = (uint32_t)(c >> 32);
+                        } else {
+                            lo = col_load32(s.carry, row);
+                        }
+                    }
+                    HotCand* c = hs->cand + slot;
+                    atomicAdd(&c->n, 1u);
+                    c->lo = lo;
+                    c->hi = hi;
+                }
+                if (v) atomicAdd(&s_h[pass_digit(pp, hk[j], mask)], 1u);
+            } else {
+                nhot += (uint32_t)__popcll(__ballot(hit));
+                if (v && !hit) atomicAdd(&s_h[pass_digit(pp, hk[j], mask)], 1u);
+            }
+        }
+    }
+    if constexpr (!BUILD)
+        if ((threadIdx.x & 63u) == 0 && nhot) atomicAdd(&s_nhot, nhot);
+    lds_barrier();
+    for (uint32_t d = threadIdx.x; d < F; d += PT_THREADS) {
+        uint32_t c = s_h[d];
+        if (c) atomicAdd(&pp.hist[(((size_t)seg * F + d) << pp.xcd_log2) | (blockIdx.x & ((1u << pp.xcd_log2) - 1u))], c);
+    }
+    if constexpr (!BUILD)
+        if (threadIdx.x == 0 && s_nhot) atomicAdd(&hs->n_hot_rows, s_nhot);
+}
+
+template <int NW>
+__device__ __forceinline__ uint32_t hot_mark(const uint4* s_set, uint32_t* s_hot, const uint32_t (&w)[PT_ITEMS][NW],
+                                             uint32_t& ok, uint32_t& wave_base) {
+    uint32_t hot = 0, n = 0;
+#pragma unroll
+    for (int j = 0; j < PT_ITEMS; ++j) {
+        const bool hit = ((ok >> j) & 1u) && hot_find(s_set, w[j][0]) < HOT_SLOTS;
+        hot |= (uint32_t)hit << j;
+        n += (uint32_t)__popcll(__ballot(hit));
+    }
+    ok &= ~hot;
+    uint32_t b = 0;
+    if ((threadIdx.x & 63u) == 0 && n) b = atomicAdd(&s_hot[0], n);
+    wave_base = __builtin_amdgcn_readfirstlane(b);
+    return hot;
+}
+__device__ __forceinline__ void hot_reserve(const HotParams& hp, uint32_t* s_hot) {
+    const uint32_t n = s_hot[0];
+    const unsigned long long at = n ? atomicAdd(&hp.st->cursor, (unsigned long long)n) : 0ull;
+    s_hot[2] = (uint32_t)at;
+    s_hot[3] = (uint32_t)(at >> 32);
+}
+template <int NW>
+__device__ __forceinline__ void hot_emit(const HotParams& hp, const uint4* s_set, const uint32_t* s_hot, uint32_t hot,
+                                         uint32_t wave_base, const uint32_t (&w)[PT_ITEMS][NW]) {
+    static_assert(NW == 2 || NW == 3, "one key word + a carry of one or two words");
+    uint64_t at = ((uint64_t)s_hot[2] | ((uint64_t)s_hot[3] << 32)) + wave_base;
+#pragma unroll
+    for (int j = 0; j < PT_ITEMS; ++j) {
+        const bool     h = (hot >> j) & 1u;
+        const uint64_t b = __ballot(h);
+        const uint64_t row = at + lane_prefix(b);
+        if (h && row < hp.out_cap) {
+            const HotCand* c = hp.st->cand + hot_find(s_set, w[j][0]);
+            stream_store(hp.key, row, unfmix32(w[j][0]), 0u);
+            stream_store(hp.bc, row, c->lo, c->hi);
+            stream_store(hp.pc, row, w[j][1], w[j][NW - 1]);
+        }
+        at += (uint64_t)__popcll(b);
     }
 }
 
@@ -979,29 +1095,43 @@
     }
 }
 
-template <int NW, class Loader, int PAIR, bool AOS>
-__global__ __launch_bounds__(PT_THREADS) void k_pass_scatter(Loader ld, PassParams pp, Words out) {
+template <int NW, class Loader, int PAIR, bool AOS, bool HOT>
+__device__ __forceinline__ void pass_scatter_body(Loader ld, PassParams pp, Words out, const HotParams* hp) {
     static_assert(PAIR < 0 || (PAIR >= 1 && PAIR + 1 < NW), "pair = two carry words behind the key");
     static_assert(!AOS || (NW == 3 && PAIR == 1), "12-byte tuples: one key word + a two-word carry");
+    static_assert(!HOT || (NW == 3 && PAIR == 1), "skew bypass: one key word + a two-word carry");
     __shared__ uint2    s_stage2[PT_TILE];
     uint32_t* const     s_stage = reinterpret_cast<uint32_t*>(s_stage2);
     __shared__ uint32_t s_cnt[PT_MAXF];
     __shared__ uint32_t s_base[PT_MAXF];
     __shared__ uint32_t s_delta[PT_MAXF];
     __shared__ uint32_t s_wsum[PT_THREADS / 64];
+    uint4*              s_set = nullptr;
+    uint32_t*           s_hot = nullptr;
+    if constexpr (HOT) {
+        __shared__ uint4    set_[HOT_SLOTS / 4];
+        __shared__ uint32_t hot_[4];
+        s_set = set_;
+        s_hot = hot_;
+    }
     uint32_t            seg, begin, end;
     if (!group_range(pp, blockIdx.x, seg, begin, end)) return;
     const uint32_t F = 1u << pp.fanout_log2, mask = F - 1u;
+    if constexpr (HOT) hot_load_set(s_set, hp->st);
 
     uint32_t run = 0;
     uint32_t w[PT_ITEMS][NW];
 
     for (uint32_t base = begin; base < end; base += PT_TILE) {
         for (uint32_t d = threadIdx.x; d < F; d += PT_THREADS) s_cnt[d] = 0;
+        if constexpr (HOT)
+            if (threadIdx.x == 0) s_hot[0] = 0;
         lds_barrier();
 
         uint32_t dr[PT_ITEMS];
-        const uint32_t ok = ld.template load_tile<NW>(base, end, w);
+        uint32_t ok = ld.template load_tile<NW>(base, end, w);
+        [[maybe_unused]] uint32_t hot = 0, hot_wave = 0;
+        if constexpr (HOT) hot = hot_mark<NW>(s_set, s_hot, w, ok, hot_wave);
 #pragma unroll
         for (int j = 0; j < PT_ITEMS; ++j) {
             dr[j] = 0xffffffffu;
@@ -1032,6 +1162,8 @@
             uint2* const       s_p = s_stage2;
             uint32_t* const    s_k = reinterpret_cast<uint32_t*>(s_stage2 + HALF);
             if (threadIdx.x < F) s_delta[threadIdx.x] = run - ex;
+            if constexpr (HOT)
+                if (threadIdx.x == 0) hot_reserve(*hp, s_hot);
 #pragma unroll
             for (int h = 0; h < 2; ++h) {
 #pragma unroll
@@ -1064,6 +1196,7 @@
                 }
                 lds_barrier();
             }
+            if constexpr (HOT) hot_emit<NW>(*hp, s_set, s_hot, hot, hot_wave, w);
             continue;
         }
 #pragma unroll
@@ -1117,27 +1250,47 @@
         }
     }
 }
-
-template <class Loader, bool BLK_OUT = false>
-__global__ __launch_bounds__(PT_THREADS) void k_pass_scatter_packed(Loader ld, PassParams pp, uint2* out) {
+template <int NW, class Loader, int PAIR, bool AOS>
+__global__ __launch_bounds__(PT_THREADS) void k_pass_scatter(Loader ld, PassParams pp, Words out) {
+    pass_scatter_body<NW, Loader, PAIR, AOS, false>(ld, pp, out, nullptr);
+}
+__global__ __launch_bounds__(PT_THREADS) void k_hot_pass_scatter(SrcLoader<1, 2> ld, PassParams pp, Words out, HotParams hp) {
+    pass_scatter_body<3, SrcLoader<1, 2>, 1, false, true>(ld, pp, out, &hp);
+}
+
+template <class Loader, bool BLK_OUT, bool HOT>
+__device__ __forceinline__ void pass_scatter_packed_body(Loader ld, PassParams pp, uint2* out, const HotParams* hp) {
     __shared__ uint2    s_stage[PT_TILE];
     __shared__ uint32_t s_cnt[PT_MAXF];
     __shared__ uint32_t s_base[PT_MAXF];
     __shared__ uint32_t s_delta[PT_MAXF];
     __shared__ uint32_t s_wsum[PT_THREADS / 64];
+    uint4*              s_set = nullptr;
+    uint32_t*           s_hot = nullptr;
+    if constexpr (HOT) {
+        __shared__ uint4    set_[HOT_SLOTS / 4];
+        __shared__ uint32_t hot_[4];
+        s_set = set_;
+        s_hot = hot_;
+    }
     uint32_t            seg, begin, end;
     if (!group_range(pp, blockIdx.x, seg, begin, end)) return;
     const uint32_t F = 1u << pp.fanout_log2, mask = F - 1u;
+    if constexpr (HOT) hot_load_set(s_set, hp->st);
 
     uint32_t run = 0;
     uint32_t w[PT_ITEMS][2];
     uint32_t ok_raw = ld.template issue_tile<2>(begin, end, w);
     for (uint32_t base = begin; base < end; base += PT_TILE) {
         for (uint32_t d = threadIdx.x; d < F; d += PT_THREADS) s_cnt[d] = 0;
+        if constexpr (HOT)
+            if (threadIdx.x == 0) s_hot[0] = 0;
         lds_barrier();
 
-        uint32_t       dr[PT_ITEMS];
-        const uint32_t ok = ld.template finish_tile<2>(base, end, ok_raw, w);
+        uint32_t dr[PT_ITEMS];
+        uint32_t ok = ld.template finish_tile<2>(base, end, ok_raw, w);
+        [[maybe_unused]] uint32_t hot = 0, hot_wave = 0;
+        if constexpr (HOT) hot = hot_mark<2>(s_set, s_hot, w, ok, hot_wave);
 #pragma unroll
         for (int j = 0; j < PT_ITEMS; ++j) {
             dr[j] = 0xffffffffu;
@@ -1156,12 +1309,15 @@
         uint32_t total;
         uint32_t ex = block_excl_scan(c, s_wsum, total);
         if (threadIdx.x < F) s_base[threadIdx.x] = ex;
+        if constexpr (HOT)
+            if (threadIdx.x == 0) hot_reserve(*hp, s_hot);
         lds_barrier();
 
 #pragma unroll
         for (int j = 0; j < PT_ITEMS; ++j)
             if (dr[j] != 0xffffffffu)
                 s_stage[s_base[dr[j] >> 16] + (dr[j] & 0xffffu)] = make_uint2(w[j][0], w[j][1]);
+        if constexpr (HOT) hot_emit<2>(*hp, s_set, s_hot, hot, hot_wave, w);
         if (base + PT_TILE < end) ok_raw = ld.template issue_tile<2>(base + PT_TILE, end, w);
         if (threadIdx.x < F) s_delta[threadIdx.x] = run - ex;
         lds_barrier();
@@ -1184,6 +1340,84 @@
         }
     }
 }
+template <class Loader, bool BLK_OUT = false>
+__global__ __launch_bounds__(PT_THREADS) void k_pass_scatter_packed(Loader ld, PassParams pp, uint2* out) {
+    pass_scatter_packed_body<Loader, BLK_OUT, false>(ld, pp, out, nullptr);
+}
+template <bool BLK_OUT>
+__global__ __launch_bounds__(PT_THREADS) void k_hot_pass_scatter_packed(SrcLoader<1, 1> ld, PassParams pp, uint2* out,
+                                                                         HotParams hp) {
+    pass_scatter_packed_body<SrcLoader<1, 1>, BLK_OUT, true>(ld, pp, out, &hp);
+}
+
+__global__ __launch_bounds__(256) void k_hot_sample(TupleSrc src, uint32_t n_samples, uint32_t* ckey, uint32_t* ccnt) {
+    const uint32_t i = blockIdx.x * 256u + threadIdx.x;
+    if (i >= n_samples) return;
+    const uint32_t row = (uint32_t)(((uint64_t)i * src.n_rows) / n_samples);
+    if (row >= src.n_rows || (src.key.valid && !src.key.valid[row])) return;
+    const uint32_t k = col_load32(src.key, row), hk = src.prehashed ? k : fmix32(k);
+    if (!hk) return;
+    uint32_t s = hk & (HOT_CNT_SLOTS - 1u);
+    for (int t = 0; t < HOT_CNT_WALK; ++t, s = (s + 1u) & (HOT_CNT_SLOTS - 1u)) {
+        const uint32_t prev = atomicCAS(&ckey[s], 0u, hk);
+        if (prev == 0u || prev == hk) {
+            atomicAdd(&ccnt[s], 1u);
+            return;
+        }
+    }
+}
+__global__ __launch_bounds__(256) void k_hot_tally(const uint32_t* ccnt, HotState* hs) {
+    for (uint32_t s = blockIdx.x * 256u + threadIdx.x; s < HOT_CNT_SLOTS; s += gridDim.x * 256u) {
+        const uint32_t c = ccnt[s];
+        if (c >= HOT_MIN_COUNT) atomicAdd(&hs->tally[min(c, HOT_CNT_BINS - 1u)], 1u);
+    }
+}
+__global__ __launch_bounds__(256) void k_hot_select(const uint32_t* ckey, const uint32_t* ccnt, HotState* hs) {
+    __shared__ uint32_t s_t[HOT_CNT_BINS];
+    __shared__ uint32_t s_thr;
+    for (uint32_t b = threadIdx.x; b < HOT_CNT_BINS; b += 256u) s_t[b] = hs->tally[b];
+    __syncthreads();
+    if (threadIdx.x == 0) {
+        uint32_t above = 0, thr = 0xffffffffu;
+        for (uint32_t b = HOT_CNT_BINS - 1u; b >= HOT_MIN_COUNT && above + s_t[b] <= HOT_MAX; --b) {
+            above += s_t[b];
+            thr = b;
+        }
+        s_thr = thr;
+    }
+    __syncthreads();
+    const uint32_t thr = s_thr;
+    for (uint32_t s = blockIdx.x * 256u + threadIdx.x; s < HOT_CNT_SLOTS; s += gridDim.x * 256u) {
+        if (ccnt[s] < thr) continue;
+        const uint32_t hk = ckey[s], b = hot_bucket(hk);
+        for (uint32_t t = 0; t < 4u; ++t)
+            if (atomicCAS(&hs->set[b + t], 0u, hk) == 0u) {
+                atomicAdd(&hs->n_sel, 1u);
+                break;
+            }
+    }
+}
+__global__ __launch_bounds__(256) void k_hot_finalize(HotState* hs) {
+    __shared__ uint32_t s_n;
+    if (threadIdx.x == 0) s_n = 0;
+    __syncthreads();
+    uint32_t n = 0;
+    for (uint32_t s = threadIdx.x; s < HOT_SLOTS; s += 256u) {
+        if (hs->set[s] == 0u) continue;
+        if (hs->cand[s].n == 1u)
+            ++n;
+        else
+            hs->set[s] = 0u;
+    }
+    if (n) atomicAdd(&s_n, n);
+    __syncthreads();
+    if (threadIdx.x == 0) {
+        hs->n_set = s_n;
+        hs->n_hot_rows = 0;
+        hs->cursor = 0;
+    }
+}
+__global__ void k_hot_seed(const HotState* hs, unsigned long long* out_cursor) { *out_cursor = hs->n_hot_rows; }
 
 __global__ void k_heavy_tasks(const uint32_t* offR, const uint32_t* offS, uint32_t NP,
                               uint32_t* tasks, uint32_t* n_heavy, uint32_t max_tasks) {
@@ -3145,6 +3379,45 @@
     });
 }
 
+void launch_hot_sample(const Launch& L, const TupleSrc& src, uint32_t* ckey, uint32_t* ccnt, HotState* hs) {
+    const uint32_t n_samples = std::min<uint32_t>(HOT_SAMPLES, src.n_rows);
+    if (!n_samples) return;
+    RJ_KLAUNCH(L, "hot_sample", k_hot_sample, (n_samples + 255u) / 256u, 256, src, n_samples, ckey, ccnt);
+    RJ_KLAUNCH(L, "hot_tally", k_hot_tally, 512, 256, (const uint32_t*)ccnt, hs);
+    RJ_KLAUNCH(L, "hot_select", k_hot_select, 512, 256, (const uint32_t*)ckey, (const uint32_t*)ccnt, hs);
+}
+void launch_hot_finalize(const Launch& L, HotState* hs) { RJ_KLAUNCH(L, "hot_finalize", k_hot_finalize, 1, 256, hs); }
+void launch_hot_seed(const Launch& L, const HotState* hs, unsigned long long* out_cursor) {
+    RJ_KLAUNCH(L, "hot_seed", k_hot_seed, 1, 1, hs, out_cursor);
+}
+void launch_hot_pass_hist(const Launch& L, const TupleSrc& src, const PassParams& pp, uint32_t n_groups, HotState* hs,
+                          bool build) {
+    if (!n_groups) return;
+    SrcLoader<1, 0> ld{src};
+    if (build)
+        RJ_KLAUNCH(L, "pass1_hist", (k_hot_pass_hist<true>), n_groups, PT_THREADS, ld, pp, hs);
+    else
+        RJ_KLAUNCH(L, "pass1_hist", (k_hot_pass_hist<false>), n_groups, PT_THREADS, ld, pp, hs);
+}
+void launch_hot_pass_scatter(const Launch& L, const TupleSrc& src, int carry_words, const PassParams& pp,
+                             uint32_t n_groups, const Words& out, bool blocked_out, const HotParams& hp) {
+    if (!n_groups) return;
+    if (src.carry_mode == CARRY_WIDE) launch_failed("pass1_scatter", "skew bypass: wide carry", true);
+    if (carry_words == 2) {
+        SrcLoader<1, 2> ld{src};
+        RJ_KLAUNCH(L, "pass1_scatter", k_hot_pass_scatter, n_groups, PT_THREADS, ld, pp, out, hp);
+    } else if (carry_words == 1) {
+        SrcLoader<1, 1> ld{src};
+        uint2*          o = reinterpret_cast<uint2*>(out.w[0]);
+        if (blocked_out)
+            RJ_KLAUNCH(L, "pass1_scatter", (k_hot_pass_scatter_packed<true>), n_groups, PT_THREADS, ld, pp, o, hp);
+        else
+            RJ_KLAUNCH(L, "pass1_scatter", (k_hot_pass_scatter_packed<false>), n_groups, PT_THREADS, ld, pp, o, hp);
+    } else {
+        launch_failed("pass1_scatter", "skew bypass: one or two carry words", true);
+    }
+}
+
 void launch_pass_hist_dense(const Launch& L, const Words& in, const PassParams& pp,
                             uint32_t n_groups) {
     if (!n_groups) return;
diff --git a/radix-join_amd/csrc/rj_kernels.hpp b/radix-join_amd/csrc/rj_kernels.hpp
--- a/radix-join_amd/csrc/rj_kernels.hpp
+++ b/radix-join_amd/csrc/rj_kernels.hpp
@@ -42,6 +42,14 @@
                       const uint32_t* coarse_x = nullptr);
 void launch_pass_scatter_src(const Launch& L, const TupleSrc& src, int key_words, int carry_words,
                              const PassParams& pp, uint32_t n_groups, const Words& out, bool aos3 = false);
+void launch_hot_sample(const Launch& L, const TupleSrc& probe, uint32_t* ckey, uint32_t* ccnt, HotState* hs);
+void launch_hot_pass_hist(const Launch& L, const TupleSrc& src, const PassParams& pp, uint32_t n_groups, HotState* hs,
+                          bool build);
+void launch_hot_finalize(const Launch& L, HotState* hs);
+void launch_hot_pass_scatter(const Launch& L, const TupleSrc& src, int carry_words, const PassParams& pp,
+                             uint32_t n_groups, const Words& out, bool blocked_out, const HotParams& hp);
+void launch_hot_seed(const Launch& L, const HotState* hs, unsigned long long* out_cursor);
+
 void launch_pass_hist_dense(const Launch& L, const Words& in, const PassParams& pp,
                             uint32_t n_groups);
 void launch_pass_scatter_dense(const Launch& L, const Words& in, int n_words, int pair_word,
diff --git a/radix-join_amd/pyrj/capi.py b/radix-join_amd/pyrj/capi.py
--- a/radix-join_amd/pyrj/capi.py
+++ b/radix-join_amd/pyrj/capi.py
@@ -131,6 +131,7 @@
     "rj_debug_launch_log",
     "rj_debug_launch_read",
     "rj_debug_pool",
+    "rj_debug_hot",
     "rj_device_query",
 ]
 
@@ -243,6 +244,8 @@
     L.rj_debug_launch_read.restype = C.c_int
     L.rj_debug_pool.argtypes = [vp, C.POINTER(u64)]
     L.rj_debug_pool.restype = C.c_int
+    L.rj_debug_hot.argtypes = [vp, C.POINTER(u64)]
+    L.rj_debug_hot.restype = C.c_int
     L.rj_device_query.argtypes = [vp, C.POINTER(rj_device_info)]
     L.rj_device_query.restype = C.c_int
     _LIB = L
@@ -483,6 +486,11 @@
         self._check(self.L.rj_debug_pool(self.h, out))
         return {"in_use": out[0], "cached": out[1], "fills": out[2], "filled_bytes": out[3]}
 
+    def hot_stats(self) -> dict:
+        out = (C.c_uint64 * 4)()
+        self._check(self.L.rj_debug_hot(self.h, out))
+        return {"taken": bool(out[0]), "set_size": out[1], "n_hot_rows": out[2], "hot_cursor": out[3]}
+
     def launch_log(self, on=True):
         self._check(self.L.rj_debug_launch_log(self.h, 1 if on else 0))
 
```

Result: slower. 28.69 billion (-9.5%).
